# bentherien/point-cloud-reid

Hardware: NVIDIA B200
Metric: pair scores/sec (PT-256 encode + all-pairs xcorr_eff match) (higher is better)
Workload: dtype f16

## Files before the change

point-cloud-reid_b200/_lib.py:

```python
import ctypes
import os

_HERE = os.path.dirname(os.path.abspath(__file__))
LIB_PATH = os.path.join(_HERE, "libpcreid_sm100.so")
_lib = None

c_int, c_ll, c_float, c_vp = ctypes.c_int, ctypes.c_longlong, ctypes.c_float, ctypes.c_void_p


class LinearArgs(ctypes.Structure):
    _fields_ = [
        ("B", c_int), ("rows", c_int), ("CO", c_int), ("K1", c_int), ("K2", c_int),
        ("X1", c_vp), ("x1_bs", c_ll), ("ldx1", c_int), ("x1_pm", c_int), ("x1_map", c_vp),
        ("X2", c_vp), ("x2_bs", c_ll), ("ldx2", c_int), ("x2_pm", c_int), ("x2_map", c_vp),
        ("W1", c_vp), ("w1_bs", c_ll), ("w1_map", c_vp),
        ("W2", c_vp), ("w2_bs", c_ll),
        ("bias", c_vp),
        ("R", c_vp), ("r_bs", c_ll), ("ldr", c_int), ("r_map", c_vp), ("res_after_act", c_int),
        ("act", c_int),
        ("Y", c_vp), ("y_bs", c_ll), ("ldy", c_int), ("y_pm", c_int),
    ]


class NormArgs(ctypes.Structure):
    _fields_ = [
        ("B", c_int), ("rows", c_int), ("C", c_int), ("G", c_int),
        ("X", c_vp), ("x_bs", c_ll), ("ldx", c_int),
        ("gamma", c_vp), ("beta", c_vp),
        ("R", c_vp), ("r_bs", c_ll), ("ldr", c_int), ("r_map", c_vp),
        ("act", c_int),
        ("Y", c_vp), ("y_bs", c_ll), ("ldy", c_int),
    ]


_SIGS = {
    "pcreid_abi_version": [],
    "pcreid_fps": [c_int, c_int, c_int, c_vp, c_vp, c_vp, c_vp],
    "pcreid_fps_with_dist": [c_int, c_int, c_int, c_vp, c_vp, c_vp, c_vp],
    "pcreid_fps_block_size": [c_int],
    "pcreid_fps_torch": [c_int, c_int, c_int, c_vp, c_vp, c_vp, c_vp],
    "pcreid_pairwise_sqdist": [c_int, c_int, c_int, c_int, c_vp, c_vp, c_vp, c_int, c_vp],
    "pcreid_knn": [c_int, c_int, c_int, c_int, c_vp, c_vp, c_vp, c_vp, c_vp],
    "pcreid_knn_t": [c_int, c_int, c_int, c_int, c_vp, c_vp, c_vp, c_vp, c_vp],
    "pcreid_knn_point": [c_int, c_int, c_int, c_int, c_vp, c_vp, c_vp, c_vp],
    "pcreid_knn_point_set": [c_int, c_int, c_int, c_int, c_vp, c_vp, c_vp, c_vp],
    "pcreid_knn_feature": [c_int, c_int, c_int, c_int, c_vp, c_ll, c_vp, c_vp],
    "pcreid_ball_query": [c_int, c_int, c_int, c_float, c_float, c_int, c_vp, c_vp, c_vp, c_vp],
    "pcreid_query_ball_point": [c_int, c_int, c_int, c_float, c_int, c_vp, c_vp, c_vp, c_vp],
    "pcreid_group_points": [c_int, c_int, c_int, c_int, c_int, c_vp, c_vp, c_vp, c_vp],
    "pcreid_gather_points": [c_int, c_int, c_int, c_int, c_vp, c_vp, c_vp, c_vp],
    "pcreid_query_group": [c_int] * 5 + [c_vp] * 4 + [c_int, c_float, c_vp, c_vp, c_vp],
    "pcreid_crop_tiles": [c_int],
    "pcreid_crop_mask": [c_int, c_int, c_vp, c_int, c_vp, c_vp, c_vp, c_vp],
    "pcreid_crop_gather": [c_int, c_int, c_int, c_vp, c_int, c_vp, c_vp, c_vp, c_vp, c_vp, c_vp],
    "pcreid_three_nn": [c_int, c_int, c_int, c_vp, c_vp, c_vp, c_vp, c_vp],
    "pcreid_three_interpolate": [c_int, c_int, c_int, c_int, c_vp, c_vp, c_vp, c_vp, c_vp],
    "pcreid_cn_linear": [ctypes.POINTER(LinearArgs), c_vp],
    "pcreid_cn_linear_tc": [ctypes.POINTER(LinearArgs), c_vp],
    "pcreid_cn_linear_tc2": [ctypes.POINTER(LinearArgs), c_vp, c_vp, c_int, c_vp],
    "pcreid_cn_linear_tma": [ctypes.POINTER(LinearArgs), c_ll, c_ll, c_ll, c_int, c_int, c_vp],
    "pcreid_cn_linear_tma_x3": [ctypes.POINTER(LinearArgs), c_vp, c_vp, c_ll, c_ll, c_ll, c_int, c_vp],
    "pcreid_cn_groupnorm": [ctypes.POINTER(NormArgs), c_vp],
    "pcreid_gn_res_relu_dot": [c_int, c_int, c_int, c_vp, c_int, c_vp, c_vp, c_vp, c_int, c_vp, c_float, c_vp, c_vp],
    "pcreid_attn_front_blob_bytes": [c_int, c_int, c_int, c_int],
    "pcreid_attn_front": [c_int, c_int, c_int, c_int, c_int, c_int, c_vp, c_vp, c_ll, c_int, c_vp, c_vp, c_vp, c_vp, c_vp, c_ll, c_int,
                          c_vp],
    "pcreid_linattn_kv_img": [c_int, c_int, c_int, c_int, c_vp, c_ll, c_int, c_vp, c_ll, c_int, c_vp, c_vp, c_vp],
    "pcreid_attn_back_objects_per_tile": [c_int, c_int],
    "pcreid_attn_back_blob_bytes": [c_int, c_int, c_int, c_int],
    "pcreid_attn_back": [c_int] * 8 + [c_vp, c_ll, c_int, c_vp, c_ll, c_int] + [c_vp] * 7 + [c_vp, c_ll, c_int, c_vp],
    "pcreid_linattn_kv": [c_int, c_int, c_int, c_int, c_vp, c_ll, c_int, c_vp, c_ll, c_int, c_vp, c_vp, c_vp],
    "pcreid_linattn_scale": [c_int, c_int, c_int, c_int, c_int, c_vp, c_ll, c_int, c_vp, c_vp, c_vp, c_vp, c_ll, c_int, c_vp],
    "pcreid_local_linattn": [c_int, c_int, c_int, c_int, c_int, c_vp, c_vp, c_vp, c_vp],
    "pcreid_cn_pool": [c_int, c_int, c_int, c_vp, c_ll, c_int, c_int, c_vp, c_ll, c_int, c_int, c_vp, c_ll, c_ll, c_vp],
    "pcreid_cn_chanmax": [c_int, c_int, c_int, c_vp, c_ll, c_int, c_vp, c_ll, c_ll, c_vp],
    "pcreid_sa_edge_mlp": [c_int, c_int, c_int, c_int, c_int, c_vp, c_vp, c_vp, c_vp, c_vp, c_vp, c_vp, c_vp, c_vp],
    "pcreid_edge_build": [c_int, c_int, c_int, c_int, c_int, c_vp, c_vp, c_vp, c_vp, c_vp],
    "pcreid_seg_max": [c_ll, c_int, c_vp, c_vp, c_vp],
    "pcreid_seg_mean": [c_ll, c_int, c_vp, c_vp, c_vp],
    "pcreid_edge_gather_max": [c_int, c_int, c_int, c_int, c_vp, c_vp, c_vp, c_int, c_vp, c_ll, c_int, c_vp],
    "pcreid_pack_image": [c_int, c_int, c_int, c_vp, c_ll, c_int, c_int, c_int, c_vp, c_vp],
    "pcreid_pack_image_bias": [c_int, c_int, c_int, c_vp, c_ll, c_int, c_vp, c_int, c_vp, c_vp],
    "pcreid_pack_b7": [c_int, c_vp, c_vp, c_int, c_vp, c_vp],
    "pcreid_pool_finish2": [c_int, c_int, c_vp, c_vp, c_vp, c_vp],
    "pcreid_pair_p1a2": [c_int, c_int, c_int, c_int, c_float] + [c_vp] * 8 + [c_int, c_vp],
    "pcreid_pair_p1b_n": [c_int, c_int, c_int, c_int, c_float] + [c_vp] * 7 + [c_int, c_vp],
    "pcreid_pair_p2y": [c_int, c_int, c_int, c_int, c_float] + [c_vp] * 5 + [c_int, c_vp],
    "pcreid_sa_edge_mlp_tc": [c_int, c_int, c_int, c_int, c_int] + [c_vp] * 8 + [c_int, c_vp],
    "pcreid_sa_edge_mlp_tc2": [c_int, c_int, c_int, c_int, c_int] + [c_vp] * 8 + [c_int, c_int, c_vp],
    "pcreid_pair_concat_head_tc": [c_int, c_int, c_int, c_int] + [c_vp] * 10 + [c_float, c_vp, c_vp, c_int, c_vp],
    "pcreid_pair_concat_head": [c_int, c_int, c_int, c_int] + [c_vp] * 10 + [c_float, c_vp, c_vp, c_vp],
}

ERRORS = {1: "PCREID_ERR_ARG (bad pointer/size)", 2: "PCREID_ERR_LAUNCH (CUDA launch failed)",
          3: "PCREID_ERR_UNSUPPORTED (shape outside the built kernels)"}


def exported_symbols():
    return sorted(_SIGS.keys())


def lib():
    global _lib
    if _lib is not None:
        return _lib
    if not os.path.exists(LIB_PATH):
        from . import build as _build
        _build.build_library()
    if not os.path.exists(LIB_PATH):
        raise RuntimeError(f"{LIB_PATH} is missing and could not be built: the CUDA extension is required "
                           "(no CPU fallback exists)")
    L = ctypes.CDLL(LIB_PATH)
    for name, argt in _SIGS.items():
        fn = getattr(L, name)
        fn.argtypes = argt
        fn.restype = c_int
    _lib = L
    return L


ABI_CALLS = 0


def check(rc, what):
    global ABI_CALLS
    ABI_CALLS += 1
    if rc != 0:
        raise RuntimeError(f"{what} failed: {ERRORS.get(rc, rc)}")
```

point-cloud-reid_b200/csrc/attn_tc.cu:

```cuda
#include "../../include/pcreid.h"
#include "common.cuh"
#include "tc_common.cuh"

namespace {

constexpr int NTH = 128;
constexpr int RING = 3;
constexpr int MAXCH = 56;
constexpr int MAX_SLOT = 16384;

struct ChunkTab {
  int n;
  int slot_bytes;
  uint32_t off[MAXCH];
  uint32_t bytes[MAXCH];
  uint8_t per_obj[MAXCH];
};

__device__ __forceinline__ void expect_tx(uint64_t* bar, uint32_t bytes) {
  asm volatile("mbarrier.arrive.expect_tx.shared::cta.b64 _, [%0], %1;" ::"r"(tc::smem_u32(bar)), "r"(bytes) : "memory");
}
__device__ __forceinline__ void bulk_g2s(uint32_t dst, const void* src, uint32_t bytes, uint64_t* bar) {
  asm volatile("cp.async.bulk.shared::cluster.global.mbarrier::complete_tx::bytes [%0], [%1], %2, [%3];" ::"r"(dst), "l"(src),
               "r"(bytes), "r"(tc::smem_u32(bar))
               : "memory");
}

struct Pipe {
  uint64_t *full, *empty;
  uint32_t ring_s;
  const uint8_t *blob, *obj;
  const ChunkTab* tab;
  int loaded, used;
};

__device__ __forceinline__ void pipe_prefetch(Pipe& p) {
  while (p.loaded < p.tab->n && p.loaded < p.used + RING) {
    const int s = p.loaded % RING, n = p.loaded / RING;
    if (n > 0) tc::mbar_wait(&p.empty[s], (uint32_t)((n - 1) & 1));
    const uint8_t* src = (p.tab->per_obj[p.loaded] ? p.obj : p.blob) + p.tab->off[p.loaded];
    const uint32_t nb = p.tab->bytes[p.loaded];
    expect_tx(&p.full[s], nb);
    bulk_g2s(p.ring_s + (uint32_t)(s * p.tab->slot_bytes), src, nb, &p.full[s]);
    ++p.loaded;
  }
}

__device__ __forceinline__ void pipe_gemm(Pipe& p, uint32_t tmem_d, uint32_t a_img_s, int K, int N, bool accumulate) {
  int kk = 0;
  while (kk < K) {
    pipe_prefetch(p);
    const int s = p.used % RING, n = p.used / RING;
    const int kc = (int)(p.tab->bytes[p.used] / (uint32_t)(N * 4));
    tc::mbar_wait(&p.full[s], (uint32_t)(n & 1));
    tc::tc_fence_after();
    const uint32_t slot = p.ring_s + (uint32_t)(s * p.tab->slot_bytes);
    for (int n0 = 0; n0 < N; n0 += 256) {
      const int nb = min(256, N - n0);
      const uint32_t idesc = tc::instr_desc(128, nb, tc::FMT_TF32, tc::MAJOR_K, tc::MAJOR_K);
      for (int ks = 0; ks < kc / 8; ++ks) {
        const uint64_t ad = tc::smem_desc(a_img_s + (uint32_t)(((kk >> 3) + ks) * 4096), 2048, 128, tc::LAYOUT_NONE);
        const uint64_t bd = tc::smem_desc(slot + (uint32_t)(ks * 2 * N * 16 + n0 * 16), (uint32_t)(N * 16), 128, tc::LAYOUT_NONE);
        tc::umma_tf32(tmem_d + (uint32_t)n0, ad, bd, idesc, (accumulate || kk > 0 || ks > 0) ? 1u : 0u);
      }
    }
    tc::umma_commit(&p.empty[s]);
    ++p.used;
    kk += kc;
  }
}

__device__ __forceinline__ void stage_sync() {
  tc::fence_async_smem();
  tc::tc_fence_before();
  __syncthreads();
  tc::tc_fence_after();
}

__device__ __forceinline__ float elu1(float v) { return v > 0.f ? v + 1.f : __expf(v); }

template <bool RNA>
__device__ __forceinline__ void load_image_cm(uint8_t* img, const float* __restrict__ Xr, int ld, int C, int CP, bool valid, int tid) {
  for (int c0 = 0; c0 < CP; c0 += 32) {
    float v[32];
#pragma unroll
    for (int i = 0; i < 32; ++i) v[i] = (valid && c0 + i < C) ? __ldg(Xr + (size_t)(c0 + i) * ld) : 0.f;
#pragma unroll
    for (int j = 0; j < 8; ++j)
      if (c0 + 4 * j < CP)
        *reinterpret_cast<float4*>(img + ((c0 >> 2) + j) * 2048 + tid * 16) =
            RNA ? tc::tf32_rna4(make_float4(v[4 * j], v[4 * j + 1], v[4 * j + 2], v[4 * j + 3])) : make_float4(v[4 * j], v[4 * j + 1], v[4 * j + 2], v[4 * j + 3]);
  }
}
template <bool RNA>
__device__ __forceinline__ void load_image_pm(uint8_t* img, const float* __restrict__ x, int C, int CP, bool valid, int tid) {
  for (int c0 = 0; c0 < CP; c0 += 32) {
    float v[32];
#pragma unroll
    for (int i = 0; i < 32; ++i) v[i] = (valid && c0 + i < C) ? __ldg(x + c0 + i) : 0.f;
#pragma unroll
    for (int j = 0; j < 8; ++j)
      if (c0 + 4 * j < CP)
        *reinterpret_cast<float4*>(img + ((c0 >> 2) + j) * 2048 + tid * 16) =
            RNA ? tc::tf32_rna4(make_float4(v[4 * j], v[4 * j + 1], v[4 * j + 2], v[4 * j + 3])) : make_float4(v[4 * j], v[4 * j + 1], v[4 * j + 2], v[4 * j + 3]);
  }
}

__device__ __forceinline__ void row_stats(uint32_t tl, int n, float& mean, float& rstd) {
  float s = 0.f;
  for (int q = 0; q < n / 16; ++q) {
    uint32_t r[16];
    tc::tmem_ld16(tl + 16 * q, r);
    tc::tmem_ld_wait();
#pragma unroll
    for (int j = 0; j < 16; ++j) s += __uint_as_float(r[j]);
  }
  mean = s / (float)n;
  float v = 0.f;
  for (int q = 0; q < n / 16; ++q) {
    uint32_t r[16];
    tc::tmem_ld16(tl + 16 * q, r);
    tc::tmem_ld_wait();
#pragma unroll
    for (int j = 0; j < 16; ++j) {
      const float d = __uint_as_float(r[j]) - mean;
      v = fmaf(d, d, v);
    }
  }
  rstd = rsqrtf(v / (float)n + 1e-5f);
}

__host__ __device__ inline int tmem_cols(int n) {
  int c = 32;
  while (c < n) c <<= 1;
  return c;
}

struct FrontArgs {
  int B, S, C2, DP, NFP, NF;
  const float* xyz;
  const float* feat;
  long long f_bs;
  int ldf;
  const float *wp0, *bp0, *bp2;
  const uint8_t* blob;
  float* out;
  long long o_bs;
  int ldo;
  ChunkTab tab;
};

__global__ void __launch_bounds__(NTH) attn_front_kernel(const __grid_constant__ FrontArgs a) {
  extern __shared__ __align__(128) uint8_t smem[];
  __shared__ uint64_t full[RING], empty[RING], stagebar;
  __shared__ uint32_t tmem_base_s;
  const int tid = threadIdx.x, warp = tid >> 5;
  const long long flat = (long long)blockIdx.x * 128 + tid;
  const bool valid = flat < (long long)a.B * a.S;
  const int b = valid ? (int)(flat / a.S) : 0, row = valid ? (int)(flat % a.S) : 0;
  const int CA = a.DP > a.C2 ? a.DP : a.C2;
  uint8_t* imgF = smem;
  uint8_t* imgA = imgF + a.C2 * 512;
  uint8_t* ring = imgA + CA * 512;
  float* wp0_s = reinterpret_cast<float*>(ring + RING * a.tab.slot_bytes);
  float* bp0_s = wp0_s + 3 * a.DP;
  float* bp2_s = bp0_s + a.DP;
  const int ncols = a.NFP + a.NF;
  if (tid == 0) {
    for (int i = 0; i < RING; ++i) { tc::mbar_init(&full[i], 1); tc::mbar_init(&empty[i], 1); }
    tc::mbar_init(&stagebar, 1);
    tc::fence_mbar_init();
  }
  if (warp == 0) { tc::tmem_alloc(&tmem_base_s, (uint32_t)tmem_cols(max(ncols, a.C2))); tc::tmem_relinquish(); }
  for (int i = tid; i < 3 * a.DP; i += NTH) wp0_s[i] = a.wp0[i];
  for (int i = tid; i < a.DP; i += NTH) bp0_s[i] = a.bp0[i];
  for (int i = tid; i < a.C2; i += NTH) bp2_s[i] = a.bp2[i];
  tc::tc_fence_before();
  __syncthreads();
  tc::tc_fence_after();
  Pipe p;
  if (tid == 0) {
    p.full = full; p.empty = empty; p.ring_s = tc::smem_u32(ring); p.blob = a.blob; p.obj = nullptr; p.tab = &a.tab;
    p.loaded = 0; p.used = 0;
    pipe_prefetch(p);
  }
  const uint32_t tmem = tmem_base_s;
  const uint32_t tl = tmem + ((uint32_t)(warp * 32) << 16);
  uint32_t par = 0;
  load_image_cm<false>(imgF, a.feat + (size_t)b * a.f_bs + row, a.ldf, a.C2, a.C2, valid, tid);
  {
    float x = 0.f, y = 0.f, z = 0.f;
    if (valid) {
      const float* pp = a.xyz + ((size_t)b * a.S + row) * 3;
      x = __ldg(pp); y = __ldg(pp + 1); z = __ldg(pp + 2);
    }
    for (int c4 = 0; c4 < a.DP / 4; ++c4) {
      float h[4];
#pragma unroll
      for (int j = 0; j < 4; ++j) {
        const int c = 4 * c4 + j;
        h[j] = fmaxf(fmaf(x, wp0_s[c], fmaf(y, wp0_s[a.DP + c], fmaf(z, wp0_s[2 * a.DP + c], bp0_s[c]))), 0.f);
      }
      *reinterpret_cast<float4*>(imgA + c4 * 2048 + tid * 16) = tc::tf32_rna4(make_float4(h[0], h[1], h[2], h[3]));
    }
  }
  stage_sync();
  if (tid == 0) {
    pipe_gemm(p, tmem, tc::smem_u32(imgA), a.DP, a.C2, false);
    tc::umma_commit(&stagebar);
    pipe_prefetch(p);
  }
  __syncwarp();
  tc::mbar_wait(&stagebar, par);
  par ^= 1u;
  tc::tc_fence_after();
  for (int q = 0; q < a.C2 / 16; ++q) {
    uint32_t r[16];
    tc::tmem_ld16(tl + 16 * q, r);
    tc::tmem_ld_wait();
#pragma unroll
    for (int j = 0; j < 16; j += 4) {
      const int c = 16 * q + j;
      const float4 f = *reinterpret_cast<const float4*>(imgF + (c / 4) * 2048 + tid * 16);
      float4 v;
      v.x = __uint_as_float(r[j + 0]) + bp2_s[c + 0] + f.x;
      v.y = __uint_as_float(r[j + 1]) + bp2_s[c + 1] + f.y;
      v.z = __uint_as_float(r[j + 2]) + bp2_s[c + 2] + f.z;
      v.w = __uint_as_float(r[j + 3]) + bp2_s[c + 3] + f.w;
      *reinterpret_cast<float4*>(imgA + (c / 4) * 2048 + tid * 16) = tc::tf32_rna4(v);
      *reinterpret_cast<float4*>(imgF + (c / 4) * 2048 + tid * 16) = tc::tf32_rna4(f);
    }
  }
  stage_sync();
  if (tid == 0) {
    pipe_gemm(p, tmem, tc::smem_u32(imgA), a.C2, a.NFP, false);
    if (a.NF > 0) pipe_gemm(p, tmem + (uint32_t)a.NFP, tc::smem_u32(imgF), a.C2, a.NF, false);
    tc::umma_commit(&stagebar);
  }
  __syncwarp();
  tc::mbar_wait(&stagebar, par);
  par ^= 1u;
  tc::tc_fence_after();
  float* O = a.out + (size_t)b * a.o_bs;
  for (int q = 0; q < ncols / 16; ++q) {
    uint32_t r[16];
    tc::tmem_ld16(tl + 16 * q, r);
    tc::tmem_ld_wait();
    if (valid) {
#pragma unroll
      for (int j = 0; j < 16; ++j) O[(size_t)(16 * q + j) * a.ldo + row] = __uint_as_float(r[j]);
    }
  }
  tc::tc_fence_before();
  __syncthreads();
  if (warp == 0) tc::tmem_dealloc(tmem, (uint32_t)tmem_cols(max(ncols, a.C2)));
}

constexpr int KV_SC = 64, KV_SCP = KV_SC + 4;
template <int TPT>
__global__ void __launch_bounds__(256, 3) linattn_kv_img_kernel(int S, int d, int H, const float* __restrict__ K, long long k_bs, int ldk,
                                                             const float* __restrict__ V, long long v_bs, int ldv,
                                                             float* __restrict__ kvimg, float* __restrict__ ksum) {
  extern __shared__ __align__(16) float kvs[];
  float* Ks = kvs;
  float* Vs = kvs + d * KV_SCP;
  const int b = blockIdx.x, tid = threadIdx.x, dh = d / H, nb = dh / 4;
  const int ntiles = H * nb * nb;
  const int G = ntiles >= 256 ? 1 : 256 / ntiles;
  const float* Kb = K + (size_t)b * k_bs;
  const float* Vb = V + (size_t)b * v_bs;
  float acc[TPT][4][4];
#pragma unroll
  for (int u = 0; u < TPT; ++u)
#pragma unroll
    for (int i = 0; i < 4; ++i)
#pragma unroll
      for (int j = 0; j < 4; ++j) acc[u][i][j] = 0.f;
  float ks = 0.f;
  const int g = G > 1 ? tid / ntiles : 0;
  for (int s0 = 0; s0 < S; s0 += KV_SC) {
    for (int i0 = tid; i0 < d * KV_SC; i0 += 256 * 8) {
      float kq[8], vq[8];
#pragma unroll
      for (int e = 0; e < 8; ++e) {
        const int i = i0 + e * 256, c = i / KV_SC, s = i % KV_SC;
        const bool in = i < d * KV_SC && s0 + s < S;
        kq[e] = in ? __ldg(Kb + (size_t)c * ldk + s0 + s) : 0.f;
        vq[e] = in ? __ldg(Vb + (size_t)c * ldv + s0 + s) : 0.f;
      }
#pragma unroll
      for (int e = 0; e < 8; ++e) {
        const int i = i0 + e * 256, c = i / KV_SC, s = i % KV_SC;
        if (i < d * KV_SC) {
          Ks[c * KV_SCP + s] = s0 + s < S ? elu1(kq[e]) : 0.f;
          Vs[c * KV_SCP + s] = vq[e];
        }
      }
    }
    __syncthreads();
    if (tid < d) {
      const float4* kr = reinterpret_cast<const float4*>(Ks + tid * KV_SCP);
#pragma unroll 4
      for (int s = 0; s < KV_SC / 4; ++s) { const float4 x = kr[s]; ks += (x.x + x.y) + (x.z + x.w); }
    }
#pragma unroll
    for (int u = 0; u < TPT; ++u) {
      const int tile = (G > 1 ? tid % ntiles : tid) + u * 256;
      if (tile < ntiles) {
        const int h = tile / (nb * nb), ti = (tile % (nb * nb)) / nb, tj = tile % nb;
        const float* kr = Ks + (h * dh + 4 * ti) * KV_SCP;
        const float* vr = Vs + (h * dh + 4 * tj) * KV_SCP;
        for (int s = 4 * g; s < KV_SC; s += 4 * G) {
          float4 kq[4], vq[4];
#pragma unroll
          for (int i = 0; i < 4; ++i) kq[i] = *reinterpret_cast<const float4*>(kr + i * KV_SCP + s);
#pragma unroll
          for (int j = 0; j < 4; ++j) vq[j] = *reinterpret_cast<const float4*>(vr + j * KV_SCP + s);
#pragma unroll
          for (int i = 0; i < 4; ++i)
#pragma unroll
            for (int j = 0; j < 4; ++j)
              acc[u][i][j] = fmaf(kq[i].x, vq[j].x, fmaf(kq[i].y, vq[j].y, fmaf(kq[i].z, vq[j].z, fmaf(kq[i].w, vq[j].w, acc[u][i][j]))));
        }
      }
    }
    __syncthreads();
  }
  if (tid < d) ksum[(size_t)b * d + tid] = ks;
  if (G > 1) {
    float* red = kvs;
    const int tile = tid % ntiles;
#pragma unroll
    for (int i = 0; i < 4; ++i)
      *reinterpret_cast<float4*>(red + ((size_t)(g * ntiles + tile) * 16) + 4 * i) = make_float4(acc[0][i][0], acc[0][i][1], acc[0][i][2], acc[0][i][3]);
    __syncthreads();
    if (g == 0) {
      for (int gg = 1; gg < G; ++gg)
#pragma unroll
        for (int i = 0; i < 4; ++i) {
          const float4 x = *reinterpret_cast<const float4*>(red + ((size_t)(gg * ntiles + tile) * 16) + 4 * i);
          acc[0][i][0] += x.x; acc[0][i][1] += x.y; acc[0][i][2] += x.z; acc[0][i][3] += x.w;
        }
    }
  }
  float* img = kvimg + (size_t)b * d * dh;
#pragma unroll
  for (int u = 0; u < TPT; ++u) {
    const int tile = (G > 1 ? tid % ntiles : tid) + u * 256;
    if (tile < ntiles && g == 0) {
      const int h = tile / (nb * nb), ti = (tile % (nb * nb)) / nb, tj = tile % nb;
      float* ih = img + (size_t)h * dh * dh;
#pragma unroll
      for (int j = 0; j < 4; ++j)
        *reinterpret_cast<float4*>(ih + ((size_t)ti * dh + 4 * tj + j) * 4) = tc::tf32_rna4(make_float4(acc[u][0][j], acc[u][1][j], acc[u][2][j], acc[u][3][j]));
    }
  }
}

struct BackArgs {
  int B, rows, D, H, C1, C1P, CO, opt;
  int qpre, res, f1_pm;
  const float* feat1;
  long long f1_bs;
  int ldf1;
  const float* q;
  long long q_bs;
  int ldq;
  const float* ksum;
  const uint8_t* kvimg;
  const float *g1, *b1, *g2, *b2;
  const uint8_t* blob;
  float* out;
  long long o_bs;
  int ldo;
  ChunkTab tab;
};

__global__ void __launch_bounds__(NTH) attn_back_kernel(const __grid_constant__ BackArgs a) {
  extern __shared__ __align__(128) uint8_t smem[];
  __shared__ uint64_t full[RING], empty[RING], stagebar;
  __shared__ uint32_t tmem_base_s;
  const int tid = threadIdx.x, warp = tid >> 5;
  const int D = a.D, D2 = 2 * a.D, dh = a.D / a.H;
  int b0, ob, row;
  bool valid;
  if (a.opt > 1) {
    b0 = blockIdx.x * a.opt; ob = tid / a.rows; row = tid % a.rows;
    valid = b0 + ob < a.B;
  } else {
    const int tpo = (a.rows + 127) / 128;
    b0 = blockIdx.x / tpo; ob = 0; row = (blockIdx.x % tpo) * 128 + tid;
    valid = row < a.rows;
  }
  const int b = valid ? b0 + ob : b0;
  const int img_ch = (a.C1P + D) > D2 ? (a.C1P + D) : D2;
  uint8_t* imgF = smem;
  uint8_t* imgQ = imgF + a.C1P * 512;
  uint8_t* imgH = smem;
  uint8_t* ring = smem + img_ch * 512;
  float* ksum_s = reinterpret_cast<float*>(ring + RING * a.tab.slot_bytes);
  float* g1_s = ksum_s + a.opt * D;
  float* b1_s = g1_s + D;
  float* g2_s = b1_s + D;
  float* b2_s = g2_s + a.CO;
  const int tcols = tmem_cols(max(max(D2, a.CO), a.opt * D));
  if (tid == 0) {
    for (int i = 0; i < RING; ++i) { tc::mbar_init(&full[i], 1); tc::mbar_init(&empty[i], 1); }
    tc::mbar_init(&stagebar, 1);
    tc::fence_mbar_init();
  }
  if (warp == 0) { tc::tmem_alloc(&tmem_base_s, (uint32_t)tcols); tc::tmem_relinquish(); }
  for (int i = tid; i < a.opt * D; i += NTH) ksum_s[i] = (b0 + i / D < a.B) ? a.ksum[(size_t)(b0 + i / D) * D + i % D] : 0.f;
  for (int i = tid; i < D; i += NTH) { g1_s[i] = a.g1[i]; b1_s[i] = a.b1[i]; }
  for (int i = tid; i < a.CO; i += NTH) { g2_s[i] = a.g2[i]; b2_s[i] = a.b2[i]; }
  tc::tc_fence_before();
  __syncthreads();
  tc::tc_fence_after();
  Pipe p;
  if (tid == 0) {
    p.full = full; p.empty = empty; p.ring_s = tc::smem_u32(ring); p.blob = a.blob;
    p.obj = a.kvimg + (size_t)b0 * D * dh * 4; p.tab = &a.tab;
    p.loaded = 0; p.used = 0;
    pipe_prefetch(p);
  }
  const uint32_t tmem = tmem_base_s;
  const uint32_t tl = tmem + ((uint32_t)(warp * 32) << 16);
  uint32_t par = 0;
  const float* F1 = a.feat1 + (size_t)b * a.f1_bs;
  if (a.f1_pm) load_image_pm<true>(imgF, F1 + (size_t)row * a.C1, a.C1, a.C1P, valid, tid);
  else load_image_cm<true>(imgF, F1 + row, a.ldf1, a.C1, a.C1P, valid, tid);
  const float* ksr = ksum_s + ob * D;

  float z[4] = {0.f, 0.f, 0.f, 0.f};
  if (a.qpre) {
    const float* Q = a.q + (size_t)b * a.q_bs + row;
    float dot[4] = {0.f, 0.f, 0.f, 0.f};
    for (int c0 = 0; c0 < D; c0 += 16) {
      float v[16];
#pragma unroll
      for (int i = 0; i < 16; ++i) v[i] = valid ? __ldg(Q + (size_t)(c0 + i) * a.ldq) : 0.f;
      const int h = c0 / dh;
      float dd = 0.f;
#pragma unroll
      for (int i = 0; i < 16; ++i) {
        v[i] = elu1(v[i]);
        dd = fmaf(v[i], ksr[c0 + i], dd);
      }
#pragma unroll
      for (int hh = 0; hh < 4; ++hh) dot[hh] += (hh == h) ? dd : 0.f;
#pragma unroll
      for (int j = 0; j < 4; ++j)
        *reinterpret_cast<float4*>(imgQ + ((c0 >> 2) + j) * 2048 + tid * 16) = tc::tf32_rna4(make_float4(v[4 * j], v[4 * j + 1], v[4 * j + 2], v[4 * j + 3]));
    }
#pragma unroll
    for (int hh = 0; hh < 4; ++hh) z[hh] = 1.f / (dot[hh] + 1e-6f);
    stage_sync();
  } else {
    stage_sync();
    if (tid == 0) {
      pipe_gemm(p, tmem, tc::smem_u32(imgF), a.C1P, D, false);
      tc::umma_commit(&stagebar);
      pipe_prefetch(p);
    }
    __syncwarp();
    tc::mbar_wait(&stagebar, par);
    par ^= 1u;
    tc::tc_fence_after();
    float dot[4] = {0.f, 0.f, 0.f, 0.f};
    for (int q = 0; q < D / 16; ++q) {
      uint32_t r[16];
      tc::tmem_ld16(tl + 16 * q, r);
      tc::tmem_ld_wait();
      const int h = (16 * q) / dh;
      float v[16];
      float dd = 0.f;
#pragma unroll
      for (int j = 0; j < 16; ++j) {
        v[j] = elu1(__uint_as_float(r[j]));
        dd = fmaf(v[j], ksr[16 * q + j], dd);
      }
#pragma unroll
      for (int hh = 0; hh < 4; ++hh) dot[hh] += (hh == h) ? dd : 0.f;
#pragma unroll
      for (int j = 0; j < 16; j += 4)
        *reinterpret_cast<float4*>(imgQ + ((16 * q + j) / 4) * 2048 + tid * 16) = tc::tf32_rna4(make_float4(v[j], v[j + 1], v[j + 2], v[j + 3]));
    }
#pragma unroll
    for (int hh = 0; hh < 4; ++hh) z[hh] = 1.f / (dot[hh] + 1e-6f);
    stage_sync();
  }
  if (tid == 0) {
    for (int o = 0; o < a.opt; ++o)
      for (int h = 0; h < a.H; ++h)
        pipe_gemm(p, tmem + (uint32_t)(o * D + h * dh), tc::smem_u32(imgQ) + (uint32_t)((h * dh / 8) * 4096), dh, dh, false);
    tc::umma_commit(&stagebar);
    pipe_prefetch(p);
  }
  __syncwarp();
  tc::mbar_wait(&stagebar, par);
  par ^= 1u;
  tc::tc_fence_after();
  for (int q = 0; q < D / 16; ++q) {
    uint32_t r[16];
    tc::tmem_ld16(tl + (uint32_t)(ob * D + 16 * q), r);
    tc::tmem_ld_wait();
    const int h = (16 * q) / dh;
    float zz = z[0];
#pragma unroll
    for (int hh = 1; hh < 4; ++hh) zz = (hh == h) ? z[hh] : zz;
#pragma unroll
    for (int j = 0; j < 16; j += 4)
      *reinterpret_cast<float4*>(imgQ + ((16 * q + j) / 4) * 2048 + tid * 16) =
          tc::tf32_rna4(make_float4(__uint_as_float(r[j]) * zz, __uint_as_float(r[j + 1]) * zz, __uint_as_float(r[j + 2]) * zz, __uint_as_float(r[j + 3]) * zz));
  }
  stage_sync();
  if (tid == 0) {
    pipe_gemm(p, tmem, tc::smem_u32(imgQ), D, D, false);
    tc::umma_commit(&stagebar);
    pipe_prefetch(p);
  }
  __syncwarp();
  tc::mbar_wait(&stagebar, par);
  par ^= 1u;
  tc::tc_fence_after();
  {
    float mean, rstd;
    row_stats(tl, D, mean, rstd);
    for (int q = 0; q < D / 16; ++q) {
      uint32_t r[16];
      tc::tmem_ld16(tl + 16 * q, r);
      tc::tmem_ld_wait();
#pragma unroll
      for (int j = 0; j < 16; j += 4) {
        const int c = 16 * q + j;
        float4 v;
        v.x = (__uint_as_float(r[j + 0]) - mean) * rstd * g1_s[c + 0] + b1_s[c + 0];
        v.y = (__uint_as_float(r[j + 1]) - mean) * rstd * g1_s[c + 1] + b1_s[c + 1];
        v.z = (__uint_as_float(r[j + 2]) - mean) * rstd * g1_s[c + 2] + b1_s[c + 2];
        v.w = (__uint_as_float(r[j + 3]) - mean) * rstd * g1_s[c + 3] + b1_s[c + 3];
        *reinterpret_cast<float4*>(imgQ + (c / 4) * 2048 + tid * 16) = tc::tf32_rna4(v);
      }
    }
  }
  stage_sync();
  if (tid == 0) {
    pipe_gemm(p, tmem, tc::smem_u32(imgF), a.C1P, D2, false);
    pipe_gemm(p, tmem, tc::smem_u32(imgQ), D, D2, true);
    tc::umma_commit(&stagebar);
    pipe_prefetch(p);
  }
  __syncwarp();
  tc::mbar_wait(&stagebar, par);
  par ^= 1u;
  tc::tc_fence_after();
  for (int q = 0; q < D2 / 16; ++q) {
    uint32_t r[16];
    tc::tmem_ld16(tl + 16 * q, r);
    tc::tmem_ld_wait();
#pragma unroll
    for (int j = 0; j < 16; j += 4) {
      float4 v;
      v.x = fmaxf(__uint_as_float(r[j + 0]), 0.f);
      v.y = fmaxf(__uint_as_float(r[j + 1]), 0.f);
      v.z = fmaxf(__uint_as_float(r[j + 2]), 0.f);
      v.w = fmaxf(__uint_as_float(r[j + 3]), 0.f);
      *reinterpret_cast<float4*>(imgH + ((16 * q + j) / 4) * 2048 + tid * 16) = tc::tf32_rna4(v);
    }
  }
  stage_sync();
  if (tid == 0) {
    pipe_gemm(p, tmem, tc::smem_u32(imgH), D2, a.CO, false);
    tc::umma_commit(&stagebar);
  }
  __syncwarp();
  tc::mbar_wait(&stagebar, par);
  par ^= 1u;
  tc::tc_fence_after();
  {
    float mean, rstd;
    row_stats(tl, a.CO, mean, rstd);
    float* O = a.out + (size_t)b * a.o_bs;
    for (int q = 0; q < a.CO / 16; ++q) {
      uint32_t r[16];
      tc::tmem_ld16(tl + 16 * q, r);
      tc::tmem_ld_wait();
      if (valid) {
        float rr[16];
#pragma unroll
        for (int j = 0; j < 16; ++j) {
          const int c = 16 * q + j;
          rr[j] = !a.res ? 0.f : (a.f1_pm ? __ldg(F1 + (size_t)row * a.C1 + c) : __ldg(F1 + (size_t)c * a.ldf1 + row));
        }
#pragma unroll
        for (int j = 0; j < 16; ++j) {
          const int c = 16 * q + j;
          O[(size_t)c * a.ldo + row] = (__uint_as_float(r[j]) - mean) * rstd * g2_s[c] + b2_s[c] + rr[j];
        }
      }
    }
  }
  tc::tc_fence_before();
  __syncthreads();
  if (warp == 0) tc::tmem_dealloc(tmem, (uint32_t)tcols);
}

struct TabBuilder {
  ChunkTab t;
  uint32_t blob_off = 0;
  bool ok = true;
  int cap;
  explicit TabBuilder(int img_bytes) : cap(img_bytes > 96 * 1024 ? MAX_SLOT : 8192) { t.n = 0; t.slot_bytes = 0; }
  void part(int K, int N, bool per_obj, uint32_t obj_off = 0) {
    int kc = K < 32 ? K : 32;
    while (kc > 8 && kc * N * 4 > cap) kc >>= 1;
    if (kc * N * 4 > MAX_SLOT || (K % 8) || (N % 16)) { ok = false; return; }
    uint32_t off = per_obj ? obj_off : blob_off;
    for (int kk = 0; kk < K; kk += kc) {
      const int k = (K - kk) < kc ? (K - kk) : kc;
      if (t.n >= MAXCH) { ok = false; return; }
      t.off[t.n] = off;
      t.bytes[t.n] = (uint32_t)(k * N * 4);
      t.per_obj[t.n] = per_obj ? 1 : 0;
      if ((int)t.bytes[t.n] > t.slot_bytes) t.slot_bytes = (int)t.bytes[t.n];
      off += t.bytes[t.n];
      ++t.n;
    }
    if (!per_obj) blob_off = off;
  }
  void finish() { t.slot_bytes = (t.slot_bytes + 1023) & ~1023; }
};

}

extern "C" {

int pcreid_attn_front_blob_bytes(int C2, int DP, int NFP, int NF) { return 4 * (DP * C2 + C2 * NFP + C2 * NF); }

int pcreid_attn_front(int B, int S, int C2, int DP, int NFP, int NF, const float* xyz, const float* feat, long long f_bs, int ldf,
                      const float* wp0, const float* bp0, const float* bp2, const void* blob, float* out, long long o_bs, int ldo,
                      void* stream) {
  if (B <= 0 || S <= 0) return PCREID_OK;
  if (!xyz || !feat || !wp0 || !bp0 || !bp2 || !blob || !out) return PCREID_ERR_ARG;
  if (C2 % 16 || DP % 16 || NFP % 16 || NF % 16 || NFP <= 0 || C2 > 128 || DP > 128 || NFP + NF > 512 || ((long long)B * S + 127) / 128 > 0x7fffffffLL)
    return PCREID_ERR_UNSUPPORTED;
  FrontArgs a;
  a.B = B; a.S = S; a.C2 = C2; a.DP = DP; a.NFP = NFP; a.NF = NF;
  a.xyz = xyz; a.feat = feat; a.f_bs = f_bs; a.ldf = ldf; a.wp0 = wp0; a.bp0 = bp0; a.bp2 = bp2;
  a.blob = static_cast<const uint8_t*>(blob); a.out = out; a.o_bs = o_bs; a.ldo = ldo;
  TabBuilder tb((C2 + (DP > C2 ? DP : C2)) * 512);
  tb.part(DP, C2, false);
  tb.part(C2, NFP, false);
  if (NF > 0) tb.part(C2, NF, false);
  tb.finish();
  if (!tb.ok) return PCREID_ERR_UNSUPPORTED;
  a.tab = tb.t;
  const int CA = DP > C2 ? DP : C2;
  const int smem = (C2 + CA) * 512 + RING * a.tab.slot_bytes + (4 * DP + C2) * 4;
  if (smem > 227 * 1024) return PCREID_ERR_UNSUPPORTED;
  cudaFuncSetAttribute(attn_front_kernel, cudaFuncAttributeMaxDynamicSharedMemorySize, smem);
  attn_front_kernel<<<(unsigned)(((long long)B * S + 127) / 128), NTH, smem, (cudaStream_t)stream>>>(a);
  return pcreid_launch_status();
}

int pcreid_linattn_kv_img(int B, int S, int d, int H, const float* K, long long k_bs, int ldk, const float* V, long long v_bs, int ldv,
                          float* kvimg, float* ksum, void* stream) {
  if (B <= 0) return PCREID_OK;
  if (!K || !V || !kvimg || !ksum || H <= 0 || S <= 0) return PCREID_ERR_ARG;
  if (d % H || (d / H) % 4 || d > 128 || d < 16) return PCREID_ERR_UNSUPPORTED;
  const int ntiles = H * (d / H / 4) * (d / H / 4);
  if (ntiles > 512 || (ntiles < 256 && 256 % ntiles)) return PCREID_ERR_UNSUPPORTED;
  const int G = ntiles >= 256 ? 1 : 256 / ntiles;
  int smem = 2 * d * KV_SCP * 4;
  if (G > 1 && G * ntiles * 16 * 4 > smem) smem = G * ntiles * 16 * 4;
  if (ntiles > 256) {
    if (smem > 48 * 1024) cudaFuncSetAttribute(linattn_kv_img_kernel<2>, cudaFuncAttributeMaxDynamicSharedMemorySize, smem);
    linattn_kv_img_kernel<2><<<B, 256, smem, (cudaStream_t)stream>>>(S, d, H, K, k_bs, ldk, V, v_bs, ldv, kvimg, ksum);
  } else {
    if (smem > 48 * 1024) cudaFuncSetAttribute(linattn_kv_img_kernel<1>, cudaFuncAttributeMaxDynamicSharedMemorySize, smem);
    linattn_kv_img_kernel<1><<<B, 256, smem, (cudaStream_t)stream>>>(S, d, H, K, k_bs, ldk, V, v_bs, ldv, kvimg, ksum);
  }
  return pcreid_launch_status();
}

int pcreid_attn_back_objects_per_tile(int rows, int D) {
  if (rows >= 128 || rows <= 0 || 128 % rows) return 1;
  const int opt = 128 / rows;
  return (opt <= 4 && opt * D <= 512) ? opt : 1;
}

int pcreid_attn_back_blob_bytes(int D, int C1P, int CO, int qpre) {
  return 4 * ((qpre ? 0 : C1P * D) + D * D + C1P * 2 * D + D * 2 * D + 2 * D * CO);
}

int pcreid_attn_back(int B, int rows, int D, int H, int C1, int CO, int res, int f1_pm, const float* feat1, long long f1_bs,
                     int ldf1, const float* q, long long q_bs, int ldq, const float* ksum, const float* kvimg, const float* g1,
                     const float* b1, const float* g2, const float* b2, const void* blob, float* out, long long o_bs, int ldo,
                     void* stream) {
  if (B <= 0 || rows <= 0) return PCREID_OK;
  if (!feat1 || !ksum || !kvimg || !g1 || !b1 || !g2 || !b2 || !blob || !out || H <= 0) return PCREID_ERR_ARG;
  const int C1P = (C1 + 7) & ~7;
  if (D % 16 || D > 128 || H > 4 || D % H || (D / H) % 16 || CO % 16 || CO > 2 * D || C1 <= 0 || C1P > 128) return PCREID_ERR_UNSUPPORTED;
  if (res && C1 != CO) return PCREID_ERR_ARG;
  const int dh = D / H;
  BackArgs a;
  a.B = B; a.rows = rows; a.D = D; a.H = H; a.C1 = C1; a.C1P = C1P; a.CO = CO;
  a.opt = pcreid_attn_back_objects_per_tile(rows, D);
  a.qpre = q ? 1 : 0; a.res = res; a.f1_pm = f1_pm;
  a.feat1 = feat1; a.f1_bs = f1_bs; a.ldf1 = ldf1; a.q = q; a.q_bs = q_bs; a.ldq = ldq; a.ksum = ksum;
  a.kvimg = reinterpret_cast<const uint8_t*>(kvimg); a.g1 = g1; a.b1 = b1; a.g2 = g2; a.b2 = b2;
  a.blob = static_cast<const uint8_t*>(blob); a.out = out; a.o_bs = o_bs; a.ldo = ldo;
  const long long tiles = a.opt > 1 ? ((long long)B + a.opt - 1) / a.opt : (long long)B * ((rows + 127) / 128);
  if (tiles > 0x7fffffffLL) return PCREID_ERR_UNSUPPORTED;
  TabBuilder tb(((C1P + D) > 2 * D ? (C1P + D) : 2 * D) * 512);
  if (!q) tb.part(C1P, D, false);
  for (int o = 0; o < a.opt; ++o)
    for (int h = 0; h < H; ++h) tb.part(dh, dh, true, (uint32_t)((o * H + h) * dh * dh * 4));
  tb.part(D, D, false);
  tb.part(C1P, 2 * D, false);
  tb.part(D, 2 * D, false);
  tb.part(2 * D, CO, false);
  tb.finish();
  if (!tb.ok) return PCREID_ERR_UNSUPPORTED;
  a.tab = tb.t;
  const int img_ch = (C1P + D) > 2 * D ? (C1P + D) : 2 * D;
  const int smem = img_ch * 512 + RING * a.tab.slot_bytes + ((a.opt + 2) * D + 2 * CO) * 4;
  if (smem > 227 * 1024 - 256) return PCREID_ERR_UNSUPPORTED;
  cudaFuncSetAttribute(attn_back_kernel, cudaFuncAttributeMaxDynamicSharedMemorySize, smem);
  attn_back_kernel<<<(unsigned)tiles, NTH, smem, (cudaStream_t)stream>>>(a);
  return pcreid_launch_status();
}

}
```

point-cloud-reid_b200/csrc/pair_common.cuh:

```cuda
#pragma once
#include "../../include/pcreid.h"
#include "common.cuh"
#include "tc_common.cuh"

namespace {


constexpr int IMG = 16384;
constexpr int NB7H = 80;
constexpr int B7_HEAD = (NB7H / 8) * 32 * 16;
constexpr int B7_BYTES = 2 * B7_HEAD;
constexpr int ONES_BYTES = 2 * 2048;
constexpr float LN_EPS = 1e-5f;

struct P1Args {
  int n_units, NT, role;
  int npts;
  float att_eps;
  float kv_scale;
  const int *u_search, *u_templ, *u_slot;
  const uint8_t *QF1, *H, *PV;
  const uint8_t* MK1;
  const uint8_t* W;
  uint8_t* A_out;
  uint8_t* B7_out;
};
struct P2Args {
  int n_units, NT, role;
  int npts;
  float att_eps;
  const int* u_slot;
  const uint8_t* A_in;
  const uint8_t* B7_in;
  const uint8_t* W;
  float* pool_part;
};

__device__ __forceinline__ float elu1(float x) { return x > 0.f ? x + 1.f : __expf(x); }

__device__ __forceinline__ uint4 ldg_early(const void* p) {
  uint4 v;
  asm volatile("ld.global.nc.L1::no_allocate.v4.u32 {%0,%1,%2,%3}, [%4];" : "=r"(v.x), "=r"(v.y), "=r"(v.z), "=r"(v.w) : "l"(p));
  return v;
}

__device__ __forceinline__ void prefetch_l2_16k(const uint8_t* img, int t) {
  asm volatile("prefetch.global.L2 [%0];" ::"l"(img + (size_t)t * 128));
}

__device__ __forceinline__ void copy_to_smem(uint8_t* dst, const uint8_t* __restrict__ src, int bytes, int t, int nthr) {
  for (int i = t * 16; i < bytes; i += nthr * 16) cp_async16(dst + i, src + i);
}

struct Opnd {
  uint64_t desc;
  uint32_t kstep;
};
__device__ __forceinline__ Opnd opnd(uint32_t addr, uint32_t lbo, uint32_t sbo, uint32_t kstep_bytes) {
  Opnd o;
  o.desc = tc::smem_desc(addr, lbo, sbo, tc::LAYOUT_NONE);
  o.kstep = kstep_bytes >> 4;
  return o;
}
#define A_IMG(addr) opnd((addr), 2048u, 128u, 4096u)
#define W_IMG(addr, N) opnd((addr), (uint32_t)((N)*16), 128u, (uint32_t)(2 * (N)*16))
#define B7_IMG(addr) opnd((addr), 128u, 512u, 256u)

template <int KSTEPS>
__device__ __forceinline__ void issue_gemm(uint32_t tmem_d, const Opnd& A, const Opnd& B, uint32_t idesc, bool accumulate) {
#pragma unroll
  for (int ks = 0; ks < KSTEPS; ++ks)
    tc::umma_f16(tmem_d, A.desc + (uint64_t)(ks * A.kstep), B.desc + (uint64_t)(ks * B.kstep), idesc, (accumulate || ks > 0) ? 1u : 0u);
}

template <int NCH>
__device__ __forceinline__ void load_side(uint4 (&sd)[NCH], const uint8_t* __restrict__ img, int chunk0, int row) {
#pragma unroll
  for (int c = 0; c < NCH; ++c) sd[c] = __ldg(reinterpret_cast<const uint4*>(img + (chunk0 + c) * 2048 + row * 16));
}

template <class F>
__device__ __forceinline__ void write_b7_part(const float (&M32)[32], int c_lo, float ksum, bool tail, int d, uint8_t* dst) {
  uint8_t* base = dst + (d >> 5) * B7_HEAD + (d & 31) * 16;
#pragma unroll
  for (int c = 0; c < 4; ++c) {
    uint32_t w[4];
#pragma unroll
    for (int j = 0; j < 4; ++j) w[j] = F::pack(M32[c * 8 + 2 * j], M32[c * 8 + 2 * j + 1]);
    *reinterpret_cast<uint4*>(base + (c_lo + c) * 512) = make_uint4(w[0], w[1], w[2], w[3]);
  }
  if (tail) {
    *reinterpret_cast<uint4*>(base + 8 * 512) = make_uint4(F::pack(ksum, 0.f), 0, 0, 0);
    *reinterpret_cast<uint4*>(base + 9 * 512) = make_uint4(0, 0, 0, 0);
  }
}

constexpr int GX = 128, NGX = 3;
struct GroupX {
  int t, gid;
  bool issuer;
  uint32_t tmem, tlane;
  uint64_t* bar;
  uint32_t par;
  __device__ __forceinline__ void sync() { tc::bar_sync(1 + gid, GX); }
  __device__ __forceinline__ void publish() { tc::fence_async_smem(); tc::tc_fence_before(); sync(); tc::tc_fence_after(); }
  __device__ __forceinline__ void wait() { tc::mbar_wait(bar, par); par ^= 1u; tc::tc_fence_after(); }
};

__device__ __forceinline__ void ld32_stats(uint32_t taddr, float (&o)[32], float& s, float& ss) {
#pragma unroll
  for (int half = 0; half < 2; ++half) {
    uint32_t r[16];
    tc::tmem_ld16(taddr + 16 * half, r);
    tc::tmem_ld_wait();
#pragma unroll
    for (int j = 0; j < 16; ++j) {
      const float v = __uint_as_float(r[j]);
      o[16 * half + j] = v;
      s += v;
      ss = fmaf(v, v, ss);
    }
  }
}

template <class F>
__device__ __forceinline__ void write_b7_row(const float (&M)[64], float ksum, int d, uint8_t* dst) {
  float lo[32], hi[32];
#pragma unroll
  for (int j = 0; j < 32; ++j) { lo[j] = M[j]; hi[j] = M[32 + j]; }
  write_b7_part<F>(lo, 0, ksum, true, d, dst);
  write_b7_part<F>(hi, 4, ksum, false, d, dst);
}

__device__ __forceinline__ void groupx_setup(GroupX& g, uint64_t* bars, uint32_t tmem_base) {
  const int warp_u = (int)tc::uniform(threadIdx.x >> 5);
  g.gid = warp_u / 4;
  g.t = threadIdx.x % GX;
  g.issuer = (warp_u % 4) == 0;
  g.tmem = tc::uniform(tmem_base) + g.gid * 160;
  g.tlane = g.tmem + ((uint32_t)((warp_u % 4) * 32) << 16);
  g.bar = bars + g.gid;
  g.par = 0;
}

}
```

point-cloud-reid_b200/csrc/pair_tc.cu:

```cuda
#include "pair_common.cuh"
#include <stdlib.h>

namespace {

constexpr int P1B_WKV = 0, P1B_WM = 16384, P1B_WBYTES = 24576;
constexpr int P1B_AIMG = 0, P1B_KFV = IMG, P1B_GBYTES = IMG + 2 * IMG + ONES_BYTES;

template <class F, int CS>
__global__ void __launch_bounds__(NGX * GX * CS, 1) pair_p1b_kernel(const P1Args a) {
  constexpr int GT = GX * CS, NTHR = NGX * GT;
  constexpr int QB = 4 / CS, CB = 8 / CS;
  extern __shared__ __align__(1024) uint8_t smem[];
  __shared__ uint64_t bars[2 * NGX];
  __shared__ uint32_t tmem_base_s;
  uint8_t* Wsm = smem;
  if (threadIdx.x == 0) {
    for (int i = 0; i < 2 * NGX; ++i) tc::mbar_init(&bars[i], 1);
    tc::fence_mbar_init();
  }
  if (threadIdx.x < 32) { tc::tmem_alloc(&tmem_base_s, 512); tc::tmem_relinquish(); }
  copy_to_smem(Wsm, a.W, P1B_WBYTES, threadIdx.x, NTHR);
  cp_async_commit();
  cp_async_wait<0>();
  tc::fence_async_smem();
  tc::tc_fence_before();
  __syncthreads();
  tc::tc_fence_after();
  const int warp_u = (int)tc::uniform(threadIdx.x >> 5);
  const int gid = warp_u / (4 * CS), wg = warp_u % (4 * CS), gt = threadIdx.x % GT;
  const int half = wg / 4;
  const int row = (wg % 4) * 32 + (threadIdx.x & 31);
  const bool issuer = wg == 0;
  const uint32_t tmem = tc::uniform(tmem_base_s) + gid * 160;
  const uint32_t tlane = tmem + ((uint32_t)((wg % 4) * 32) << 16);
  uint64_t* bar = bars + gid;
  uint32_t par = 0;
  auto gsync = [&]() { tc::bar_sync(1 + gid, GT); };
  auto publish = [&]() { tc::fence_async_smem(); tc::tc_fence_before(); gsync(); tc::tc_fence_after(); };
  auto gwait = [&]() { tc::mbar_wait(bar, par); par ^= 1u; tc::tc_fence_after(); };
  uint64_t* bar2 = bars + NGX + gid;
  uint32_t par2 = 0;
  uint8_t* G = smem + P1B_WBYTES + gid * P1B_GBYTES;
  uint8_t* Aimg = G + P1B_AIMG;
  uint8_t* KfV = G + P1B_KFV;
  {
    uint4* ones = reinterpret_cast<uint4*>(KfV + 2 * IMG);
    for (int i = gt; i < 256; i += GT) ones[i] = i < 128 ? make_uint4(F::ONE_LO, 0, 0, 0) : make_uint4(0, 0, 0, 0);
  }
  const uint32_t sA = tc::smem_u32(Aimg), sKfV = tc::smem_u32(KfV), sW = tc::smem_u32(Wsm);
  const uint32_t id64 = tc::instr_desc(128, 64, F::FMT, tc::MAJOR_K, tc::MAJOR_K);
  const uint32_t idkv = tc::instr_desc(128, 80, F::FMT, tc::MAJOR_MN, tc::MAJOR_MN);
  const Opnd oA = A_IMG(sA), oWk = W_IMG(sW + P1B_WKV, 128), oWv = W_IMG(sW + P1B_WKV + 64 * 16, 128), oWm = W_IMG(sW + P1B_WM, 64),
             oKfV = opnd(sKfV, 128u, 2048u, 256u), oVones = opnd(sKfV + 8 * 2048, 128u, 2048u, 256u);
  const uint32_t KVC = 64;

  const int ngroups = gridDim.x * NGX, gg = blockIdx.x * NGX + gid;
  const int u0 = (int)((long long)a.n_units * gg / ngroups), u1 = (int)((long long)a.n_units * (gg + 1) / ngroups);
  int so_next = u0 < u1 ? a.u_search[u0] : 0, slot_next = u0 < u1 ? a.u_slot[u0] : 0;
  bool prefetched = false;
  for (int u = u0; u < u1; ++u) {
    const int so = so_next, slot = slot_next;
    if (u + 1 < u1) { so_next = a.u_search[u + 1]; slot_next = a.u_slot[u + 1]; }
    for (int tile = 0; tile < a.NT; ++tile) {
      const size_t ti = (size_t)so * a.NT + tile;
      if (!prefetched) copy_to_smem(Aimg, a.A_out + (((size_t)slot * 2 + a.role) * a.NT + tile) * IMG, IMG, gt, GT);
      prefetched = false;
      cp_async_commit();
      {
        int ns = slot, nt = tile + 1;
        if (nt == a.NT) { ns = slot_next; nt = 0; }
        if ((nt != 0 || u + 1 < u1) && gt < 128) prefetch_l2_16k(a.A_out + (((size_t)ns * 2 + a.role) * a.NT + nt) * IMG, gt);
      }
      cp_async_wait<0>();
      publish();
      if (issuer) { if (tc::elect_one()) { issue_gemm<4>(tmem, oA, oWk, id64, false); tc::umma_commit(bar); } __syncwarp(); }
      gwait();
      if (tile > 0) { tc::mbar_wait(bar2, par2); par2 ^= 1u; tc::tc_fence_after(); }
      {
        const bool keep = tile * 128 + row < a.npts;
#pragma unroll
        for (int qq = 0; qq < QB; ++qq) {
          const int q = half * QB + qq;
          uint32_t r[16];
          tc::tmem_ld16(tlane + 16 * q, r);
          tc::tmem_ld_wait();
#pragma unroll
          for (int c = 0; c < 2; ++c) {
            uint32_t w[4];
#pragma unroll
            for (int j = 0; j < 4; ++j)
              w[j] = keep ? F::elu1(__uint_as_float(r[c * 8 + 2 * j]), __uint_as_float(r[c * 8 + 2 * j + 1])) : 0u;
            *reinterpret_cast<uint4*>(KfV + (2 * q + c) * 2048 + row * 16) = make_uint4(w[0], w[1], w[2], w[3]);
          }
        }
      }
      tc::tc_fence_before();
      gsync();
      tc::tc_fence_after();
      if (issuer) { if (tc::elect_one()) { issue_gemm<4>(tmem, oA, oWv, id64, false); tc::umma_commit(bar); } __syncwarp(); }
      {
        uint4 sdPV[CB];
        load_side<CB>(sdPV, a.PV + ti * IMG, half * CB, row);
        gwait();
        if (tile + 1 < a.NT) {
          copy_to_smem(Aimg, a.A_out + (((size_t)slot * 2 + a.role) * a.NT + tile + 1) * IMG, IMG, gt, GT);
          cp_async_commit();
          prefetched = true;
        }
#pragma unroll
        for (int qq = 0; qq < QB; ++qq) {
          const int q = half * QB + qq;
          uint32_t r[16];
          tc::tmem_ld16(tlane + 16 * q, r);
          tc::tmem_ld_wait();
#pragma unroll
          for (int c = 0; c < 2; ++c) {
            const uint4 s4 = sdPV[2 * qq + c];
            const uint32_t sw[4] = {s4.x, s4.y, s4.z, s4.w};
            uint32_t w[4];
#pragma unroll
            for (int j = 0; j < 4; ++j)
              w[j] = F::add(__uint_as_float(r[c * 8 + 2 * j]), __uint_as_float(r[c * 8 + 2 * j + 1]), sw[j]);
            *reinterpret_cast<uint4*>(KfV + (8 + 2 * q + c) * 2048 + row * 16) = make_uint4(w[0], w[1], w[2], w[3]);
          }
        }
      }
      publish();
      if (issuer) {
        if (tc::elect_one()) { issue_gemm<8>(tmem + KVC, oKfV, oVones, idkv, tile > 0); tc::umma_commit(bar2); }
        __syncwarp();
      }
    }
    tc::mbar_wait(bar2, par2);
    par2 ^= 1u;
    tc::tc_fence_after();
    {
      float kv[64 / CS];
      float ksum = 0.f;
      if (row < 64) {
#pragma unroll
        for (int qq = 0; qq < QB; ++qq) {
          uint32_t r[16];
          tc::tmem_ld16(tlane + KVC + 16 * (half * QB + qq), r);
          tc::tmem_ld_wait();
#pragma unroll
          for (int j = 0; j < 16; ++j) kv[16 * qq + j] = __uint_as_float(r[j]) * a.kv_scale;
        }
        uint32_t r8[8];
        tc::tmem_ld8(tlane + KVC + 64, r8);
        tc::tmem_ld_wait();
        ksum = __uint_as_float(r8[0]) * a.kv_scale;
        const int hd = row >> 5;
#pragma unroll
        for (int cc = 0; cc < CB; ++cc) {
          const int c = half * CB + cc;
          uint32_t w[4];
#pragma unroll
          for (int j = 0; j < 4; ++j) w[j] = ((c >> 2) == hd) ? F::pack(kv[cc * 8 + 2 * j], kv[cc * 8 + 2 * j + 1]) : 0u;
          *reinterpret_cast<uint4*>(Aimg + c * 2048 + row * 16) = make_uint4(w[0], w[1], w[2], w[3]);
        }
      } else {
#pragma unroll
        for (int cc = 0; cc < CB; ++cc) *reinterpret_cast<uint4*>(Aimg + (half * CB + cc) * 2048 + row * 16) = make_uint4(0, 0, 0, 0);
      }
      publish();
      if (issuer) { if (tc::elect_one()) { issue_gemm<4>(tmem, oA, oWm, id64, false); tc::umma_commit(bar); } __syncwarp(); }
      gwait();
      if (u + 1 < u1) {
        copy_to_smem(Aimg, a.A_out + ((size_t)slot_next * 2 + a.role) * a.NT * IMG, IMG, gt, GT);
        cp_async_commit();
        prefetched = true;
      }
      if (row < 64) {
#pragma unroll
        for (int qq = 0; qq < QB; ++qq) {
          uint32_t r[16];
          tc::tmem_ld16(tlane + 16 * (half * QB + qq), r);
          tc::tmem_ld_wait();
#pragma unroll
          for (int j = 0; j < 16; ++j) kv[16 * qq + j] = __uint_as_float(r[j]);
        }
        uint8_t* dst = a.B7_out + ((size_t)slot * 2 + a.role) * B7_BYTES;
        if constexpr (CS == 1) write_b7_row<F>(kv, ksum, row, dst);
        else write_b7_part<F>(kv, 4 * half, ksum, half == 0, row, dst);
      }
      tc::tc_fence_before();
      gsync();
    }
  }
  tc::tc_fence_before();
  __syncthreads();
  if (threadIdx.x < 32) tc::tmem_dealloc(tmem_base_s, 512);
}

template <class F>
__global__ void __launch_bounds__(NGX * GX, 1) pair_p1b2_kernel(const P1Args a) {
  constexpr int TG = 168, KVC = 64, AC = 136;
  extern __shared__ __align__(1024) uint8_t smem[];
  __shared__ uint64_t bars[2 * NGX];
  __shared__ uint32_t tmem_base_s;
  __shared__ float ksum_s[NGX][64];
  uint8_t* Wsm = smem;
  if (threadIdx.x == 0) {
    for (int i = 0; i < 2 * NGX; ++i) tc::mbar_init(&bars[i], 1);
    tc::fence_mbar_init();
  }
  if (threadIdx.x < 32) { tc::tmem_alloc(&tmem_base_s, 512); tc::tmem_relinquish(); }
  copy_to_smem(Wsm, a.W, P1B_WBYTES, threadIdx.x, NGX * GX);
  cp_async_commit();
  cp_async_wait<0>();
  tc::fence_async_smem();
  tc::tc_fence_before();
  __syncthreads();
  tc::tc_fence_after();
  const int warp_u = (int)tc::uniform(threadIdx.x >> 5);
  const int gid = warp_u / 4, wq = warp_u % 4, row = threadIdx.x % GX, lane = threadIdx.x & 31;
  const bool issuer = wq == 0;
  const uint32_t tmem = tc::uniform(tmem_base_s) + gid * TG;
  const uint32_t tlane = tmem + ((uint32_t)(wq * 32) << 16);
  uint64_t* bar = bars + gid;
  uint32_t par = 0;
  auto gsync = [&]() { tc::bar_sync(1 + gid, GX); };
  auto publish = [&]() { tc::fence_async_smem(); tc::tc_fence_before(); gsync(); tc::tc_fence_after(); };
  auto gwait = [&]() { tc::mbar_wait(bar, par); par ^= 1u; tc::tc_fence_after(); };
  uint64_t* bar2 = bars + NGX + gid;
  uint32_t par2 = 0;
  uint8_t* G = smem + P1B_WBYTES + gid * P1B_GBYTES;
  uint8_t* Aimg = G + P1B_AIMG;
  uint8_t* KfV = G + P1B_KFV;
  {
    uint4* ones = reinterpret_cast<uint4*>(KfV + 2 * IMG);
    ones[row] = make_uint4(F::ONE_LO, 0, 0, 0);
    ones[128 + row] = make_uint4(0, 0, 0, 0);
  }
  const uint32_t sA = tc::smem_u32(Aimg), sKfV = tc::smem_u32(KfV), sW = tc::smem_u32(Wsm);
  const uint32_t id64 = tc::instr_desc(128, 64, F::FMT, tc::MAJOR_K, tc::MAJOR_K);
  const uint32_t idkv = tc::instr_desc(64, 72, F::FMT, tc::MAJOR_MN, tc::MAJOR_MN);
  const Opnd oA = A_IMG(sA), oWk = W_IMG(sW + P1B_WKV, 128), oWv = W_IMG(sW + P1B_WKV + 64 * 16, 128), oWm = W_IMG(sW + P1B_WM, 64),
             oKf = opnd(sKfV, 128u, 2048u, 256u), oVones = opnd(sKfV + 8 * 2048, 128u, 2048u, 256u);

  const int ngroups = gridDim.x * NGX, gg = blockIdx.x * NGX + gid;
  const int u0 = (int)((long long)a.n_units * gg / ngroups), u1 = (int)((long long)a.n_units * (gg + 1) / ngroups);
  int so_next = u0 < u1 ? a.u_search[u0] : 0, slot_next = u0 < u1 ? a.u_slot[u0] : 0;
  uint32_t areg[32];
  auto load_row = [&](const uint8_t* img) {
#pragma unroll
    for (int c = 0; c < 8; ++c) {
      const uint4 v = ldg_early(img + c * 2048 + row * 16);
      areg[4 * c] = v.x; areg[4 * c + 1] = v.y; areg[4 * c + 2] = v.z; areg[4 * c + 3] = v.w;
    }
  };
  if (u0 < u1) load_row(a.A_out + ((size_t)slot_next * 2 + a.role) * a.NT * IMG);
  for (int u = u0; u < u1; ++u) {
    const int so = so_next, slot = slot_next;
    if (u + 1 < u1) { so_next = a.u_search[u + 1]; slot_next = a.u_slot[u + 1]; }
    for (int tile = 0; tile < a.NT; ++tile) {
      const size_t ti = (size_t)so * a.NT + tile;
      tc::tmem_st32(tlane + AC, areg);
      tc::tmem_st_wait();
      tc::tc_fence_before();
      gsync();
      tc::tc_fence_after();
      if (issuer) {
        if (tc::elect_one()) {
#pragma unroll
          for (int ks = 0; ks < 4; ++ks) tc::umma_f16_ts(tmem, tmem + AC + 8 * ks, oWk.desc + (uint64_t)(ks * oWk.kstep), id64, ks > 0 ? 1u : 0u);
          tc::umma_commit(bar);
        }
        __syncwarp();
      }
      {
        int ns = slot, nt = tile + 1;
        if (nt == a.NT) { ns = slot_next; nt = 0; }
        if (nt != 0 || u + 1 < u1) {
          load_row(a.A_out + (((size_t)ns * 2 + a.role) * a.NT + nt) * IMG);
          int ns2 = ns, nt2 = nt + 1;
          if (nt2 == a.NT) { nt2 = 0; ns2 = -1; }
          if (ns2 >= 0) prefetch_l2_16k(a.A_out + (((size_t)ns2 * 2 + a.role) * a.NT + nt2) * IMG, row);
        }
      }
      gwait();
      if (tile > 0) { tc::mbar_wait(bar2, par2); par2 ^= 1u; tc::tc_fence_after(); }
      {
        const bool keep = tile * 128 + row < a.npts;
#pragma unroll
        for (int q = 0; q < 4; ++q) {
          uint32_t r[16];
          tc::tmem_ld16(tlane + 16 * q, r);
          tc::tmem_ld_wait();
#pragma unroll
          for (int c = 0; c < 2; ++c) {
            uint32_t w[4];
#pragma unroll
            for (int j = 0; j < 4; ++j)
              w[j] = keep ? F::elu1(__uint_as_float(r[c * 8 + 2 * j]), __uint_as_float(r[c * 8 + 2 * j + 1])) : 0u;
            *reinterpret_cast<uint4*>(KfV + (2 * q + c) * 2048 + row * 16) = make_uint4(w[0], w[1], w[2], w[3]);
          }
        }
      }
      tc::tc_fence_before();
      gsync();
      tc::tc_fence_after();
      if (issuer) {
        if (tc::elect_one()) {
#pragma unroll
          for (int ks = 0; ks < 4; ++ks) tc::umma_f16_ts(tmem, tmem + AC + 8 * ks, oWv.desc + (uint64_t)(ks * oWv.kstep), id64, ks > 0 ? 1u : 0u);
          tc::umma_commit(bar);
        }
        __syncwarp();
      }
      {
        uint4 sdPV[8];
        load_side<8>(sdPV, a.PV + ti * IMG, 0, row);
        gwait();
#pragma unroll
        for (int q = 0; q < 4; ++q) {
          uint32_t r[16];
          tc::tmem_ld16(tlane + 16 * q, r);
          tc::tmem_ld_wait();
#pragma unroll
          for (int c = 0; c < 2; ++c) {
            const uint4 s4 = sdPV[2 * q + c];
            const uint32_t sw[4] = {s4.x, s4.y, s4.z, s4.w};
            uint32_t w[4];
#pragma unroll
            for (int j = 0; j < 4; ++j)
              w[j] = F::add(__uint_as_float(r[c * 8 + 2 * j]), __uint_as_float(r[c * 8 + 2 * j + 1]), sw[j]);
            *reinterpret_cast<uint4*>(KfV + (8 + 2 * q + c) * 2048 + row * 16) = make_uint4(w[0], w[1], w[2], w[3]);
          }
        }
      }
      publish();
      if (issuer) {
        if (tc::elect_one()) { issue_gemm<8>(tmem + KVC, oKf, oVones, idkv, tile > 0); tc::umma_commit(bar2); }
        __syncwarp();
      }
    }
    tc::mbar_wait(bar2, par2);
    par2 ^= 1u;
    tc::tc_fence_after();
    {
      {
        float kv[64];
        uint32_t r8[8];
#pragma unroll
        for (int q = 0; q < 4; ++q) {
          uint32_t r[16];
          tc::tmem_ld16(tlane + KVC + 16 * q, r);
          tc::tmem_ld_wait();
#pragma unroll
          for (int j = 0; j < 16; ++j) kv[16 * q + j] = __uint_as_float(r[j]) * a.kv_scale;
        }
        tc::tmem_ld8(tlane + KVC + 64, r8);
        tc::tmem_ld_wait();
        if (lane < 16) {
          const int i = 16 * wq + lane, hd = i >> 5;
          ksum_s[gid][i] = __uint_as_float(r8[0]) * a.kv_scale;
#pragma unroll
          for (int c = 0; c < 8; ++c) {
            uint32_t w[4];
#pragma unroll
            for (int j = 0; j < 4; ++j) w[j] = ((c >> 2) == hd) ? F::pack(kv[c * 8 + 2 * j], kv[c * 8 + 2 * j + 1]) : 0u;
            *reinterpret_cast<uint4*>(Aimg + c * 2048 + i * 16) = make_uint4(w[0], w[1], w[2], w[3]);
          }
        }
      }
      if (row >= 64) {
#pragma unroll
        for (int c = 0; c < 8; ++c) *reinterpret_cast<uint4*>(Aimg + c * 2048 + row * 16) = make_uint4(0, 0, 0, 0);
      }
      publish();
      if (issuer) { if (tc::elect_one()) { issue_gemm<4>(tmem, oA, oWm, id64, false); tc::umma_commit(bar); } __syncwarp(); }
      gwait();
      if (row < 64) {
        float kv[64];
#pragma unroll
        for (int q = 0; q < 4; ++q) {
          uint32_t r[16];
          tc::tmem_ld16(tlane + 16 * q, r);
          tc::tmem_ld_wait();
#pragma unroll
          for (int j = 0; j < 16; ++j) kv[16 * q + j] = __uint_as_float(r[j]);
        }
        write_b7_row<F>(kv, ksum_s[gid][row], row, a.B7_out + ((size_t)slot * 2 + a.role) * B7_BYTES);
      }
      tc::tc_fence_before();
      gsync();
    }
  }
  tc::tc_fence_before();
  __syncthreads();
  if (threadIdx.x < 32) tc::tmem_dealloc(tmem_base_s, 512);
}


template <class F>
__global__ void __launch_bounds__(256) pack_image_kernel(int B, int C, int N, const float* __restrict__ src, long long s_bs,
                                                         int lds, int act, uint8_t* __restrict__ dst) {
  const int nt = (N + 127) / 128, nch = C / 8;
  const long long idx = (long long)blockIdx.x * blockDim.x + threadIdx.x;
  const int row = (int)(idx % 128);
  const int chunk = (int)((idx / 128) % nch);
  const int tile = (int)((idx / (128LL * nch)) % nt);
  const long long b = idx / (128LL * nch * nt);
  if (b >= B) return;
  const float* s = src + b * s_bs + (size_t)(chunk * 8) * lds + tile * 128 + row;
  uint32_t w[4] = {0u, 0u, 0u, 0u};
  if (tile * 128 + row < N) {
#pragma unroll
    for (int j = 0; j < 4; ++j) {
      float x0 = s[(size_t)(2 * j) * lds], x1 = s[(size_t)(2 * j + 1) * lds];
      if (act == ACT_ELU1) { x0 = x0 > 0.f ? x0 + 1.f : expf(x0); x1 = x1 > 0.f ? x1 + 1.f : expf(x1); }
      w[j] = F::pack(x0, x1);
    }
  }
  *reinterpret_cast<uint4*>(dst + (((size_t)b * nt + tile) * nch + chunk) * 2048 + row * 16) = make_uint4(w[0], w[1], w[2], w[3]);
}

template <class F>
__global__ void __launch_bounds__(64) pack_b7_kernel(const float* __restrict__ M, const float* __restrict__ ksum,
                                                     uint8_t* __restrict__ dst) {
  const int b = blockIdx.x, d = threadIdx.x;
  float m[64];
#pragma unroll
  for (int j = 0; j < 64; ++j) m[j] = M[((size_t)b * 64 + d) * 64 + j];
  write_b7_row<F>(m, ksum[(size_t)b * 64 + d], d, dst + (size_t)b * B7_BYTES);
}

}

template <class F, int CS>
static int launch_p1b_cs(const P1Args& a, int grid, cudaStream_t st) {
  const int smem = P1B_WBYTES + NGX * P1B_GBYTES;
  cudaFuncSetAttribute(pair_p1b_kernel<F, CS>, cudaFuncAttributeMaxDynamicSharedMemorySize, smem);
  pair_p1b_kernel<F, CS><<<grid, NGX * GX * CS, smem, st>>>(a);
  return pcreid_launch_status();
}
template <class F>
static int launch_p1b(const P1Args& a, int grid, cudaStream_t st) {
  static const int gen = [] { const char* e = getenv("PCREID_P1B"); return e ? atoi(e) : 2; }();
  static const int cs = [] { const char* e = getenv("PCREID_P1B_SPLIT"); return e ? atoi(e) : 1; }();
  if (gen == 2) {
    const int smem = P1B_WBYTES + NGX * P1B_GBYTES;
    cudaFuncSetAttribute(pair_p1b2_kernel<F>, cudaFuncAttributeMaxDynamicSharedMemorySize, smem);
    pair_p1b2_kernel<F><<<grid, NGX * GX, smem, st>>>(a);
    return pcreid_launch_status();
  }
  return cs == 2 ? launch_p1b_cs<F, 2>(a, grid, st) : launch_p1b_cs<F, 1>(a, grid, st);
}

extern "C" {

int pcreid_pack_image(int B, int C, int N, const float* src, long long s_bs, int lds, int act, int fmt, void* dst, void* stream) {
  if (B <= 0) return PCREID_OK;
  if (!src || !dst || C % 8 || N <= 0 || (fmt != PCREID_FMT_BF16 && fmt != PCREID_FMT_F16)) return PCREID_ERR_ARG;
  const long long per = 128LL * (C / 8) * ((N + 127) / 128);
  const unsigned grid = (unsigned)((per * B + 255) / 256);
  if (fmt == PCREID_FMT_F16)
    pack_image_kernel<tc::OpF16><<<grid, 256, 0, (cudaStream_t)stream>>>(B, C, N, src, s_bs, lds, act, (uint8_t*)dst);
  else
    pack_image_kernel<tc::OpBF16><<<grid, 256, 0, (cudaStream_t)stream>>>(B, C, N, src, s_bs, lds, act, (uint8_t*)dst);
  return pcreid_launch_status();
}

int pcreid_pack_b7(int B, const float* M, const float* ksum, int fmt, void* dst, void* stream) {
  if (B <= 0) return PCREID_OK;
  if (!M || !ksum || !dst || (fmt != PCREID_FMT_BF16 && fmt != PCREID_FMT_F16)) return PCREID_ERR_ARG;
  if (fmt == PCREID_FMT_F16) pack_b7_kernel<tc::OpF16><<<B, 64, 0, (cudaStream_t)stream>>>(M, ksum, (uint8_t*)dst);
  else pack_b7_kernel<tc::OpBF16><<<B, 64, 0, (cudaStream_t)stream>>>(M, ksum, (uint8_t*)dst);
  return pcreid_launch_status();
}

int pcreid_pair_p1b_n(int n_units, int npts, int role, int fmt, float kv_scale, const int* u_search, const int* u_templ,
                      const int* u_slot, const void* PV, const void* W, void* A_out, void* B7_out, int n_ctas, void* stream) {
  if (n_units <= 0) return PCREID_OK;
  if (!u_search || !u_templ || !u_slot || !PV || !W || !A_out || !B7_out || npts <= 0 ||
      (fmt != PCREID_FMT_BF16 && fmt != PCREID_FMT_F16))
    return PCREID_ERR_ARG;
  const int NT = (npts + 127) / 128;
  P1Args a{n_units, NT, role, npts, 0.f, kv_scale, u_search, u_templ, u_slot, nullptr, nullptr, (const uint8_t*)PV, nullptr,
           (const uint8_t*)W, (uint8_t*)A_out, (uint8_t*)B7_out};
  int grid = n_ctas > 0 ? n_ctas : 148;
  if (grid * NGX > n_units) grid = (n_units + NGX - 1) / NGX;
  return fmt == PCREID_FMT_F16 ? launch_p1b<tc::OpF16>(a, grid, (cudaStream_t)stream) : launch_p1b<tc::OpBF16>(a, grid, (cudaStream_t)stream);
}

}
```

point-cloud-reid_b200/csrc/rowops.cu:

```cuda
#include "../../include/pcreid.h"
#include "common.cuh"

namespace {

constexpr int TR = 128;
constexpr int KC = 16;
constexpr int NTHR = 256;

template <int TN>
struct TileCols { static constexpr int value = 16 * TN; };

template <int TN>
__device__ __forceinline__ void fma_chunk(const float* __restrict__ Xs, const float* __restrict__ Ws, int tx, int ty,
                                          float (&acc)[8][TN]) {
  constexpr int TC = TileCols<TN>::value;
#pragma unroll
  for (int kk = 0; kk < KC; ++kk) {
    const float4 a0 = *reinterpret_cast<const float4*>(Xs + kk * TR + tx * 4);
    const float4 a1 = *reinterpret_cast<const float4*>(Xs + kk * TR + 64 + tx * 4);
    const float a[8] = {a0.x, a0.y, a0.z, a0.w, a1.x, a1.y, a1.z, a1.w};
    float w[TN];
    {
      const float4 w0 = *reinterpret_cast<const float4*>(Ws + kk * TC + ty * 4);
      w[0] = w0.x; w[1] = w0.y; w[2] = w0.z; w[3] = w0.w;
      if (TN == 8) {
        const float4 w1 = *reinterpret_cast<const float4*>(Ws + kk * TC + 64 + ty * 4);
        w[TN - 4] = w1.x; w[TN - 3] = w1.y; w[TN - 2] = w1.z; w[TN - 1] = w1.w;
      }
    }
#pragma unroll
    for (int i = 0; i < 8; ++i)
#pragma unroll
      for (int j = 0; j < TN; ++j) acc[i][j] = fmaf(a[i], w[j], acc[i][j]);
  }
}

template <int TN>
__device__ __forceinline__ int col_of(int ty, int j) {
  return (TN == 8 && j >= 4) ? 64 + ty * 4 + (j - 4) : ty * 4 + j;
}
__device__ __forceinline__ int row_of(int tx, int i) { return (i >= 4 ? 64 : 0) + tx * 4 + (i & 3); }

template <int TN>
__device__ __forceinline__ void load_w_chunk(float* __restrict__ Ws, const float* __restrict__ W, int K, int CO, int k0,
                                             int co0, bool vec) {
  constexpr int TC = TileCols<TN>::value;
  if (vec) {
    for (int i = threadIdx.x; i < KC * TC / 4; i += NTHR) {
      int kk = i / (TC / 4), c4 = (i % (TC / 4)) * 4;
      float* dst = Ws + kk * TC + c4;
      int k = k0 + kk, co = co0 + c4;
      if (k < K && co < CO) cp_async16(dst, W + (size_t)k * CO + co);
      else *reinterpret_cast<float4*>(dst) = make_float4(0.f, 0.f, 0.f, 0.f);
    }
  } else {
    for (int i = threadIdx.x; i < KC * TC; i += NTHR) {
      int kk = i / TC, c = i % TC;
      int k = k0 + kk, co = co0 + c;
      Ws[kk * TC + c] = (k < K && co < CO) ? __ldg(W + (size_t)k * CO + co) : 0.f;
    }
  }
}

__device__ __forceinline__ void load_x_chunk(float* __restrict__ Xs, const float* __restrict__ X, int K, int ld, int pm,
                                             int rows, int k0, int n0, bool vec) {
  if (!pm && vec) {
    for (int i = threadIdx.x; i < KC * TR / 4; i += NTHR) {
      int kk = i / (TR / 4), r4 = (i % (TR / 4)) * 4;
      float* dst = Xs + kk * TR + r4;
      int k = k0 + kk, n = n0 + r4;
      if (k < K && n < rows) cp_async16(dst, X + (size_t)k * ld + n);
      else *reinterpret_cast<float4*>(dst) = make_float4(0.f, 0.f, 0.f, 0.f);
    }
  } else if (!pm) {
    for (int i = threadIdx.x; i < KC * TR; i += NTHR) {
      int kk = i / TR, r = i % TR;
      int k = k0 + kk, n = n0 + r;
      Xs[kk * TR + r] = (k < K && n < rows) ? __ldg(X + (size_t)k * ld + n) : 0.f;
    }
  } else {
    for (int i = threadIdx.x; i < KC * TR; i += NTHR) {
      int r = i / KC, kk = i % KC;
      int k = k0 + kk, n = n0 + r;
      Xs[kk * TR + r] = (k < K && n < rows) ? __ldg(X + (size_t)n * ld + k) : 0.f;
    }
  }
}

__device__ __forceinline__ void load_x_chunk_packed(float* __restrict__ Xs, const float* __restrict__ X, long long bs, int K, int ld,
                                                    int rows, int k0, int b0, int B) {
  for (int i = threadIdx.x; i < KC * TR / 4; i += NTHR) {
    int kk = i / (TR / 4), r4 = (i % (TR / 4)) * 4;
    float* dst = Xs + kk * TR + r4;
    int k = k0 + kk, ob = b0 + r4 / rows, n = r4 % rows;
    if (k < K && ob < B) cp_async16(dst, X + (size_t)ob * bs + (size_t)k * ld + n);
    else *reinterpret_cast<float4*>(dst) = make_float4(0.f, 0.f, 0.f, 0.f);
  }
}

__device__ __forceinline__ bool aligned16(const void* p) { return (reinterpret_cast<uintptr_t>(p) & 15) == 0; }

template <int TN, bool PACK = false>
__global__ void __launch_bounds__(NTHR) cn_linear_kernel(const pcreid_linear_args a) {
  constexpr int TC = TileCols<TN>::value;
  __shared__ __align__(16) float Xs[2][KC * TR];
  __shared__ __align__(16) float Ws[2][KC * TC];
  const int b = PACK ? blockIdx.z * (TR / a.rows) : blockIdx.z, n0 = blockIdx.x * TR, co0 = blockIdx.y * TC;
  const int tx = threadIdx.x & 15, ty = threadIdx.x >> 4;
  if (PACK) {
    const float* W1 = a.W1;
    const float* W2 = a.K2 > 0 ? a.W2 : nullptr;
    const int nch1 = ceil_div(a.K1, KC), nch2 = a.K2 > 0 ? ceil_div(a.K2, KC) : 0, nch = nch1 + nch2;
    auto load = [&](int stage, int ch) {
      if (ch < nch1) {
        load_x_chunk_packed(Xs[stage], a.X1, a.x1_bs, a.K1, a.ldx1, a.rows, ch * KC, b, a.B);
        load_w_chunk<TN>(Ws[stage], W1, a.K1, a.CO, ch * KC, co0, true);
      } else {
        load_x_chunk_packed(Xs[stage], a.X2, a.x2_bs, a.K2, a.ldx2, a.rows, (ch - nch1) * KC, b, a.B);
        load_w_chunk<TN>(Ws[stage], W2, a.K2, a.CO, (ch - nch1) * KC, co0, true);
      }
    };
    float acc[8][TN];
#pragma unroll
    for (int i = 0; i < 8; ++i)
#pragma unroll
      for (int j = 0; j < TN; ++j) acc[i][j] = 0.f;
    load(0, 0);
    cp_async_commit();
    for (int ch = 0; ch < nch; ++ch) {
      if (ch + 1 < nch) load((ch + 1) & 1, ch + 1);
      cp_async_commit();
      cp_async_wait<1>();
      __syncthreads();
      fma_chunk<TN>(Xs[ch & 1], Ws[ch & 1], tx, ty, acc);
      __syncthreads();
    }
#pragma unroll
    for (int j = 0; j < TN; ++j) {
      const int co = co0 + col_of<TN>(ty, j);
      if (co >= a.CO) continue;
      const float bv = a.bias ? __ldg(a.bias + co) : 0.f;
#pragma unroll
      for (int h = 0; h < 2; ++h) {
        const int r = h * 64 + tx * 4, ob = b + r / a.rows, n = r % a.rows;
        if (ob >= a.B) continue;
        float4 rr = make_float4(0.f, 0.f, 0.f, 0.f);
        if (a.R) rr = *reinterpret_cast<const float4*>(a.R + (size_t)ob * a.r_bs + (size_t)co * a.ldr + n);
        const float rv[4] = {rr.x, rr.y, rr.z, rr.w};
        float v[4];
#pragma unroll
        for (int i = 0; i < 4; ++i) {
          float x = acc[h * 4 + i][j] + bv;
          if (a.R && !a.res_after_act) x += rv[i];
          x = apply_act(x, a.act);
          if (a.R && a.res_after_act) x += rv[i];
          v[i] = x;
        }
        *reinterpret_cast<float4*>(a.Y + (size_t)ob * a.y_bs + (size_t)co * a.ldy + n) = make_float4(v[0], v[1], v[2], v[3]);
      }
    }
    return;
  }

  const int xb1 = a.x1_map ? a.x1_map[b] : b;
  const float* X1 = a.X1 + (size_t)xb1 * a.x1_bs;
  const int wb1 = a.w1_map ? a.w1_map[b] : b;
  const float* W1 = a.W1 + (size_t)wb1 * a.w1_bs;
  const float* X2 = nullptr;
  const float* W2 = nullptr;
  if (a.K2 > 0) {
    const int xb2 = a.x2_map ? a.x2_map[b] : b;
    X2 = a.X2 + (size_t)xb2 * a.x2_bs;
    W2 = a.W2 + (size_t)b * a.w2_bs;
  }
  const bool vx1 = !a.x1_pm && (a.ldx1 % 4 == 0) && (a.rows % 4 == 0) && aligned16(X1);
  const bool vx2 = a.K2 > 0 && !a.x2_pm && (a.ldx2 % 4 == 0) && (a.rows % 4 == 0) && aligned16(X2);
  const bool vw1 = (a.CO % 4 == 0) && aligned16(W1);
  const bool vw2 = a.K2 > 0 && (a.CO % 4 == 0) && aligned16(W2);

  const int nch1 = ceil_div(a.K1, KC), nch2 = a.K2 > 0 ? ceil_div(a.K2, KC) : 0, nch = nch1 + nch2;
  auto load = [&](int stage, int ch) {
    if (ch < nch1) {
      load_x_chunk(Xs[stage], X1, a.K1, a.ldx1, a.x1_pm, a.rows, ch * KC, n0, vx1);
      load_w_chunk<TN>(Ws[stage], W1, a.K1, a.CO, ch * KC, co0, vw1);
    } else {
      load_x_chunk(Xs[stage], X2, a.K2, a.ldx2, a.x2_pm, a.rows, (ch - nch1) * KC, n0, vx2);
      load_w_chunk<TN>(Ws[stage], W2, a.K2, a.CO, (ch - nch1) * KC, co0, vw2);
    }
  };

  float acc[8][TN];
#pragma unroll
  for (int i = 0; i < 8; ++i)
#pragma unroll
    for (int j = 0; j < TN; ++j) acc[i][j] = 0.f;

  load(0, 0);
  cp_async_commit();
  for (int ch = 0; ch < nch; ++ch) {
    if (ch + 1 < nch) load((ch + 1) & 1, ch + 1);
    cp_async_commit();
    cp_async_wait<1>();
    __syncthreads();
    fma_chunk<TN>(Xs[ch & 1], Ws[ch & 1], tx, ty, acc);
    __syncthreads();
  }

  float* Y = a.Y + (size_t)b * a.y_bs;
  const float* R = nullptr;
  if (a.R) R = a.R + (size_t)(a.r_map ? a.r_map[b] : b) * a.r_bs;
  const bool vy = !a.y_pm && (a.ldy % 4 == 0) && (a.rows % 4 == 0) && aligned16(Y) && (!R || ((a.ldr % 4 == 0) && aligned16(R)));
  if (a.y_pm && !R && (a.ldy % 4 == 0) && (a.CO % 4 == 0) && aligned16(Y)) {
#pragma unroll
    for (int jb = 0; jb < TN; jb += 4) {
      const int co = co0 + col_of<TN>(ty, jb);
      if (co >= a.CO) continue;
      float bv[4];
#pragma unroll
      for (int j = 0; j < 4; ++j) bv[j] = a.bias ? __ldg(a.bias + co + j) : 0.f;
#pragma unroll
      for (int i = 0; i < 8; ++i) {
        const int n = n0 + (i >= 4 ? 64 : 0) + tx * 4 + (i & 3);
        if (n >= a.rows) continue;
        float4 v;
        v.x = apply_act(acc[i][jb + 0] + bv[0], a.act);
        v.y = apply_act(acc[i][jb + 1] + bv[1], a.act);
        v.z = apply_act(acc[i][jb + 2] + bv[2], a.act);
        v.w = apply_act(acc[i][jb + 3] + bv[3], a.act);
        *reinterpret_cast<float4*>(Y + (size_t)n * a.ldy + co) = v;
      }
    }
    return;
  }
#pragma unroll
  for (int j = 0; j < TN; ++j) {
    const int co = co0 + col_of<TN>(ty, j);
    if (co >= a.CO) continue;
    const float bv = a.bias ? __ldg(a.bias + co) : 0.f;
#pragma unroll
    for (int h = 0; h < 2; ++h) {
      const int n = n0 + h * 64 + tx * 4;
      if (n >= a.rows) continue;
      float v[4];
#pragma unroll
      for (int i = 0; i < 4; ++i) v[i] = acc[h * 4 + i][j] + bv;
      if (vy) {
        float4 r = make_float4(0.f, 0.f, 0.f, 0.f);
        if (R) r = *reinterpret_cast<const float4*>(R + (size_t)co * a.ldr + n);
        const float rr[4] = {r.x, r.y, r.z, r.w};
#pragma unroll
        for (int i = 0; i < 4; ++i) {
          if (R && !a.res_after_act) v[i] += rr[i];
          v[i] = apply_act(v[i], a.act);
          if (R && a.res_after_act) v[i] += rr[i];
        }
        *reinterpret_cast<float4*>(Y + (size_t)co * a.ldy + n) = make_float4(v[0], v[1], v[2], v[3]);
      } else {
#pragma unroll
        for (int i = 0; i < 4; ++i) {
          if (n + i >= a.rows) break;
          float x = v[i];
          float r = R ? R[(size_t)co * a.ldr + n + i] : 0.f;
          if (R && !a.res_after_act) x += r;
          x = apply_act(x, a.act);
          if (R && a.res_after_act) x += r;
          if (a.y_pm) Y[(size_t)(n + i) * a.ldy + co] = x;
          else Y[(size_t)co * a.ldy + n + i] = x;
        }
      }
    }
  }
}

template <int CG>
__global__ void __launch_bounds__(128) cn_groupnorm_kernel(const pcreid_norm_args a) {
  const long long idx = (long long)blockIdx.x * blockDim.x + threadIdx.x;
  if (idx >= (long long)a.B * a.rows) return;
  const int b = (int)(idx / a.rows), n = (int)(idx % a.rows);
  const float* X = a.X + (size_t)b * a.x_bs + n;
  const float* R = a.R ? a.R + (size_t)(a.r_map ? a.r_map[b] : b) * a.r_bs + n : nullptr;
  float* Y = a.Y + (size_t)b * a.y_bs + n;
  const int cg = CG > 0 ? CG : a.C / a.G;
  for (int g = 0; g < a.G; ++g) {
    if (CG > 0) {
      float x[CG > 0 ? CG : 1];
#pragma unroll
      for (int i = 0; i < CG; ++i) x[i] = X[(size_t)(g * CG + i) * a.ldx];
      float s = 0.f;
#pragma unroll
      for (int i = 0; i < CG; ++i) s += x[i];
      const float mean = s / (float)CG;
      float v = 0.f;
#pragma unroll
      for (int i = 0; i < CG; ++i) { const float d = x[i] - mean; v = fmaf(d, d, v); }
      const float rstd = rsqrtf(v / (float)CG + 1e-5f);
#pragma unroll
      for (int i = 0; i < CG; ++i) {
        const int c = g * CG + i;
        float y = (x[i] - mean) * rstd * __ldg(a.gamma + c) + __ldg(a.beta + c);
        if (R) y += R[(size_t)c * a.ldr];
        Y[(size_t)c * a.ldy] = apply_act(y, a.act);
      }
      continue;
    }
    float s = 0.f;
    for (int c = g * cg; c < (g + 1) * cg; ++c) s += X[(size_t)c * a.ldx];
    const float mean = s / (float)cg;
    float v = 0.f;
    for (int c = g * cg; c < (g + 1) * cg; ++c) {
      float d = X[(size_t)c * a.ldx] - mean;
      v = fmaf(d, d, v);
    }
    const float rstd = rsqrtf(v / (float)cg + 1e-5f);
    for (int c = g * cg; c < (g + 1) * cg; ++c) {
      float y = (X[(size_t)c * a.ldx] - mean) * rstd * __ldg(a.gamma + c) + __ldg(a.beta + c);
      if (R) y += R[(size_t)c * a.ldr];
      Y[(size_t)c * a.ldy] = apply_act(y, a.act);
    }
  }
}

template <int CG>
__global__ void __launch_bounds__(128) gn_res_relu_dot_kernel(int rows, int C, int G, const float* __restrict__ X, int ldx,
                                                              const float* __restrict__ gamma, const float* __restrict__ beta,
                                                              const float* __restrict__ R, int ldr, const float* __restrict__ w,
                                                              float bias, float* __restrict__ out) {
  const int n = blockIdx.x * blockDim.x + threadIdx.x;
  if (n >= rows) return;
  const int cg = CG > 0 ? CG : C / G;
  float acc = 0.f;
  for (int g = 0; g < G; ++g) {
    if (CG > 0) {
      float x[CG > 0 ? CG : 1];
#pragma unroll
      for (int i = 0; i < CG; ++i) x[i] = X[(size_t)(g * CG + i) * ldx + n];
      float s = 0.f;
#pragma unroll
      for (int i = 0; i < CG; ++i) s += x[i];
      const float mean = s / (float)CG;
      float v = 0.f;
#pragma unroll
      for (int i = 0; i < CG; ++i) { const float d = x[i] - mean; v = fmaf(d, d, v); }
      const float rstd = rsqrtf(v / (float)CG + 1e-5f);
#pragma unroll
      for (int i = 0; i < CG; ++i) {
        const int c = g * CG + i;
        const float y = (x[i] - mean) * rstd * __ldg(gamma + c) + __ldg(beta + c) + R[(size_t)c * ldr + n];
        acc = fmaf(fmaxf(y, 0.f), __ldg(w + c), acc);
      }
      continue;
    }
    float s = 0.f;
    for (int c = g * cg; c < (g + 1) * cg; ++c) s += X[(size_t)c * ldx + n];
    const float mean = s / (float)cg;
    float v = 0.f;
    for (int c = g * cg; c < (g + 1) * cg; ++c) { const float d = X[(size_t)c * ldx + n] - mean; v = fmaf(d, d, v); }
    const float rstd = rsqrtf(v / (float)cg + 1e-5f);
    for (int c = g * cg; c < (g + 1) * cg; ++c) {
      const float y = (X[(size_t)c * ldx + n] - mean) * rstd * __ldg(gamma + c) + __ldg(beta + c) + R[(size_t)c * ldr + n];
      acc = fmaf(fmaxf(y, 0.f), __ldg(w + c), acc);
    }
  }
  out[n] = acc + bias;
}

constexpr int KV_SC_DEFAULT = 128;
template <int KV_SC>
__global__ void __launch_bounds__(256) linattn_kv_kernel(int S, int d, int H, const float* __restrict__ K, long long k_bs,
                                                         int ldk, const float* __restrict__ V, long long v_bs, int ldv,
                                                         float* __restrict__ Wkv, float* __restrict__ ksum) {
  extern __shared__ float sm[];
  const int D = d / H, h = blockIdx.x, b = blockIdx.y, e0 = blockIdx.z * 4096;
  float* Ks = sm;
  float* Vs = sm + D * (KV_SC + 1);
  const float* Kb = K + (size_t)b * k_bs + (size_t)h * D * ldk;
  const float* Vb = V + (size_t)b * v_bs + (size_t)h * D * ldv;
  const int nout = D * D;
  float acc[16];
#pragma unroll
  for (int o = 0; o < 16; ++o) acc[o] = 0.f;
  float ks = 0.f;
  const float invS = (float)S;
  for (int s0 = 0; s0 < S; s0 += KV_SC) {
    const int sc = min(KV_SC, S - s0);
    for (int i = threadIdx.x; i < D * KV_SC; i += blockDim.x) {
      int c = i / KV_SC, s = i % KV_SC;
      float kv = 0.f, vv = 0.f;
      if (s < sc) {
        kv = apply_act(Kb[(size_t)c * ldk + s0 + s], ACT_ELU1);
        vv = Vb[(size_t)c * ldv + s0 + s] / invS;
      }
      Ks[c * (KV_SC + 1) + s] = kv;
      Vs[c * (KV_SC + 1) + s] = vv;
    }
    __syncthreads();
#pragma unroll
    for (int o = 0; o < 16; ++o) {
      int e = e0 + threadIdx.x + o * 256;
      if (e < nout) {
        const float* kr = Ks + (e / D) * (KV_SC + 1);
        const float* vr = Vs + (e % D) * (KV_SC + 1);
        float s = acc[o];
        for (int t = 0; t < sc; ++t) s = fmaf(kr[t], vr[t], s);
        acc[o] = s;
      }
    }
    if (blockIdx.z == 0 && threadIdx.x < D) {
      const float* kr = Ks + threadIdx.x * (KV_SC + 1);
      for (int t = 0; t < sc; ++t) ks += kr[t];
    }
    __syncthreads();
  }
  float* Wb = Wkv + (size_t)b * d * d;
#pragma unroll
  for (int o = 0; o < 16; ++o) {
    int e = e0 + threadIdx.x + o * 256;
    if (e < nout) Wb[(size_t)(h * D + e / D) * d + h * D + (e % D)] = acc[o];
  }
  if (blockIdx.z == 0 && threadIdx.x < D) ksum[(size_t)b * d + h * D + threadIdx.x] = ks;
}

__global__ void __launch_bounds__(128) linattn_scale_kernel(int rows, int d, int H, int S, const float* __restrict__ Q,
                                                            long long q_bs, int ldq, const int* __restrict__ q_map,
                                                            const float* __restrict__ ksum, const int* __restrict__ ksum_map,
                                                            float* __restrict__ Qs, long long qs_bs, int ldqs) {
  const int n = blockIdx.x * blockDim.x + threadIdx.x, b = blockIdx.y;
  if (n >= rows) return;
  const float* q = Q + (size_t)(q_map ? q_map[b] : b) * q_bs + n;
  const float* ks = ksum + (size_t)(ksum_map ? ksum_map[b] : b) * d;
  float* o = Qs + (size_t)b * qs_bs + n;
  const int D = d / H;
  for (int h = 0; h < H; ++h) {
    float dot = 0.f;
    for (int c = h * D; c < (h + 1) * D; ++c) dot = fmaf(apply_act(q[(size_t)c * ldq], ACT_ELU1), __ldg(ks + c), dot);
    const float z = (1.f / (dot + 1e-6f)) * (float)S;
    for (int c = h * D; c < (h + 1) * D; ++c) o[(size_t)c * ldqs] = apply_act(q[(size_t)c * ldq], ACT_ELU1) * z;
  }
}

template <int CPL>
__global__ void __launch_bounds__(256) local_linattn_kernel(long long rows, int N, int C, int H, int knum, const float* __restrict__ qkv,
                                                            const int* __restrict__ idx, float* __restrict__ out) {
  const long long r = (long long)blockIdx.x * 8 + (threadIdx.x >> 5);
  const int lane = threadIdx.x & 31;
  if (r >= rows) return;
  const long long b = r / N;
  const float* base = qkv + (size_t)b * N * 3 * C;
  const float* qrow = qkv + (size_t)r * 3 * C + lane * CPL;
  const int lph = 32 / H;
  float qf[CPL], acc[CPL];
#pragma unroll
  for (int i = 0; i < CPL; ++i) { qf[i] = apply_act(qrow[i], ACT_ELU1); acc[i] = 0.f; }
  float wsum = 0.f;
  const int* ir = idx + (size_t)r * knum;
  for (int j = 0; j < knum; ++j) {
    const float* nrow = base + (size_t)__ldg(ir + j) * 3 * C + lane * CPL;
    float w = 0.f;
#pragma unroll
    for (int i = 0; i < CPL; ++i) w = fmaf(qf[i], apply_act(__ldg(nrow + C + i), ACT_ELU1), w);
    for (int o = lph >> 1; o > 0; o >>= 1) w += __shfl_xor_sync(FULL_MASK, w, o);
    wsum += w;
#pragma unroll
    for (int i = 0; i < CPL; ++i) acc[i] = fmaf(w, __ldg(nrow + 2 * C + i), acc[i]);
  }
  const float z = 1.f / (wsum + 1e-6f);
  float* o = out + (size_t)r * C + lane * CPL;
#pragma unroll
  for (int i = 0; i < CPL; ++i) o[i] = acc[i] * z;
}

__global__ void __launch_bounds__(256) edge_build_kernel(int C, int N, int S, int k, const float* __restrict__ P1,
                                                         const float* __restrict__ Cc, const int* __restrict__ idx,
                                                         float* __restrict__ out) {
  const int e = blockIdx.x * blockDim.x + threadIdx.x, b = blockIdx.z;
  const int E = S * k;
  if (e >= E) return;
  const int s = e / k, src = idx[(size_t)b * E + e];
  const int c0 = blockIdx.y * 16;
#pragma unroll 4
  for (int c = c0; c < min(c0 + 16, C); ++c)
    out[((size_t)b * C + c) * E + e] = fmaxf(__ldg(P1 + ((size_t)b * C + c) * N + src) + __ldg(Cc + ((size_t)b * C + c) * S + s), 0.f);
}

__global__ void __launch_bounds__(256) seg_max_kernel(long long rows, int k, const float* __restrict__ x, float* __restrict__ out) {
  const long long i = (long long)blockIdx.x * blockDim.x + threadIdx.x;
  if (i >= rows) return;
  const float* r = x + i * k;
  float mx = r[0];
  for (int j = 1; j < k; ++j) mx = fmaxf(mx, r[j]);
  out[i] = mx;
}

__global__ void __launch_bounds__(256) seg_mean_kernel(long long rows, int k, const float* __restrict__ x, float* __restrict__ out) {
  const long long i = (long long)blockIdx.x * blockDim.x + threadIdx.x;
  if (i >= rows) return;
  const float* r = x + i * k;
  float s = r[0];
  for (int j = 1; j < k; ++j) s += r[j];
  out[i] = s / (float)k;
}

__global__ void __launch_bounds__(256) cn_pool_kernel(int B, int C, int rows1, const float* __restrict__ X1, long long x1_bs,
                                                      int ldx1, int rows2, const float* __restrict__ X2, long long x2_bs,
                                                      int ldx2, int mode, float* __restrict__ out, long long ob, long long oc) {
  const int w = blockIdx.x * (blockDim.x >> 5) + (threadIdx.x >> 5), lane = threadIdx.x & 31;
  if (w >= B * C) return;
  const int b = w / C, c = w % C;
  float mx = -INFINITY, sm = 0.f;
  const float* r1 = X1 + (size_t)b * x1_bs + (size_t)c * ldx1;
  for (int n = lane; n < rows1; n += 32) { float v = r1[n]; mx = fmaxf(mx, v); sm += v; }
  if (X2) {
    const float* r2 = X2 + (size_t)b * x2_bs + (size_t)c * ldx2;
    for (int n = lane; n < rows2; n += 32) { float v = r2[n]; mx = fmaxf(mx, v); sm += v; }
  }
  mx = warp_max(mx);
  sm = warp_sum(sm);
  if (lane == 0) {
    out[(size_t)b * ob + (size_t)c * oc] = mx;
    if (mode == 0) out[(size_t)b * ob + (size_t)(C + c) * oc] = sm / (float)(rows1 + (X2 ? rows2 : 0));
  }
}

__global__ void __launch_bounds__(128) cn_chanmax_kernel(int C, int rows, const float* __restrict__ X, long long x_bs, int ldx,
                                                         float* __restrict__ out, long long ob, long long on) {
  const int n = blockIdx.x * blockDim.x + threadIdx.x, b = blockIdx.y;
  if (n >= rows) return;
  const float* x = X + (size_t)b * x_bs + n;
  float mx = -INFINITY;
  for (int c = 0; c < C; ++c) mx = fmaxf(mx, x[(size_t)c * ldx]);
  out[(size_t)b * ob + (size_t)n * on] = mx;
}

template <int TN>
__global__ void __launch_bounds__(NTHR) sa_edge_mlp_kernel(int C, int N, int S, int k, int cpt, const float* __restrict__ P1,
                                                           const float* __restrict__ Cc, const int* __restrict__ idx,
                                                           const float* __restrict__ W2, const float* __restrict__ b2,
                                                           const float* __restrict__ W3, const float* __restrict__ b3,
                                                           float* __restrict__ out) {
  constexpr int TC = TileCols<TN>::value;
  extern __shared__ __align__(16) float smf[];
  float* A = smf;
  float* Bm = A + (size_t)C * TR;
  float* Ws = Bm + (size_t)C * TR;
  const int b = blockIdx.y, s0 = blockIdx.x * cpt;
  const int ncen = min(cpt, S - s0), nedge = ncen * k;
  const int tx = threadIdx.x & 15, ty = threadIdx.x >> 4;
  const float* Pb = P1 + (size_t)b * C * N;
  const float* Cb = Cc + (size_t)b * C * S;

  {
    const int e = threadIdx.x & (TR - 1);
    int src = -1, cen = 0;
    if (e < nedge) { cen = s0 + e / k; src = idx[((size_t)b * S + cen) * k + (e % k)]; }
    for (int c = threadIdx.x / TR; c < C; c += NTHR / TR) {
      float v = 0.f;
      if (src >= 0) v = fmaxf(__ldg(Pb + (size_t)c * N + src) + __ldg(Cb + (size_t)c * S + cen), 0.f);
      A[c * TR + e] = v;
    }
  }
  const bool vw = (C % 4 == 0) && aligned16(W2) && aligned16(W3);
  const int nch = ceil_div(C, KC);
  for (int layer = 0; layer < 2; ++layer) {
    const float* W = layer == 0 ? W2 : W3;
    const float* bias = layer == 0 ? b2 : b3;
    const float* Xin = layer == 0 ? A : Bm;
    float* Xout = layer == 0 ? Bm : A;
    for (int co0 = 0; co0 < C; co0 += TC) {
      float acc[8][TN];
#pragma unroll
      for (int i = 0; i < 8; ++i)
#pragma unroll
        for (int j = 0; j < TN; ++j) acc[i][j] = 0.f;
      __syncthreads();
      load_w_chunk<TN>(Ws, W, C, C, 0, co0, vw);
      cp_async_commit();
      for (int ch = 0; ch < nch; ++ch) {
        if (ch + 1 < nch) load_w_chunk<TN>(Ws + ((ch + 1) & 1) * KC * TC, W, C, C, (ch + 1) * KC, co0, vw);
        cp_async_commit();
        cp_async_wait<1>();
        __syncthreads();
        fma_chunk<TN>(Xin + (size_t)ch * KC * TR, Ws + (ch & 1) * KC * TC, tx, ty, acc);
        __syncthreads();
      }
#pragma unroll
      for (int j = 0; j < TN; ++j) {
        const int co = co0 + col_of<TN>(ty, j);
        if (co >= C) continue;
        const float bv = __ldg(bias + co);
#pragma unroll
        for (int h = 0; h < 2; ++h) {
          float4 v;
          v.x = fmaxf(acc[h * 4 + 0][j] + bv, 0.f);
          v.y = fmaxf(acc[h * 4 + 1][j] + bv, 0.f);
          v.z = fmaxf(acc[h * 4 + 2][j] + bv, 0.f);
          v.w = fmaxf(acc[h * 4 + 3][j] + bv, 0.f);
          *reinterpret_cast<float4*>(Xout + (size_t)co * TR + h * 64 + tx * 4) = v;
        }
      }
    }
  }
  __syncthreads();
  for (int i = threadIdx.x; i < C * ncen; i += NTHR) {
    const int c = i / ncen, cl = i % ncen;
    const float* r = A + (size_t)c * TR + cl * k;
    float mx = r[0];
    for (int j = 1; j < k; ++j) mx = fmaxf(mx, r[j]);
    out[((size_t)b * C + c) * S + s0 + cl] = mx;
  }
}

__global__ void __launch_bounds__(256) edge_gather_max_kernel(int C, int N, int k, const float* __restrict__ P,
                                                              const float* __restrict__ Q, const int* __restrict__ idx,
                                                              int act, float* __restrict__ out, long long o_bs, int ldo) {
  extern __shared__ int sidx[];
  const int b = blockIdx.y, i0 = blockIdx.x * 128;
  const int ni = min(128, N - i0);
  for (int t = threadIdx.x; t < ni * k; t += blockDim.x) sidx[t] = idx[((size_t)b * N + i0) * k + t];
  __syncthreads();
  const int il = threadIdx.x & 127;
  if (il >= ni) return;
  const int* id = sidx + il * k;
  for (int c = threadIdx.x >> 7; c < C; c += 2) {
    const float* row = P + ((size_t)b * C + c) * N;
    float mx = -INFINITY;
    for (int j = 0; j < k; ++j) mx = fmaxf(mx, __ldg(row + id[j]));
    out[(size_t)b * o_bs + (size_t)c * ldo + i0 + il] = apply_act(mx + Q[((size_t)b * C + c) * N + i0 + il], act);
  }
}

constexpr int PH_DT = 32;
template <int HD, int CG>
__global__ void __launch_bounds__(256) pair_concat_head_kernel(int T, int D, int E, const float* __restrict__ A,
                                                               const float* __restrict__ Bv, const float* __restrict__ Et,
                                                               const float* __restrict__ Ed, const float* __restrict__ W2,
                                                               const float* __restrict__ g1, const float* __restrict__ be1,
                                                               const float* __restrict__ g2, const float* __restrict__ be2,
                                                               const float* __restrict__ w, float b0,
                                                               const unsigned char* __restrict__ mask, float* __restrict__ out) {
  constexpr int CPW = HD / 8;
  static_assert(CPW % CG == 0 && CPW % 4 == 0, "groups must not straddle warps");
  __shared__ float H1[HD][PH_DT + 1];
  __shared__ float red[8][PH_DT];
  const int t = blockIdx.y, d0 = blockIdx.x * PH_DT;
  const int lane = threadIdx.x & 31, wq = threadIdx.x >> 5;
  const int d = d0 + lane;
  const bool valid = d < D;
  float x[CPW];
#pragma unroll
  for (int i = 0; i < CPW; ++i) {
    const int c = wq * CPW + i;
    x[i] = valid ? __ldg(A + (size_t)t * HD + c) + __ldg(Bv + (size_t)d * HD + c) : 0.f;
  }
#pragma unroll
  for (int g0 = 0; g0 < CPW; g0 += CG) {
    float s = 0.f;
#pragma unroll
    for (int i = 0; i < CG; ++i) s += x[g0 + i];
    const float mean = s / (float)CG;
    float v = 0.f;
#pragma unroll
    for (int i = 0; i < CG; ++i) { float dd = x[g0 + i] - mean; v = fmaf(dd, dd, v); }
    const float rstd = rsqrtf(v / (float)CG + 1e-5f);
#pragma unroll
    for (int i = 0; i < CG; ++i) {
      const int c = wq * CPW + g0 + i;
      x[g0 + i] = fmaxf((x[g0 + i] - mean) * rstd * __ldg(g1 + c) + __ldg(be1 + c), 0.f);
    }
  }
#pragma unroll
  for (int i = 0; i < CPW; ++i) H1[wq * CPW + i][lane] = x[i];
  __syncthreads();
  float y[CPW];
#pragma unroll
  for (int i = 0; i < CPW; ++i) y[i] = 0.f;
  for (int kk = 0; kk < HD; ++kk) {
    const float hv = H1[kk][lane];
    const float4* wr = reinterpret_cast<const float4*>(W2 + (size_t)kk * HD + wq * CPW);
#pragma unroll
    for (int i = 0; i < CPW / 4; ++i) {
      const float4 w4 = __ldg(wr + i);
      y[4 * i + 0] = fmaf(hv, w4.x, y[4 * i + 0]);
      y[4 * i + 1] = fmaf(hv, w4.y, y[4 * i + 1]);
      y[4 * i + 2] = fmaf(hv, w4.z, y[4 * i + 2]);
      y[4 * i + 3] = fmaf(hv, w4.w, y[4 * i + 3]);
    }
  }
  float part = 0.f;
#pragma unroll
  for (int g0 = 0; g0 < CPW; g0 += CG) {
    float s = 0.f;
#pragma unroll
    for (int i = 0; i < CG; ++i) s += y[g0 + i];
    const float mean = s / (float)CG;
    float v = 0.f;
#pragma unroll
    for (int i = 0; i < CG; ++i) { float dd = y[g0 + i] - mean; v = fmaf(dd, dd, v); }
    const float rstd = rsqrtf(v / (float)CG + 1e-5f);
#pragma unroll
    for (int i = 0; i < CG; ++i) {
      const int c = wq * CPW + g0 + i;
      float r = 0.f;
      if (valid) r = c < E ? __ldg(Et + (size_t)t * E + c) : __ldg(Ed + (size_t)d * E + (c - E));
      const float o = fmaxf((y[g0 + i] - mean) * rstd * __ldg(g2 + c) + __ldg(be2 + c) + r, 0.f);
      part = fmaf(o, __ldg(w + c), part);
    }
  }
  red[wq][lane] = part;
  __syncthreads();
  if (wq == 0 && valid) {
    float s = b0;
#pragma unroll
    for (int i = 0; i < 8; ++i) s += red[i][lane];
    if (mask && !mask[(size_t)t * D + d]) s = 0.f;
    out[(size_t)t * D + d] = s;
  }
}

}

extern "C" {

int pcreid_abi_version(void) { return 1; }

int pcreid_cn_linear(const pcreid_linear_args* p, void* stream) {
  if (!p) return PCREID_ERR_ARG;
  pcreid_linear_args a = *p;
  if (a.B <= 0 || a.rows <= 0 || a.CO <= 0) return PCREID_OK;
  if (a.K1 <= 0 || !a.X1 || !a.W1 || !a.Y) return PCREID_ERR_ARG;
  if (a.K2 > 0 && (!a.X2 || !a.W2)) return PCREID_ERR_ARG;
  if (a.B > 65535 * 32) return PCREID_ERR_UNSUPPORTED;
  cudaStream_t st = (cudaStream_t)stream;
  const int zmax = 65535;
  for (int b0 = 0; b0 < a.B; b0 += zmax) {
    pcreid_linear_args s = a;
    s.B = (a.B - b0 < zmax) ? a.B - b0 : zmax;
    if (b0) {
      if (s.x1_map) s.x1_map += b0; else s.X1 += (size_t)b0 * s.x1_bs;
      if (s.K2 > 0) { if (s.x2_map) s.x2_map += b0; else s.X2 += (size_t)b0 * s.x2_bs; s.W2 += (size_t)b0 * s.w2_bs; }
      if (s.w1_map) s.w1_map += b0; else s.W1 += (size_t)b0 * s.w1_bs;
      if (s.R) { if (s.r_map) s.r_map += b0; else s.R += (size_t)b0 * s.r_bs; }
      s.Y += (size_t)b0 * s.y_bs;
    }
    auto a16 = [](const void* q) { return (reinterpret_cast<uintptr_t>(q) & 15) == 0; };
    const bool pack = s.rows < TR && TR % s.rows == 0 && s.rows % 4 == 0 && s.B > 1 && !s.x1_map && !s.x2_map && !s.w1_map && !s.r_map &&
                      !s.x1_pm && !s.x2_pm && !s.y_pm && s.w1_bs == 0 && (s.K2 == 0 || s.w2_bs == 0) && s.CO % 4 == 0 &&
                      a16(s.X1) && s.ldx1 % 4 == 0 && s.x1_bs % 4 == 0 && a16(s.W1) && a16(s.Y) && s.ldy % 4 == 0 && s.y_bs % 4 == 0 &&
                      (s.K2 == 0 || (a16(s.X2) && s.ldx2 % 4 == 0 && s.x2_bs % 4 == 0 && a16(s.W2))) &&
                      (!s.R || (a16(s.R) && s.ldr % 4 == 0 && s.r_bs % 4 == 0));
    if (pack) {
      const int nz = ceil_div(s.B, TR / s.rows);
      if (a.CO > 64) cn_linear_kernel<8, true><<<dim3(1, ceil_div(a.CO, 128), nz), NTHR, 0, st>>>(s);
      else cn_linear_kernel<4, true><<<dim3(1, 1, nz), NTHR, 0, st>>>(s);
    } else if (a.CO > 64) {
      dim3 grid(ceil_div(a.rows, TR), ceil_div(a.CO, 128), s.B);
      cn_linear_kernel<8><<<grid, NTHR, 0, st>>>(s);
    } else {
      dim3 grid(ceil_div(a.rows, TR), 1, s.B);
      cn_linear_kernel<4><<<grid, NTHR, 0, st>>>(s);
    }
  }
  return pcreid_launch_status();
}

int pcreid_cn_groupnorm(const pcreid_norm_args* p, void* stream) {
  if (!p) return PCREID_ERR_ARG;
  pcreid_norm_args a = *p;
  if (a.B <= 0 || a.rows <= 0 || a.C <= 0) return PCREID_OK;
  if (!a.X || !a.Y || !a.gamma || !a.beta || a.G <= 0 || a.C % a.G) return PCREID_ERR_ARG;
  cudaStream_t st = (cudaStream_t)stream;
  const int ymax = 65535;
  for (int b0 = 0; b0 < a.B; b0 += ymax) {
    pcreid_norm_args s = a;
    s.B = (a.B - b0 < ymax) ? a.B - b0 : ymax;
    s.X += (size_t)b0 * s.x_bs;
    s.Y += (size_t)b0 * s.y_bs;
    if (s.R) { if (s.r_map) s.r_map += b0; else s.R += (size_t)b0 * s.r_bs; }
    const unsigned grid = (unsigned)(((long long)s.B * a.rows + 127) / 128);
    switch (a.C / a.G) {
      case 4: cn_groupnorm_kernel<4><<<grid, 128, 0, st>>>(s); break;
      case 8: cn_groupnorm_kernel<8><<<grid, 128, 0, st>>>(s); break;
      case 16: cn_groupnorm_kernel<16><<<grid, 128, 0, st>>>(s); break;
      case 32: cn_groupnorm_kernel<32><<<grid, 128, 0, st>>>(s); break;
      case 64: cn_groupnorm_kernel<64><<<grid, 128, 0, st>>>(s); break;
      case 128: cn_groupnorm_kernel<128><<<grid, 128, 0, st>>>(s); break;
      default: cn_groupnorm_kernel<0><<<grid, 128, 0, st>>>(s); break;
    }
  }
  return pcreid_launch_status();
}

int pcreid_gn_res_relu_dot(int rows, int C, int G, const float* X, int ldx, const float* gamma, const float* beta, const float* R,
                           int ldr, const float* w, float bias, float* out, void* stream) {
  if (rows <= 0) return PCREID_OK;
  if (!X || !gamma || !beta || !R || !w || !out || C <= 0 || G <= 0 || C % G) return PCREID_ERR_ARG;
  cudaStream_t st = (cudaStream_t)stream;
  const unsigned grid = (unsigned)((rows + 127) / 128);
  switch (C / G) {
    case 8: gn_res_relu_dot_kernel<8><<<grid, 128, 0, st>>>(rows, C, G, X, ldx, gamma, beta, R, ldr, w, bias, out); break;
    case 16: gn_res_relu_dot_kernel<16><<<grid, 128, 0, st>>>(rows, C, G, X, ldx, gamma, beta, R, ldr, w, bias, out); break;
    case 32: gn_res_relu_dot_kernel<32><<<grid, 128, 0, st>>>(rows, C, G, X, ldx, gamma, beta, R, ldr, w, bias, out); break;
    default: gn_res_relu_dot_kernel<0><<<grid, 128, 0, st>>>(rows, C, G, X, ldx, gamma, beta, R, ldr, w, bias, out); break;
  }
  return pcreid_launch_status();
}

int pcreid_linattn_kv(int B, int S, int d, int H, const float* K, long long k_bs, int ldk, const float* V, long long v_bs,
                      int ldv, float* Wkv, float* ksum, void* stream) {
  if (B <= 0) return PCREID_OK;
  if (!K || !V || !Wkv || !ksum || S <= 0 || H <= 0 || d % H) return PCREID_ERR_ARG;
  const int D = d / H;
  if (D > 256) return PCREID_ERR_UNSUPPORTED;
  cudaStream_t st = (cudaStream_t)stream;
  cudaMemsetAsync(Wkv, 0, (size_t)B * d * d * sizeof(float), st);
  const int nz = ceil_div(D * D, 4096);
  for (int b0 = 0; b0 < B; b0 += 65535) {
    int nb = B - b0 < 65535 ? B - b0 : 65535;
    if (D <= 64) {
      size_t smem = (size_t)2 * D * (KV_SC_DEFAULT + 1) * sizeof(float);
      if (smem > 48 * 1024) cudaFuncSetAttribute(linattn_kv_kernel<KV_SC_DEFAULT>, cudaFuncAttributeMaxDynamicSharedMemorySize, (int)smem);
      linattn_kv_kernel<KV_SC_DEFAULT><<<dim3(H, nb, nz), 256, smem, st>>>(S, d, H, K + (size_t)b0 * k_bs, k_bs, ldk, V + (size_t)b0 * v_bs,
                                                                       v_bs, ldv, Wkv + (size_t)b0 * d * d, ksum + (size_t)b0 * d);
    } else {
      size_t smem = (size_t)2 * D * (32 + 1) * sizeof(float);
      if (smem > 48 * 1024) cudaFuncSetAttribute(linattn_kv_kernel<32>, cudaFuncAttributeMaxDynamicSharedMemorySize, (int)smem);
      linattn_kv_kernel<32><<<dim3(H, nb, nz), 256, smem, st>>>(S, d, H, K + (size_t)b0 * k_bs, k_bs, ldk, V + (size_t)b0 * v_bs, v_bs, ldv,
                                                                Wkv + (size_t)b0 * d * d, ksum + (size_t)b0 * d);
    }
  }
  return pcreid_launch_status();
}

int pcreid_linattn_scale(int B, int rows, int d, int H, int S, const float* Q, long long q_bs, int ldq, const int* q_map,
                         const float* ksum, const int* ksum_map, float* Qs, long long qs_bs, int ldqs, void* stream) {
  if (B <= 0 || rows <= 0) return PCREID_OK;
  if (!Q || !ksum || !Qs || H <= 0 || d % H) return PCREID_ERR_ARG;
  cudaStream_t st = (cudaStream_t)stream;
  for (int b0 = 0; b0 < B; b0 += 65535) {
    int nb = B - b0 < 65535 ? B - b0 : 65535;
    linattn_scale_kernel<<<dim3(ceil_div(rows, 128), nb), 128, 0, st>>>(
        rows, d, H, S, q_map ? Q : Q + (size_t)b0 * q_bs, q_bs, ldq, q_map ? q_map + b0 : nullptr,
        ksum_map ? ksum : ksum + (size_t)b0 * d, ksum_map ? ksum_map + b0 : nullptr, Qs + (size_t)b0 * qs_bs, qs_bs, ldqs);
  }
  return pcreid_launch_status();
}

int pcreid_local_linattn(int B, int N, int C, int H, int knum, const float* qkv, const int* idx, float* out, void* stream) {
  if (B <= 0 || N <= 0) return PCREID_OK;
  if (!qkv || !idx || !out || knum <= 0 || H <= 0) return PCREID_ERR_ARG;
  if (C % 32 || C > 128 || (H != 1 && H != 2 && H != 4) || C % H) return PCREID_ERR_UNSUPPORTED;
  const long long rows = (long long)B * N;
  const unsigned grid = (unsigned)((rows + 7) / 8);
  cudaStream_t st = (cudaStream_t)stream;
  switch (C / 32) {
    case 1: local_linattn_kernel<1><<<grid, 256, 0, st>>>(rows, N, C, H, knum, qkv, idx, out); break;
    case 2: local_linattn_kernel<2><<<grid, 256, 0, st>>>(rows, N, C, H, knum, qkv, idx, out); break;
    case 3: local_linattn_kernel<3><<<grid, 256, 0, st>>>(rows, N, C, H, knum, qkv, idx, out); break;
    default: local_linattn_kernel<4><<<grid, 256, 0, st>>>(rows, N, C, H, knum, qkv, idx, out); break;
  }
  return pcreid_launch_status();
}

int pcreid_cn_pool(int B, int C, int rows1, const float* X1, long long x1_bs, int ldx1, int rows2, const float* X2,
                   long long x2_bs, int ldx2, int mode, float* out, long long ob, long long oc, void* stream) {
  if (B <= 0 || C <= 0) return PCREID_OK;
  if (!X1 || !out || rows1 <= 0) return PCREID_ERR_ARG;
  long long nw = (long long)B * C;
  cn_pool_kernel<<<(unsigned)((nw + 7) / 8), 256, 0, (cudaStream_t)stream>>>(B, C, rows1, X1, x1_bs, ldx1, rows2, X2, x2_bs,
                                                                             ldx2, mode, out, ob, oc);
  return pcreid_launch_status();
}

int pcreid_cn_chanmax(int B, int C, int rows, const float* X, long long x_bs, int ldx, float* out, long long ob, long long on,
                      void* stream) {
  if (B <= 0 || rows <= 0) return PCREID_OK;
  if (!X || !out || C <= 0) return PCREID_ERR_ARG;
  cudaStream_t st = (cudaStream_t)stream;
  for (int b0 = 0; b0 < B; b0 += 65535) {
    int nb = B - b0 < 65535 ? B - b0 : 65535;
    cn_chanmax_kernel<<<dim3(ceil_div(rows, 128), nb), 128, 0, st>>>(C, rows, X + (size_t)b0 * x_bs, x_bs, ldx,
                                                                     out + (size_t)b0 * ob, ob, on);
  }
  return pcreid_launch_status();
}

int pcreid_sa_edge_mlp(int B, int C, int N, int S, int k, const float* P1, const float* Cc, const int* idx, const float* W2,
                       const float* b2, const float* W3, const float* b3, float* out, void* stream) {
  if (B <= 0 || S <= 0) return PCREID_OK;
  if (!P1 || !Cc || !idx || !W2 || !b2 || !W3 || !b3 || !out || k <= 0 || N <= 0) return PCREID_ERR_ARG;
  if (k > TR || C > 128 || C % 16) return PCREID_ERR_UNSUPPORTED;
  cudaStream_t st = (cudaStream_t)stream;
  const int cpt = TR / k;
  if (B > 65535) return PCREID_ERR_UNSUPPORTED;
  dim3 grid(ceil_div(S, cpt), B);
  if (C > 64) {
    size_t smem = ((size_t)2 * C * TR + 2 * KC * 128) * sizeof(float);
    cudaFuncSetAttribute(sa_edge_mlp_kernel<8>, cudaFuncAttributeMaxDynamicSharedMemorySize, (int)smem);
    sa_edge_mlp_kernel<8><<<grid, NTHR, smem, st>>>(C, N, S, k, cpt, P1, Cc, idx, W2, b2, W3, b3, out);
  } else {
    size_t smem = ((size_t)2 * C * TR + 2 * KC * 64) * sizeof(float);
    cudaFuncSetAttribute(sa_edge_mlp_kernel<4>, cudaFuncAttributeMaxDynamicSharedMemorySize, (int)smem);
    sa_edge_mlp_kernel<4><<<grid, NTHR, smem, st>>>(C, N, S, k, cpt, P1, Cc, idx, W2, b2, W3, b3, out);
  }
  return pcreid_launch_status();
}

int pcreid_edge_build(int B, int C, int N, int S, int k, const float* P1, const float* Cc, const int* idx, float* out, void* stream) {
  if (B <= 0 || S <= 0) return PCREID_OK;
  if (!P1 || !Cc || !idx || !out || C <= 0 || k <= 0 || N <= 0) return PCREID_ERR_ARG;
  if (B > 65535 || ceil_div(C, 16) > 65535) return PCREID_ERR_UNSUPPORTED;
  edge_build_kernel<<<dim3(ceil_div(S * k, 256), ceil_div(C, 16), B), 256, 0, (cudaStream_t)stream>>>(C, N, S, k, P1, Cc, idx, out);
  return pcreid_launch_status();
}

int pcreid_seg_max(long long rows, int k, const float* x, float* out, void* stream) {
  if (rows <= 0) return PCREID_OK;
  if (!x || !out || k <= 0) return PCREID_ERR_ARG;
  seg_max_kernel<<<(unsigned)((rows + 255) / 256), 256, 0, (cudaStream_t)stream>>>(rows, k, x, out);
  return pcreid_launch_status();
}

int pcreid_seg_mean(long long rows, int k, const float* x, float* out, void* stream) {
  if (rows <= 0) return PCREID_OK;
  if (!x || !out || k <= 0) return PCREID_ERR_ARG;
  seg_mean_kernel<<<(unsigned)((rows + 255) / 256), 256, 0, (cudaStream_t)stream>>>(rows, k, x, out);
  return pcreid_launch_status();
}

int pcreid_edge_gather_max(int B, int C, int N, int k, const float* P, const float* Q, const int* idx, int act, float* out,
                           long long o_bs, int ldo, void* stream) {
  if (B <= 0 || N <= 0) return PCREID_OK;
  if (!P || !Q || !idx || !out || C <= 0 || k <= 0) return PCREID_ERR_ARG;
  if (B > 65535 || (size_t)128 * k * 4 > 48 * 1024) return PCREID_ERR_UNSUPPORTED;
  edge_gather_max_kernel<<<dim3(ceil_div(N, 128), B), 256, (size_t)128 * k * sizeof(int), (cudaStream_t)stream>>>(
      C, N, k, P, Q, idx, act, out, o_bs, ldo);
  return pcreid_launch_status();
}

int pcreid_pair_concat_head(int T, int D, int E, int G, const float* A, const float* Bv, const float* Et, const float* Ed,
                            const float* W2, const float* g1, const float* be1, const float* g2, const float* be2,
                            const float* w, float b0, const unsigned char* mask, float* out, void* stream) {
  if (T <= 0 || D <= 0) return PCREID_OK;
  if (!A || !Bv || !Et || !Ed || !W2 || !g1 || !be1 || !g2 || !be2 || !w || !out) return PCREID_ERR_ARG;
  const int HD = 2 * E;
  if (G <= 0 || HD % G) return PCREID_ERR_ARG;
  const int cg = HD / G;
  if (T > 65535) return PCREID_ERR_UNSUPPORTED;
  dim3 grid(ceil_div(D, PH_DT), T);
  cudaStream_t st = (cudaStream_t)stream;
  if ((reinterpret_cast<uintptr_t>(W2) & 15) != 0) return PCREID_ERR_ARG;
  if (HD == 256 && cg == 8)
    pair_concat_head_kernel<256, 8><<<grid, 256, 0, st>>>(T, D, E, A, Bv, Et, Ed, W2, g1, be1, g2, be2, w, b0, mask, out);
  else if (HD == 256 && cg == 16)
    pair_concat_head_kernel<256, 16><<<grid, 256, 0, st>>>(T, D, E, A, Bv, Et, Ed, W2, g1, be1, g2, be2, w, b0, mask, out);
  else if (HD == 128 && cg == 8)
    pair_concat_head_kernel<128, 8><<<grid, 256, 0, st>>>(T, D, E, A, Bv, Et, Ed, W2, g1, be1, g2, be2, w, b0, mask, out);
  else if (HD == 128 && cg == 16)
    pair_concat_head_kernel<128, 16><<<grid, 256, 0, st>>>(T, D, E, A, Bv, Et, Ed, W2, g1, be1, g2, be2, w, b0, mask, out);
  else
    return PCREID_ERR_UNSUPPORTED;
  return pcreid_launch_status();
}

}
```

point-cloud-reid_b200/csrc/tc_common.cuh:

```cuda
#pragma once
#include <cuda_bf16.h>
#include <cuda_runtime.h>
#include <stdint.h>

namespace tc {

__device__ __forceinline__ uint32_t smem_u32(const void* p) { return (uint32_t)__cvta_generic_to_shared(p); }

__device__ __forceinline__ void mbar_init(uint64_t* bar, uint32_t count) {
  asm volatile("mbarrier.init.shared::cta.b64 [%0], %1;" ::"r"(smem_u32(bar)), "r"(count) : "memory");
}
__device__ __forceinline__ void fence_mbar_init() { asm volatile("fence.mbarrier_init.release.cluster;" ::: "memory"); }
__device__ __forceinline__ void mbar_wait(uint64_t* bar, uint32_t parity) {
  uint32_t ok;
  const uint32_t a = smem_u32(bar);
  do {
    asm volatile(
        "{\n\t.reg .pred p;\n\t"
        "mbarrier.try_wait.parity.shared::cta.b64 p, [%1], %2;\n\t"
        "selp.u32 %0, 1, 0, p;\n\t}\n"
        : "=r"(ok)
        : "r"(a), "r"(parity)
        : "memory");
  } while (!ok);
}

__device__ __forceinline__ void fence_async_smem() { asm volatile("fence.proxy.async.shared::cta;" ::: "memory"); }
__device__ __forceinline__ void tc_fence_before() { asm volatile("tcgen05.fence::before_thread_sync;" ::: "memory"); }
__device__ __forceinline__ void tc_fence_after() { asm volatile("tcgen05.fence::after_thread_sync;" ::: "memory"); }

__device__ __forceinline__ void tmem_alloc(uint32_t* smem_dst, uint32_t ncols) {
  asm volatile("tcgen05.alloc.cta_group::1.sync.aligned.shared::cta.b32 [%0], %1;" ::"r"(smem_u32(smem_dst)), "r"(ncols)
               : "memory");
}
__device__ __forceinline__ void tmem_relinquish() {
  asm volatile("tcgen05.relinquish_alloc_permit.cta_group::1.sync.aligned;" ::: "memory");
}
__device__ __forceinline__ void tmem_dealloc(uint32_t taddr, uint32_t ncols) {
  asm volatile("tcgen05.dealloc.cta_group::1.sync.aligned.b32 %0, %1;" ::"r"(taddr), "r"(ncols) : "memory");
}

enum { LAYOUT_NONE = 0, LAYOUT_SW128_BASE32B = 1, LAYOUT_SW128 = 2, LAYOUT_SW64 = 4, LAYOUT_SW32 = 6 };
__device__ __forceinline__ uint64_t smem_desc(uint32_t saddr, uint32_t lbo_bytes, uint32_t sbo_bytes, uint32_t layout) {
  uint64_t d = 0;
  d |= (uint64_t)((saddr >> 4) & 0x3fff);
  d |= (uint64_t)((lbo_bytes >> 4) & 0x3fff) << 16;
  d |= (uint64_t)((sbo_bytes >> 4) & 0x3fff) << 32;
  d |= (uint64_t)1 << 46;
  d |= (uint64_t)(layout & 7) << 61;
  return d;
}
enum { FMT_F16 = 0, FMT_BF16 = 1, FMT_TF32 = 2 };
enum { MAJOR_K = 0, MAJOR_MN = 1 };
__host__ __device__ constexpr uint32_t instr_desc(int M, int N, int fmt, int a_major, int b_major) {
  return (1u << 4) | ((uint32_t)fmt << 7) | ((uint32_t)fmt << 10) | ((uint32_t)a_major << 15) | ((uint32_t)b_major << 16) |
         ((uint32_t)(N >> 3) << 17) | ((uint32_t)(M >> 4) << 24);
}

__device__ __forceinline__ void umma_f16(uint32_t tmem_d, uint64_t adesc, uint64_t bdesc, uint32_t idesc, uint32_t accumulate) {
  asm volatile(
      "{\n\t.reg .pred p;\n\t"
      "setp.ne.b32 p, %4, 0;\n\t"
      "tcgen05.mma.cta_group::1.kind::f16 [%0], %1, %2, %3, p;\n\t}\n" ::"r"(tmem_d),
      "l"(adesc), "l"(bdesc), "r"(idesc), "r"(accumulate)
      : "memory");
}
__device__ __forceinline__ void umma_tf32(uint32_t tmem_d, uint64_t adesc, uint64_t bdesc, uint32_t idesc, uint32_t accumulate) {
  asm volatile(
      "{\n\t.reg .pred p;\n\t"
      "setp.ne.b32 p, %4, 0;\n\t"
      "tcgen05.mma.cta_group::1.kind::tf32 [%0], %1, %2, %3, p;\n\t}\n" ::"r"(tmem_d),
      "l"(adesc), "l"(bdesc), "r"(idesc), "r"(accumulate)
      : "memory");
}
__device__ __forceinline__ void umma_f16_ts(uint32_t tmem_d, uint32_t tmem_a, uint64_t bdesc, uint32_t idesc, uint32_t accumulate) {
  asm volatile(
      "{\n\t.reg .pred p;\n\t"
      "setp.ne.b32 p, %4, 0;\n\t"
      "tcgen05.mma.cta_group::1.kind::f16 [%0], [%1], %2, %3, p;\n\t}\n" ::"r"(tmem_d),
      "r"(tmem_a), "l"(bdesc), "r"(idesc), "r"(accumulate)
      : "memory");
}
__device__ __forceinline__ void umma_tf32_ts(uint32_t tmem_d, uint32_t tmem_a, uint64_t bdesc, uint32_t idesc, uint32_t accumulate) {
  asm volatile(
      "{\n\t.reg .pred p;\n\t"
      "setp.ne.b32 p, %4, 0;\n\t"
      "tcgen05.mma.cta_group::1.kind::tf32 [%0], [%1], %2, %3, p;\n\t}\n" ::"r"(tmem_d),
      "r"(tmem_a), "l"(bdesc), "r"(idesc), "r"(accumulate)
      : "memory");
}
__device__ __forceinline__ void umma_commit(uint64_t* bar) {
  asm volatile("tcgen05.commit.cta_group::1.mbarrier::arrive::one.shared::cluster.b64 [%0];" ::"r"(smem_u32(bar)) : "memory");
}

__device__ __forceinline__ void tmem_ld8(uint32_t taddr, uint32_t (&r)[8]) {
  asm volatile("tcgen05.ld.sync.aligned.32x32b.x8.b32 {%0,%1,%2,%3,%4,%5,%6,%7}, [%8];"
               : "=r"(r[0]), "=r"(r[1]), "=r"(r[2]), "=r"(r[3]), "=r"(r[4]), "=r"(r[5]), "=r"(r[6]), "=r"(r[7])
               : "r"(taddr));
}
__device__ __forceinline__ void tmem_ld16(uint32_t taddr, uint32_t (&r)[16]) {
  asm volatile(
      "tcgen05.ld.sync.aligned.32x32b.x16.b32 {%0,%1,%2,%3,%4,%5,%6,%7,%8,%9,%10,%11,%12,%13,%14,%15}, [%16];"
      : "=r"(r[0]), "=r"(r[1]), "=r"(r[2]), "=r"(r[3]), "=r"(r[4]), "=r"(r[5]), "=r"(r[6]), "=r"(r[7]), "=r"(r[8]), "=r"(r[9]),
        "=r"(r[10]), "=r"(r[11]), "=r"(r[12]), "=r"(r[13]), "=r"(r[14]), "=r"(r[15])
      : "r"(taddr));
}
__device__ __forceinline__ void tmem_ld32(uint32_t taddr, uint32_t (&r)[32]) {
#pragma unroll
  for (int q = 0; q < 4; ++q)
    asm volatile("tcgen05.ld.sync.aligned.32x32b.x8.b32 {%0,%1,%2,%3,%4,%5,%6,%7}, [%8];"
                 : "=r"(r[8 * q]), "=r"(r[8 * q + 1]), "=r"(r[8 * q + 2]), "=r"(r[8 * q + 3]), "=r"(r[8 * q + 4]), "=r"(r[8 * q + 5]),
                   "=r"(r[8 * q + 6]), "=r"(r[8 * q + 7])
                 : "r"(taddr + 8 * q));
}
__device__ __forceinline__ void tmem_ld_wait() { asm volatile("tcgen05.wait::ld.sync.aligned;" ::: "memory"); }
__device__ __forceinline__ void tmem_st8(uint32_t taddr, const uint32_t (&r)[8]) {
  asm volatile("tcgen05.st.sync.aligned.32x32b.x8.b32 [%0], {%1,%2,%3,%4,%5,%6,%7,%8};" ::"r"(taddr), "r"(r[0]), "r"(r[1]),
               "r"(r[2]), "r"(r[3]), "r"(r[4]), "r"(r[5]), "r"(r[6]), "r"(r[7])
               : "memory");
}
__device__ __forceinline__ void tmem_st16(uint32_t taddr, const uint32_t (&r)[16]) {
  asm volatile("tcgen05.st.sync.aligned.32x32b.x16.b32 [%0], {%1,%2,%3,%4,%5,%6,%7,%8,%9,%10,%11,%12,%13,%14,%15,%16};" ::"r"(taddr),
               "r"(r[0]), "r"(r[1]), "r"(r[2]), "r"(r[3]), "r"(r[4]), "r"(r[5]), "r"(r[6]), "r"(r[7]), "r"(r[8]), "r"(r[9]), "r"(r[10]),
               "r"(r[11]), "r"(r[12]), "r"(r[13]), "r"(r[14]), "r"(r[15])
               : "memory");
}
__device__ __forceinline__ void tmem_st32(uint32_t taddr, const uint32_t (&r)[32]) {
  asm volatile(
      "tcgen05.st.sync.aligned.32x32b.x32.b32 [%0], "
      "{%1,%2,%3,%4,%5,%6,%7,%8,%9,%10,%11,%12,%13,%14,%15,%16,%17,%18,%19,%20,%21,%22,%23,%24,%25,%26,%27,%28,%29,%30,%31,%32};" ::"r"(taddr),
      "r"(r[0]), "r"(r[1]), "r"(r[2]), "r"(r[3]), "r"(r[4]), "r"(r[5]), "r"(r[6]), "r"(r[7]), "r"(r[8]), "r"(r[9]), "r"(r[10]),
      "r"(r[11]), "r"(r[12]), "r"(r[13]), "r"(r[14]), "r"(r[15]), "r"(r[16]), "r"(r[17]), "r"(r[18]), "r"(r[19]), "r"(r[20]),
      "r"(r[21]), "r"(r[22]), "r"(r[23]), "r"(r[24]), "r"(r[25]), "r"(r[26]), "r"(r[27]), "r"(r[28]), "r"(r[29]), "r"(r[30]),
      "r"(r[31])
      : "memory");
}
__device__ __forceinline__ void tmem_st_wait() { asm volatile("tcgen05.wait::st.sync.aligned;" ::: "memory"); }

__device__ __forceinline__ uint32_t pack_bf16(float lo, float hi) {
  __nv_bfloat162 v = __floats2bfloat162_rn(lo, hi);
  return *reinterpret_cast<uint32_t*>(&v);
}

__device__ __forceinline__ uint32_t bf2_add(uint32_t a, uint32_t b) { uint32_t r; asm("add.rn.bf16x2 %0, %1, %2;" : "=r"(r) : "r"(a), "r"(b)); return r; }
__device__ __forceinline__ uint32_t bf2_mul(uint32_t a, uint32_t b) { uint32_t r; asm("mul.rn.bf16x2 %0, %1, %2;" : "=r"(r) : "r"(a), "r"(b)); return r; }
__device__ __forceinline__ uint32_t bf2_max(uint32_t a, uint32_t b) { uint32_t r; asm("max.bf16x2 %0, %1, %2;" : "=r"(r) : "r"(a), "r"(b)); return r; }
__device__ __forceinline__ uint32_t bf2_min(uint32_t a, uint32_t b) { uint32_t r; asm("min.bf16x2 %0, %1, %2;" : "=r"(r) : "r"(a), "r"(b)); return r; }
__device__ __forceinline__ uint32_t bf2_ex2(uint32_t a) { uint32_t r; asm("ex2.approx.ftz.bf16x2 %0, %1;" : "=r"(r) : "r"(a)); return r; }
__device__ __forceinline__ uint32_t bf2_elu1(uint32_t x) {
  const uint32_t LOG2E = 0x3fb93fb9u;
  return bf2_add(bf2_max(x, 0u), bf2_ex2(bf2_mul(bf2_min(x, 0u), LOG2E)));
}

__device__ __forceinline__ uint32_t bf2_fma(uint32_t a, uint32_t b, uint32_t c) { uint32_t r; asm("fma.rn.bf16x2 %0, %1, %2, %3;" : "=r"(r) : "r"(a), "r"(b), "r"(c)); return r; }
__device__ __forceinline__ uint32_t bf2_fma_relu(uint32_t a, uint32_t b, uint32_t c) { uint32_t r; asm("fma.rn.relu.bf16x2 %0, %1, %2, %3;" : "=r"(r) : "r"(a), "r"(b), "r"(c)); return r; }
__device__ __forceinline__ uint32_t pack_bf16_relu(float lo, float hi) { uint32_t r; asm("cvt.rn.relu.bf16x2.f32 %0, %1, %2;" : "=r"(r) : "f"(hi), "f"(lo)); return r; }
__device__ __forceinline__ uint32_t bf2_elu1s(uint32_t x) {
  const uint32_t LN2B = 0x3f313f31u;
  return bf2_fma(bf2_max(x, 0u), LN2B, bf2_ex2(bf2_min(x, 0u)));
}

struct OpBF16 {
  static constexpr int FMT = FMT_BF16;
  static constexpr uint32_t ONE_LO = 0x00003f80u;
  static constexpr bool PACKED_MATH = true;
  static __device__ __forceinline__ uint32_t pack(float lo, float hi) { return pack_bf16(lo, hi); }
  static __device__ __forceinline__ uint32_t pack_relu(float lo, float hi) { return pack_bf16_relu(lo, hi); }
  static __device__ __forceinline__ float lo(uint32_t w) { return __uint_as_float(w << 16); }
  static __device__ __forceinline__ float hi(uint32_t w) { return __uint_as_float(w & 0xffff0000u); }
  static __device__ __forceinline__ uint32_t add_relu(float a, float b, uint32_t side) {
    return bf2_fma_relu(pack_bf16(a, b), 0x3f803f80u, side);
  }
  static __device__ __forceinline__ uint32_t add(float a, float b, uint32_t side) { return bf2_add(pack_bf16(a, b), side); }
  static __device__ __forceinline__ uint32_t elu1_scaled(float a, float b) { return bf2_elu1s(pack_bf16(a, b)); }
  static __device__ __forceinline__ uint32_t elu1(float a, float b) { return bf2_elu1(pack_bf16(a, b)); }
};
__device__ __forceinline__ uint32_t h2_add(uint32_t a, uint32_t b) { uint32_t r; asm("add.rn.f16x2 %0, %1, %2;" : "=r"(r) : "r"(a), "r"(b)); return r; }
__device__ __forceinline__ uint32_t h2_mul(uint32_t a, uint32_t b) { uint32_t r; asm("mul.rn.f16x2 %0, %1, %2;" : "=r"(r) : "r"(a), "r"(b)); return r; }
__device__ __forceinline__ uint32_t h2_max(uint32_t a, uint32_t b) { uint32_t r; asm("max.f16x2 %0, %1, %2;" : "=r"(r) : "r"(a), "r"(b)); return r; }
__device__ __forceinline__ uint32_t h2_min(uint32_t a, uint32_t b) { uint32_t r; asm("min.f16x2 %0, %1, %2;" : "=r"(r) : "r"(a), "r"(b)); return r; }
__device__ __forceinline__ uint32_t h2_ex2(uint32_t a) { uint32_t r; asm("ex2.approx.f16x2 %0, %1;" : "=r"(r) : "r"(a)); return r; }
__device__ __forceinline__ uint32_t h2_fma(uint32_t a, uint32_t b, uint32_t c) { uint32_t r; asm("fma.rn.f16x2 %0, %1, %2, %3;" : "=r"(r) : "r"(a), "r"(b), "r"(c)); return r; }

struct OpF16 {
  static constexpr int FMT = FMT_F16;
  static constexpr uint32_t ONE_LO = 0x00003c00u;
#ifdef PCREID_F16_PACKED
  static constexpr bool PACKED_MATH = true;
#else
  static constexpr bool PACKED_MATH = false;
#endif
  static __device__ __forceinline__ uint32_t pack(float lo, float hi) {
    uint32_t r; asm("cvt.rn.satfinite.f16x2.f32 %0, %1, %2;" : "=r"(r) : "f"(hi), "f"(lo)); return r;
  }
  static __device__ __forceinline__ uint32_t pack_relu(float lo, float hi) {
    uint32_t r; asm("cvt.rn.relu.satfinite.f16x2.f32 %0, %1, %2;" : "=r"(r) : "f"(hi), "f"(lo)); return r;
  }
  static __device__ __forceinline__ float lo(uint32_t w) {
    float f; asm("{\n\t.reg .b16 l, h;\n\tmov.b32 {l, h}, %1;\n\tcvt.f32.f16 %0, l;\n\t}\n" : "=f"(f) : "r"(w)); return f;
  }
  static __device__ __forceinline__ float hi(uint32_t w) {
    float f; asm("{\n\t.reg .b16 l, h;\n\tmov.b32 {l, h}, %1;\n\tcvt.f32.f16 %0, h;\n\t}\n" : "=f"(f) : "r"(w)); return f;
  }
  static __device__ __forceinline__ uint32_t add_relu(float a, float b, uint32_t side) { return pack_relu(a + lo(side), b + hi(side)); }
#ifdef PCREID_F16_PACKED
  static __device__ __forceinline__ uint32_t add(float a, float b, uint32_t side) { return h2_add(pack(a, b), side); }
#else
  static __device__ __forceinline__ uint32_t add(float a, float b, uint32_t side) { return pack(a + lo(side), b + hi(side)); }
#endif
  static __device__ __forceinline__ float elu1s_f(float x) {
    float e; asm("ex2.approx.ftz.f32 %0, %1;" : "=f"(e) : "f"(fminf(x, 0.f)));
    return fmaf(fmaxf(x, 0.f), 0.69314718056f, e);
  }
#ifdef PCREID_F16_PACKED
  static __device__ __forceinline__ uint32_t elu1_scaled(float a, float b) {
    const uint32_t x = pack(a, b);
    return h2_fma(h2_max(x, 0u), 0x398c398cu, h2_ex2(h2_min(x, 0u)));
  }
#else
  static __device__ __forceinline__ uint32_t elu1_scaled(float a, float b) { return pack(elu1s_f(a), elu1s_f(b)); }
#endif
  static __device__ __forceinline__ float elu1_f(float x) {
    float e; asm("ex2.approx.ftz.f32 %0, %1;" : "=f"(e) : "f"(fminf(x, 0.f) * 1.4426950408889634f));
    return fmaxf(x, 0.f) + e;
  }
#ifdef PCREID_F16_PACKED
  static __device__ __forceinline__ uint32_t elu1(float a, float b) {
    const uint32_t x = pack(a, b);
    return h2_add(h2_max(x, 0u), h2_ex2(h2_mul(h2_min(x, 0u), 0x3dc53dc5u)));
  }
#else
  static __device__ __forceinline__ uint32_t elu1(float a, float b) { return pack(elu1_f(a), elu1_f(b)); }
#endif
};

__device__ __forceinline__ float tf32_rna(float x) {
  uint32_t r;
  asm("cvt.rna.tf32.f32 %0, %1;" : "=r"(r) : "f"(x));
  return __uint_as_float(r);
}
__device__ __forceinline__ float4 tf32_rna4(float4 v) { return make_float4(tf32_rna(v.x), tf32_rna(v.y), tf32_rna(v.z), tf32_rna(v.w)); }

__device__ __forceinline__ uint32_t uniform(uint32_t v) { return __shfl_sync(0xffffffffu, v, 0); }
__device__ __forceinline__ bool elect_one() {
  uint32_t pred;
  asm volatile("{\n\t.reg .pred P;\n\telect.sync _|P, 0xffffffff;\n\tselp.u32 %0, 1, 0, P;\n\t}\n" : "=r"(pred));
  return pred != 0;
}

__device__ __forceinline__ void bar_sync(int id, int nthreads) { asm volatile("bar.sync %0, %1;" ::"r"(id), "r"(nthreads) : "memory"); }

}
```

point-cloud-reid_b200/models/fused_pairs.py:

```python
import math
import os

import torch

from .. import kernels as K
from .. import torch_ops as _T
from ._packing import kmajor

IMG = 16384
B7_BYTES = int(os.environ.get("PCREID_B7_BYTES", 10240))
FMT_BF16, FMT_F16 = 0, 1
LN2H = 0.693359375
LN2B = 0.69140625
ATT_EPS = 1e-6


def _center_out(w):
    w = w.detach().float()
    return w - w.mean(0, keepdim=True)


_OPS = _T.ops


def _w_image(w, dtype):
    N, Kd = w.shape
    return w.detach().to(dtype).view(N, Kd // 8, 8).permute(1, 0, 2).contiguous().view(torch.uint8).flatten()


def _f32_bytes(*ts):
    return torch.cat([t.detach().float().flatten() for t in ts]).contiguous().view(torch.uint8)


def supported(model, n_points):
    X1, X2 = model.cross_stage1, model.cross_stage2
    return (model.match_type == 'xcorr_eff' and model.combine == 'point-cat' and model.pool_type == 'both'
            and X1 is not None and X2 is not None and X1.q_proj.weight.shape == (64, 64) and X1.nhead == 2
            and X2.q_proj.weight.shape == (64, 64) and X2.nhead == 2 and n_points >= 1)


class ObjectPack:
    __slots__ = ("n", "npts", "fmt", "QF1", "H", "PV", "MK1")


class FusedXcorr:
    def __init__(self, model, fmt=FMT_BF16):
        self.model = model
        self.fmt = fmt
        self.dtype = torch.float16 if fmt == FMT_F16 else torch.bfloat16
        self._key = None
        self.n_ctas = None
        self._n_ctas_dev = None
        self.timing = None
        self._units = {}

    def _weights(self):
        X1, X2 = self.model.cross_stage1, self.model.cross_stage2
        key = tuple((t.data_ptr(), t._version) for t in list(X1.parameters()) + list(X2.parameters()))
        if key != self._key:
            with torch.no_grad():
                d, dt = 64, self.dtype
                f = lambda t: t.detach().float()
                W0_1, W0_2 = f(X1.mlp[0].weight), f(X2.mlp[0].weight)
                self._b2_1 = f(X1.norm2.bias).contiguous()
                W0ext1 = torch.zeros((2 * d, 2 * d + 16), device=W0_1.device)
                W0ext1[:, :d] = W0_1[:, d:] * f(X1.norm1.weight)[None, :]
                W0ext1[:, d:2 * d] = W0_1[:, :d]
                W0ext1[:, 2 * d] = W0_1[:, d:] @ f(X1.norm1.bias) - W0_1[:, :d] @ self._b2_1
                self._w1a2 = torch.cat([
                    _w_image(W0ext1, dt), _w_image(_center_out(X1.mlp[2].weight), dt), _f32_bytes(X1.norm2.weight)]).contiguous()
                self._merge1c = kmajor(_center_out(X1.merge.weight))
                self._w1b2 = torch.cat([
                    _w_image(torch.cat([X2.k_proj.weight, X2.v_proj.weight], 0), dt),
                    _w_image(_center_out(X2.merge.weight), dt)]).contiguous()
                W0ext = torch.zeros((2 * d, 2 * d + 16), device=W0_2.device)
                W0ext[:, :d] = W0_2[:, :d]
                W0ext[:, d:2 * d] = W0_2[:, d:] * f(X2.norm1.weight)[None, :]
                W0ext[:, 2 * d] = W0_2[:, d:] @ f(X2.norm1.bias)
                ln2 = (LN2H if os.environ.get("PCREID_F16_PACKED") == "1" else math.log(2.0)) if self.fmt == FMT_F16 else LN2B
                self._w2y = torch.cat([
                    _w_image(f(X2.q_proj.weight) / ln2, dt), _w_image(W0ext, dt), _w_image(_center_out(X2.mlp[2].weight), dt),
                    _f32_bytes(X2.norm2.weight)]).contiguous()
                self._b2_2 = f(X2.norm2.bias).contiguous()
                assert self._w1a2.numel() == 53504 and self._w2y.numel() == 61696 and self._w1b2.numel() == 24576
            self._key = key

    def _tick(self):
        if self.timing is None:
            return None
        e = torch.cuda.Event(enable_timing=True)
        e.record()
        return e

    def _tock(self, name, e0, units):
        if e0 is not None:
            e1 = torch.cuda.Event(enable_timing=True)
            e1.record()
            self.timing.append((name, e0, e1, units))

    def _pack_image(self, x, act=K.ACT_NONE):
        B, C, N = x.shape
        out = torch.empty((B, (N + 127) // 128, C // 8, 128, 16), device=x.device, dtype=torch.uint8)
        _OPS.pack_image(B, C, N, x, x.stride(0), x.stride(1), act, self.fmt, out)
        return out

    def kv_scale(self, npts):
        return 1.0 / npts if self.fmt == FMT_F16 else 1.0

    def prepare(self, h, xyz):
        X1, X2 = self.model.cross_stage1, self.model.cross_stage2
        pk1, pk2 = X1.packed(), X2.packed()
        self._weights()
        B, C, N = h.shape
        o = ObjectPack()
        o.n, o.npts, o.fmt = B, N, self.fmt
        o.QF1 = self._pack_image(K.cn_linear(h, pk1["q"]), K.ACT_ELU1)
        o.H = torch.empty((B, (N + 127) // 128, C // 8, 128, 16), device=h.device, dtype=torch.uint8)
        _OPS.pack_image_bias(B, C, N, h, h.stride(0), h.stride(1), self._b2_1, self.fmt, o.H)
        pos2 = X2.position_code(xyz)
        if pos2 is None:
            o.PV = torch.zeros((B, (N + 127) // 128, C // 8, 128, 16), device=h.device, dtype=torch.uint8)
        else:
            o.PV = self._pack_image(K.cn_linear(pos2, pk2["v"]))
        wkv, ksum = X1.template_summary(h, X1.position_code(xyz))
        M = K.cn_linear(wkv, self._merge1c, x1_pm=True, y_pm=True)
        sc = self.kv_scale(N)
        M.mul_(float(N) * sc)
        if sc != 1.0:
            ksum = ksum * sc
        o.MK1 = torch.empty((B, B7_BYTES), device=h.device, dtype=torch.uint8)
        _OPS.pack_b7(B, M, ksum, self.fmt, o.MK1)
        return o

    def _dense_units(self, dev, r0, nrows, Dn, by_search, b_by_search):
        key = (str(dev), r0, nrows, Dn, by_search, b_by_search)
        capturing = torch.cuda.is_current_stream_capturing()
        hit = None if capturing else self._units.get(key)
        if hit is not None:
            return hit
        P = nrows * Dn
        u = torch.arange(P, device=dev, dtype=torch.int32)
        t_of, d_of = r0 + u % nrows, u // nrows
        c = lambda *xs: tuple(x.contiguous() for x in xs)
        lists_s = (c(r0 + u // Dn, u % Dn, u),
                   c(u // nrows, r0 + u % nrows, (u % nrows) * Dn + u // nrows))
        lists_t = (c(t_of, d_of, (t_of - r0) * Dn + d_of),
                   c(u % Dn, r0 + u // Dn, u))
        out = (lists_s if by_search else lists_t, lists_s if b_by_search else lists_t)
        if not capturing:
            if len(self._units) >= 64:
                self._units.pop(next(iter(self._units)))
            self._units[key] = out
        return out

    def match(self, pt, pd, ti, dj, debug=None, dense=None):
        assert pt.npts == pd.npts, "fused matcher expects equal point counts on both sides"
        assert pt.fmt == self.fmt and pd.fmt == self.fmt, "object packs were prepared for another operand format"
        self._weights()
        dev = pt.H.device
        if self.n_ctas is None or self._n_ctas_dev != dev:
            self.n_ctas, self._n_ctas_dev = torch.cuda.get_device_properties(dev).multi_processor_count, dev
        by_search = False
        b_by_search = os.environ.get("PCREID_P1B_ORDER", "search") == "search"
        if dense is not None:
            r0, nrows, Dn = dense
            P = nrows * Dn
            unit_lists, unit_lists_b = self._dense_units(dev, r0, nrows, Dn, by_search, b_by_search)
        else:
            P = ti.numel()
            ti, dj = ti.long(), dj.long()
            unit_lists = None
        NT, N = (pt.npts + 127) // 128, pt.npts
        A = torch.empty((P, 2, NT, IMG), device=dev, dtype=torch.uint8)
        B7 = torch.empty((P, 2, B7_BYTES), device=dev, dtype=torch.uint8)
        part = torch.empty((P, 2, 128), device=dev, dtype=torch.float32)
        sc = self.kv_scale(N)
        for role, (srch, tmpl, ps, pm) in enumerate(((ti, dj, pt, pd), (dj, ti, pd, pt))):
            if unit_lists is not None:
                us, ut, sl = unit_lists[role]
                bs, bt, bl = unit_lists_b[role]
            else:
                order = torch.argsort(tmpl, stable=True)
                us, ut, sl = srch[order].int().contiguous(), tmpl[order].int().contiguous(), order.int().contiguous()
                bs, bt, bl = us, ut, sl
                if b_by_search:
                    order = torch.argsort(srch, stable=True)
                    bs, bt, bl = srch[order].int().contiguous(), tmpl[order].int().contiguous(), order.int().contiguous()
            e0 = self._tick()
            _OPS.pair_p1a2(P, N, role, self.fmt, ATT_EPS * sc, us, ut, sl, ps.QF1, ps.H, pm.MK1, self._w1a2, A, self.n_ctas)
            self._tock("pair_p1a2_kernel", e0, P)
            e0 = self._tick()
            _OPS.pair_p1b_n(P, N, role, self.fmt, sc, bs, bt, bl, ps.PV, self._w1b2, A, B7, self.n_ctas)
            self._tock("pair_p1b_kernel" if os.environ.get("PCREID_P1B") == "1" else "pair_p1b2_kernel", e0, P)
        slots = torch.arange(P, device=dev, dtype=torch.int32)
        pooled = torch.empty((1, 128, P), device=dev, dtype=torch.float32)
        for role in (0, 1):
            e0 = self._tick()
            _OPS.pair_p2y(P, N, role, self.fmt, ATT_EPS * sc, slots, A, B7, self._w2y, part, self.n_ctas)
            self._tock("pair_p2y_kernel", e0, P)
        _OPS.pool_finish2(P, N, part, self._b2_2, pooled)
        if debug is not None:
            debug.update(A=A, B7=B7, part=part, pooled=pooled)
        return self.model._head_cn(pooled)


def decode_image(img, dtype=torch.bfloat16):
    x = img.contiguous().view(dtype).float().transpose(-1, -2)
    return x.reshape(*x.shape[:-3], x.shape[-3] * 8, 128)


def decode_b7(img, dtype=torch.bfloat16):
    x = img.contiguous().view(dtype).float().reshape(*img.shape[:-1], 2, 10, 32, 8)
    nd = x.dim()
    return x.permute(*range(nd - 3), nd - 2, nd - 3, nd - 1).reshape(*img.shape[:-1], 2, 32, 80)
```

Baseline: 7.447 million.

## Fold value projection into merge weights and double-buffer A tiles with bulk copies

Folds the per-head value projection into the merge weight on the host. The pair stage-1b kernel then multiplies keys directly against the raw A tile, plus a position term, instead of first computing V per tile, which drops one GEMM and its epilogue per tile. The new p1b3 kernel double-buffers A tiles, loads them with cp.async.bulk on mbarriers by default, issues the next key GEMM ahead, and skips the position path entirely when there is no position code. It relies on reassociating matmuls in reduced precision, which may change numerics slightly, and it adds more complex barrier and parity bookkeeping.

```diff
diff --git a/point-cloud-reid_b200/_lib.py b/point-cloud-reid_b200/_lib.py
--- a/point-cloud-reid_b200/_lib.py
+++ b/point-cloud-reid_b200/_lib.py
@@ -6,6 +6,7 @@
 _lib = None
 
 c_int, c_ll, c_float, c_vp = ctypes.c_int, ctypes.c_longlong, ctypes.c_float, ctypes.c_void_p
+ABI_VERSION = 2
 
 
 class LinearArgs(ctypes.Structure):
@@ -115,6 +116,8 @@
         fn = getattr(L, name)
         fn.argtypes = argt
         fn.restype = c_int
+    if L.pcreid_abi_version() < ABI_VERSION:
+        raise RuntimeError(f"{LIB_PATH} has ABI {L.pcreid_abi_version()}, this package needs {ABI_VERSION}: rebuild it")
     _lib = L
     return L
 
diff --git a/point-cloud-reid_b200/csrc/attn_tc.cu b/point-cloud-reid_b200/csrc/attn_tc.cu
--- a/point-cloud-reid_b200/csrc/attn_tc.cu
+++ b/point-cloud-reid_b200/csrc/attn_tc.cu
@@ -17,15 +17,6 @@
   uint8_t per_obj[MAXCH];
 };
 
-__device__ __forceinline__ void expect_tx(uint64_t* bar, uint32_t bytes) {
-  asm volatile("mbarrier.arrive.expect_tx.shared::cta.b64 _, [%0], %1;" ::"r"(tc::smem_u32(bar)), "r"(bytes) : "memory");
-}
-__device__ __forceinline__ void bulk_g2s(uint32_t dst, const void* src, uint32_t bytes, uint64_t* bar) {
-  asm volatile("cp.async.bulk.shared::cluster.global.mbarrier::complete_tx::bytes [%0], [%1], %2, [%3];" ::"r"(dst), "l"(src),
-               "r"(bytes), "r"(tc::smem_u32(bar))
-               : "memory");
-}
-
 struct Pipe {
   uint64_t *full, *empty;
   uint32_t ring_s;
@@ -40,8 +31,8 @@
     if (n > 0) tc::mbar_wait(&p.empty[s], (uint32_t)((n - 1) & 1));
     const uint8_t* src = (p.tab->per_obj[p.loaded] ? p.obj : p.blob) + p.tab->off[p.loaded];
     const uint32_t nb = p.tab->bytes[p.loaded];
-    expect_tx(&p.full[s], nb);
-    bulk_g2s(p.ring_s + (uint32_t)(s * p.tab->slot_bytes), src, nb, &p.full[s]);
+    tc::expect_tx(&p.full[s], nb);
+    tc::bulk_g2s(p.ring_s + (uint32_t)(s * p.tab->slot_bytes), src, nb, &p.full[s]);
     ++p.loaded;
   }
 }
diff --git a/point-cloud-reid_b200/csrc/pair_common.cuh b/point-cloud-reid_b200/csrc/pair_common.cuh
--- a/point-cloud-reid_b200/csrc/pair_common.cuh
+++ b/point-cloud-reid_b200/csrc/pair_common.cuh
@@ -19,7 +19,8 @@
   float att_eps;
   float kv_scale;
   const int *u_search, *u_templ, *u_slot;
-  const uint8_t *QF1, *H, *PV;
+  const uint8_t *QF1, *H;
+  const uint8_t* PV;
   const uint8_t* MK1;
   const uint8_t* W;
   uint8_t* A_out;
diff --git a/point-cloud-reid_b200/csrc/pair_tc.cu b/point-cloud-reid_b200/csrc/pair_tc.cu
--- a/point-cloud-reid_b200/csrc/pair_tc.cu
+++ b/point-cloud-reid_b200/csrc/pair_tc.cu
@@ -3,19 +3,21 @@
 
 namespace {
 
-constexpr int P1B_WKV = 0, P1B_WM = 16384, P1B_WBYTES = 24576;
-constexpr int P1B_AIMG = 0, P1B_KFV = IMG, P1B_GBYTES = IMG + 2 * IMG + ONES_BYTES;
-
-template <class F, int CS>
-__global__ void __launch_bounds__(NGX * GX * CS, 1) pair_p1b_kernel(const P1Args a) {
+constexpr int P1B_WK = 0, P1B_WC = 8192, P1B_WBYTES = 24576;
+constexpr int P1B_A = 0, P1B_KF = 2 * IMG, P1B_P = 3 * IMG, P1B_ONES = 4 * IMG, P1B_GBYTES = 4 * IMG + 2048;
+constexpr int P1B_TG = 136, P1B_KVC = 64;
+
+template <class F, int CS, bool BULK>
+__global__ void __launch_bounds__(NGX * GX * CS, 1) pair_p1b3_kernel(const P1Args a) {
   constexpr int GT = GX * CS, NTHR = NGX * GT;
   constexpr int QB = 4 / CS, CB = 8 / CS;
+  constexpr uint32_t KVC = P1B_KVC;
   extern __shared__ __align__(1024) uint8_t smem[];
-  __shared__ uint64_t bars[2 * NGX];
+  __shared__ uint64_t bars[4 * NGX];
   __shared__ uint32_t tmem_base_s;
   uint8_t* Wsm = smem;
   if (threadIdx.x == 0) {
-    for (int i = 0; i < 2 * NGX; ++i) tc::mbar_init(&bars[i], 1);
+    for (int i = 0; i < 4 * NGX; ++i) tc::mbar_init(&bars[i], 1);
     tc::fence_mbar_init();
   }
   if (threadIdx.x < 32) { tc::tmem_alloc(&tmem_base_s, 512); tc::tmem_relinquish(); }
@@ -28,54 +30,79 @@
   tc::tc_fence_after();
   const int warp_u = (int)tc::uniform(threadIdx.x >> 5);
   const int gid = warp_u / (4 * CS), wg = warp_u % (4 * CS), gt = threadIdx.x % GT;
-  const int half = wg / 4;
-  const int row = (wg % 4) * 32 + (threadIdx.x & 31);
+  const int half = wg / 4, wq = wg % 4, lane = threadIdx.x & 31;
+  const int row = wq * 32 + lane;
+  const int i64 = 16 * wq + lane;
   const bool issuer = wg == 0;
-  const uint32_t tmem = tc::uniform(tmem_base_s) + gid * 160;
-  const uint32_t tlane = tmem + ((uint32_t)((wg % 4) * 32) << 16);
-  uint64_t* bar = bars + gid;
-  uint32_t par = 0;
+  const uint32_t tmem = tc::uniform(tmem_base_s) + gid * P1B_TG;
+  const uint32_t tlane = tmem + ((uint32_t)(wq * 32) << 16);
+  uint64_t* bar = bars + 4 * gid;
+  uint64_t* bar2 = bar + 1;
+  uint64_t* full = bar + 2;
+  uint32_t par = 0, par2 = 0, fpar = 0;
   auto gsync = [&]() { tc::bar_sync(1 + gid, GT); };
   auto publish = [&]() { tc::fence_async_smem(); tc::tc_fence_before(); gsync(); tc::tc_fence_after(); };
   auto gwait = [&]() { tc::mbar_wait(bar, par); par ^= 1u; tc::tc_fence_after(); };
-  uint64_t* bar2 = bars + NGX + gid;
-  uint32_t par2 = 0;
+  auto gwait2 = [&]() { tc::mbar_wait(bar2, par2); par2 ^= 1u; tc::tc_fence_after(); };
   uint8_t* G = smem + P1B_WBYTES + gid * P1B_GBYTES;
-  uint8_t* Aimg = G + P1B_AIMG;
-  uint8_t* KfV = G + P1B_KFV;
-  {
-    uint4* ones = reinterpret_cast<uint4*>(KfV + 2 * IMG);
-    for (int i = gt; i < 256; i += GT) ones[i] = i < 128 ? make_uint4(F::ONE_LO, 0, 0, 0) : make_uint4(0, 0, 0, 0);
-  }
-  const uint32_t sA = tc::smem_u32(Aimg), sKfV = tc::smem_u32(KfV), sW = tc::smem_u32(Wsm);
-  const uint32_t id64 = tc::instr_desc(128, 64, F::FMT, tc::MAJOR_K, tc::MAJOR_K);
-  const uint32_t idkv = tc::instr_desc(128, 80, F::FMT, tc::MAJOR_MN, tc::MAJOR_MN);
-  const Opnd oA = A_IMG(sA), oWk = W_IMG(sW + P1B_WKV, 128), oWv = W_IMG(sW + P1B_WKV + 64 * 16, 128), oWm = W_IMG(sW + P1B_WM, 64),
-             oKfV = opnd(sKfV, 128u, 2048u, 256u), oVones = opnd(sKfV + 8 * 2048, 128u, 2048u, 256u);
-  const uint32_t KVC = 64;
+  uint8_t* Kf = G + P1B_KF;
+  for (int i = gt; i < 128; i += GT) reinterpret_cast<uint4*>(G + P1B_ONES)[i] = make_uint4(F::ONE_LO, 0, 0, 0);
+  const uint32_t sG = tc::smem_u32(G), sW = tc::smem_u32(Wsm);
+  const uint32_t id_k = tc::instr_desc(128, 64, F::FMT, tc::MAJOR_K, tc::MAJOR_K);
+  const uint32_t id_p = tc::instr_desc(64, 72, F::FMT, tc::MAJOR_MN, tc::MAJOR_MN);
+  const uint32_t id_1 = tc::instr_desc(64, 8, F::FMT, tc::MAJOR_MN, tc::MAJOR_MN);
+  const uint32_t id_a = tc::instr_desc(64, 64, F::FMT, tc::MAJOR_MN, tc::MAJOR_MN);
+  const uint32_t id_m = tc::instr_desc(64, 64, F::FMT, tc::MAJOR_K, tc::MAJOR_K);
+  const Opnd oAk = A_IMG(sG + P1B_A), oAr = opnd(sG + P1B_A, 128u, 2048u, 256u);
+  auto buf = [](Opnd o, int b) { o.desc += (uint64_t)(b * (IMG >> 4)); return o; };
+  const Opnd oKf = opnd(sG + P1B_KF, 128u, 2048u, 256u), oP1 = opnd(sG + P1B_P, 128u, 2048u, 256u),
+             oOnes = opnd(sG + P1B_ONES, 128u, 2048u, 256u), oWk = W_IMG(sW + P1B_WK, 64), oWc = W_IMG(sW + P1B_WC, 64),
+             oKV = opnd(sG + P1B_KF, 1024u, 128u, 2048u);
+  const bool has_pos = a.PV != nullptr;
+  auto a_img = [&](int slot, int tile) { return a.A_out + (((size_t)slot * 2 + a.role) * a.NT + tile) * IMG; };
+  auto load = [&](int buf_off, const uint8_t* src, uint64_t* fb) {
+    if constexpr (BULK) {
+      if (gt == 0) { tc::expect_tx(fb, IMG); tc::bulk_g2s(sG + buf_off, src, IMG, fb); }
+    } else {
+      copy_to_smem(G + buf_off, src, IMG, gt, GT);
+      cp_async_commit();
+    }
+  };
+  auto issue_k = [&](int b) {
+    if constexpr (BULK) { tc::mbar_wait(&full[b], (fpar >> b) & 1u); tc::tc_fence_after(); }
+    issue_gemm<4>(tmem, buf(oAk, b), oWk, id_k, false);
+  };
 
   const int ngroups = gridDim.x * NGX, gg = blockIdx.x * NGX + gid;
   const int u0 = (int)((long long)a.n_units * gg / ngroups), u1 = (int)((long long)a.n_units * (gg + 1) / ngroups);
   int so_next = u0 < u1 ? a.u_search[u0] : 0, slot_next = u0 < u1 ? a.u_slot[u0] : 0;
-  bool prefetched = false;
+  int b = 0;
+  uint4 pos_r[CB];
+  auto load_pos = [&](int so_, int tile_) {
+    const uint8_t* img = a.PV + ((size_t)so_ * a.NT + tile_) * IMG;
+#pragma unroll
+    for (int c = 0; c < CB; ++c) pos_r[c] = ldg_early(img + (half * CB + c) * 2048 + row * 16);
+  };
+  if (u0 < u1) {
+    if (has_pos) load_pos(so_next, 0);
+    load(P1B_A, a_img(slot_next, 0), &full[0]);
+    if constexpr (!BULK) cp_async_wait<0>();
+    publish();
+    if (issuer) { if (tc::elect_one()) { issue_k(0); tc::umma_commit(bar); } __syncwarp(); }
+    if constexpr (BULK) fpar ^= 1u;
+  }
   for (int u = u0; u < u1; ++u) {
     const int so = so_next, slot = slot_next;
     if (u + 1 < u1) { so_next = a.u_search[u + 1]; slot_next = a.u_slot[u + 1]; }
     for (int tile = 0; tile < a.NT; ++tile) {
-      const size_t ti = (size_t)so * a.NT + tile;
-      if (!prefetched) copy_to_smem(Aimg, a.A_out + (((size_t)slot * 2 + a.role) * a.NT + tile) * IMG, IMG, gt, GT);
-      prefetched = false;
-      cp_async_commit();
-      {
-        int ns = slot, nt = tile + 1;
-        if (nt == a.NT) { ns = slot_next; nt = 0; }
-        if ((nt != 0 || u + 1 < u1) && gt < 128) prefetch_l2_16k(a.A_out + (((size_t)ns * 2 + a.role) * a.NT + nt) * IMG, gt);
-      }
-      cp_async_wait<0>();
-      publish();
-      if (issuer) { if (tc::elect_one()) { issue_gemm<4>(tmem, oA, oWk, id64, false); tc::umma_commit(bar); } __syncwarp(); }
+      const bool last = tile + 1 == a.NT, more = !last || u + 1 < u1;
       gwait();
-      if (tile > 0) { tc::mbar_wait(bar2, par2); par2 ^= 1u; tc::tc_fence_after(); }
+      if (more) load(P1B_A + (b ^ 1) * IMG, last ? a_img(slot_next, 0) : a_img(slot, tile + 1), &full[b ^ 1]);
+      if (has_pos) {
+#pragma unroll
+        for (int c = 0; c < CB; ++c) *reinterpret_cast<uint4*>(G + P1B_P + (half * CB + c) * 2048 + row * 16) = pos_r[c];
+        if (more) load_pos(last ? so_next : so, last ? 0 : tile + 1);
+      }
       {
         const bool keep = tile * 128 + row < a.npts;
 #pragma unroll
@@ -90,309 +117,85 @@
 #pragma unroll
             for (int j = 0; j < 4; ++j)
               w[j] = keep ? F::elu1(__uint_as_float(r[c * 8 + 2 * j]), __uint_as_float(r[c * 8 + 2 * j + 1])) : 0u;
-            *reinterpret_cast<uint4*>(KfV + (2 * q + c) * 2048 + row * 16) = make_uint4(w[0], w[1], w[2], w[3]);
+            *reinterpret_cast<uint4*>(Kf + (2 * q + c) * 2048 + row * 16) = make_uint4(w[0], w[1], w[2], w[3]);
           }
         }
       }
-      tc::tc_fence_before();
-      gsync();
-      tc::tc_fence_after();
-      if (issuer) { if (tc::elect_one()) { issue_gemm<4>(tmem, oA, oWv, id64, false); tc::umma_commit(bar); } __syncwarp(); }
-      {
-        uint4 sdPV[CB];
-        load_side<CB>(sdPV, a.PV + ti * IMG, half * CB, row);
-        gwait();
-        if (tile + 1 < a.NT) {
-          copy_to_smem(Aimg, a.A_out + (((size_t)slot * 2 + a.role) * a.NT + tile + 1) * IMG, IMG, gt, GT);
-          cp_async_commit();
-          prefetched = true;
-        }
-#pragma unroll
-        for (int qq = 0; qq < QB; ++qq) {
-          const int q = half * QB + qq;
-          uint32_t r[16];
-          tc::tmem_ld16(tlane + 16 * q, r);
-          tc::tmem_ld_wait();
-#pragma unroll
-          for (int c = 0; c < 2; ++c) {
-            const uint4 s4 = sdPV[2 * qq + c];
-            const uint32_t sw[4] = {s4.x, s4.y, s4.z, s4.w};
-            uint32_t w[4];
-#pragma unroll
-            for (int j = 0; j < 4; ++j)
-              w[j] = F::add(__uint_as_float(r[c * 8 + 2 * j]), __uint_as_float(r[c * 8 + 2 * j + 1]), sw[j]);
-            *reinterpret_cast<uint4*>(KfV + (8 + 2 * q + c) * 2048 + row * 16) = make_uint4(w[0], w[1], w[2], w[3]);
-          }
-        }
-      }
+      if constexpr (!BULK) cp_async_wait<0>();
       publish();
       if (issuer) {
-        if (tc::elect_one()) { issue_gemm<8>(tmem + KVC, oKfV, oVones, idkv, tile > 0); tc::umma_commit(bar2); }
+        if (tc::elect_one()) {
+          if (has_pos) issue_gemm<8>(tmem + KVC, oKf, oP1, id_p, tile > 0);
+          else issue_gemm<8>(tmem + KVC + 64, oKf, oOnes, id_1, tile > 0);
+          issue_gemm<8>(tmem + KVC, oKf, buf(oAr, b), id_a, tile > 0 || has_pos);
+          if (!last) { issue_k(b ^ 1); tc::umma_commit(bar); }
+          else tc::umma_commit(bar2);
+        }
         __syncwarp();
       }
-    }
-    tc::mbar_wait(bar2, par2);
-    par2 ^= 1u;
-    tc::tc_fence_after();
+      if constexpr (BULK) { if (!last) fpar ^= 1u << (b ^ 1); }
+      b ^= 1;
+    }
+    gwait2();
+    float kv[64 / CS];
+    float ksum = 0.f;
+#pragma unroll
+    for (int qq = 0; qq < QB; ++qq) {
+      uint32_t r[16];
+      tc::tmem_ld16(tlane + KVC + 16 * (half * QB + qq), r);
+      tc::tmem_ld_wait();
+#pragma unroll
+      for (int j = 0; j < 16; ++j) kv[16 * qq + j] = __uint_as_float(r[j]) * a.kv_scale;
+    }
     {
-      float kv[64 / CS];
-      float ksum = 0.f;
-      if (row < 64) {
-#pragma unroll
-        for (int qq = 0; qq < QB; ++qq) {
-          uint32_t r[16];
-          tc::tmem_ld16(tlane + KVC + 16 * (half * QB + qq), r);
-          tc::tmem_ld_wait();
-#pragma unroll
-          for (int j = 0; j < 16; ++j) kv[16 * qq + j] = __uint_as_float(r[j]) * a.kv_scale;
-        }
-        uint32_t r8[8];
-        tc::tmem_ld8(tlane + KVC + 64, r8);
-        tc::tmem_ld_wait();
-        ksum = __uint_as_float(r8[0]) * a.kv_scale;
-        const int hd = row >> 5;
-#pragma unroll
-        for (int cc = 0; cc < CB; ++cc) {
-          const int c = half * CB + cc;
-          uint32_t w[4];
-#pragma unroll
-          for (int j = 0; j < 4; ++j) w[j] = ((c >> 2) == hd) ? F::pack(kv[cc * 8 + 2 * j], kv[cc * 8 + 2 * j + 1]) : 0u;
-          *reinterpret_cast<uint4*>(Aimg + c * 2048 + row * 16) = make_uint4(w[0], w[1], w[2], w[3]);
-        }
-      } else {
-#pragma unroll
-        for (int cc = 0; cc < CB; ++cc) *reinterpret_cast<uint4*>(Aimg + (half * CB + cc) * 2048 + row * 16) = make_uint4(0, 0, 0, 0);
-      }
-      publish();
-      if (issuer) { if (tc::elect_one()) { issue_gemm<4>(tmem, oA, oWm, id64, false); tc::umma_commit(bar); } __syncwarp(); }
-      gwait();
-      if (u + 1 < u1) {
-        copy_to_smem(Aimg, a.A_out + ((size_t)slot_next * 2 + a.role) * a.NT * IMG, IMG, gt, GT);
-        cp_async_commit();
-        prefetched = true;
-      }
-      if (row < 64) {
-#pragma unroll
-        for (int qq = 0; qq < QB; ++qq) {
-          uint32_t r[16];
-          tc::tmem_ld16(tlane + 16 * (half * QB + qq), r);
-          tc::tmem_ld_wait();
-#pragma unroll
-          for (int j = 0; j < 16; ++j) kv[16 * qq + j] = __uint_as_float(r[j]);
-        }
-        uint8_t* dst = a.B7_out + ((size_t)slot * 2 + a.role) * B7_BYTES;
-        if constexpr (CS == 1) write_b7_row<F>(kv, ksum, row, dst);
-        else write_b7_part<F>(kv, 4 * half, ksum, half == 0, row, dst);
-      }
-      tc::tc_fence_before();
-      gsync();
-    }
-  }
+      uint32_t r8[8];
+      tc::tmem_ld8(tlane + KVC + 64, r8);
+      tc::tmem_ld_wait();
+      ksum = __uint_as_float(r8[0]) * a.kv_scale;
+    }
+    if (lane < 16) {
+      const int hd = i64 >> 5;
+#pragma unroll
+      for (int cc = 0; cc < CB; ++cc) {
+        uint32_t w[4];
+#pragma unroll
+        for (int j = 0; j < 4; ++j) w[j] = F::pack(kv[cc * 8 + 2 * j], kv[cc * 8 + 2 * j + 1]);
+        const int c = half * CB + cc;
+        *reinterpret_cast<uint4*>(Kf + (8 * hd + c) * 1024 + i64 * 16) = make_uint4(w[0], w[1], w[2], w[3]);
+        *reinterpret_cast<uint4*>(Kf + (8 * (1 - hd) + c) * 1024 + i64 * 16) = make_uint4(0, 0, 0, 0);
+      }
+    }
+    publish();
+    if (issuer) {
+      if (tc::elect_one()) {
+        issue_gemm<8>(tmem + KVC, oKV, oWc, id_m, false);
+        tc::umma_commit(bar2);
+        if (u + 1 < u1) { issue_k(b); tc::umma_commit(bar); }
+      }
+      __syncwarp();
+    }
+    if constexpr (BULK) { if (u + 1 < u1) fpar ^= 1u << b; }
+    gwait2();
+#pragma unroll
+    for (int qq = 0; qq < QB; ++qq) {
+      uint32_t r[16];
+      tc::tmem_ld16(tlane + KVC + 16 * (half * QB + qq), r);
+      tc::tmem_ld_wait();
+#pragma unroll
+      for (int j = 0; j < 16; ++j) kv[16 * qq + j] = __uint_as_float(r[j]);
+    }
+    if (lane < 16) {
+      uint8_t* dst = a.B7_out + ((size_t)slot * 2 + a.role) * B7_BYTES;
+      if constexpr (CS == 1) write_b7_row<F>(kv, ksum, i64, dst);
+      else write_b7_part<F>(kv, 4 * half, ksum, half == 0, i64, dst);
+    }
+    tc::tc_fence_before();
+  }
+  if constexpr (!BULK) cp_async_wait<0>();
   tc::tc_fence_before();
   __syncthreads();
   if (threadIdx.x < 32) tc::tmem_dealloc(tmem_base_s, 512);
 }
-
-template <class F>
-__global__ void __launch_bounds__(NGX * GX, 1) pair_p1b2_kernel(const P1Args a) {
-  constexpr int TG = 168, KVC = 64, AC = 136;
-  extern __shared__ __align__(1024) uint8_t smem[];
-  __shared__ uint64_t bars[2 * NGX];
-  __shared__ uint32_t tmem_base_s;
-  __shared__ float ksum_s[NGX][64];
-  uint8_t* Wsm = smem;
-  if (threadIdx.x == 0) {
-    for (int i = 0; i < 2 * NGX; ++i) tc::mbar_init(&bars[i], 1);
-    tc::fence_mbar_init();
-  }
-  if (threadIdx.x < 32) { tc::tmem_alloc(&tmem_base_s, 512); tc::tmem_relinquish(); }
-  copy_to_smem(Wsm, a.W, P1B_WBYTES, threadIdx.x, NGX * GX);
-  cp_async_commit();
-  cp_async_wait<0>();
-  tc::fence_async_smem();
-  tc::tc_fence_before();
-  __syncthreads();
-  tc::tc_fence_after();
-  const int warp_u = (int)tc::uniform(threadIdx.x >> 5);
-  const int gid = warp_u / 4, wq = warp_u % 4, row = threadIdx.x % GX, lane = threadIdx.x & 31;
-  const bool issuer = wq == 0;
-  const uint32_t tmem = tc::uniform(tmem_base_s) + gid * TG;
-  const uint32_t tlane = tmem + ((uint32_t)(wq * 32) << 16);
-  uint64_t* bar = bars + gid;
-  uint32_t par = 0;
-  auto gsync = [&]() { tc::bar_sync(1 + gid, GX); };
-  auto publish = [&]() { tc::fence_async_smem(); tc::tc_fence_before(); gsync(); tc::tc_fence_after(); };
-  auto gwait = [&]() { tc::mbar_wait(bar, par); par ^= 1u; tc::tc_fence_after(); };
-  uint64_t* bar2 = bars + NGX + gid;
-  uint32_t par2 = 0;
-  uint8_t* G = smem + P1B_WBYTES + gid * P1B_GBYTES;
-  uint8_t* Aimg = G + P1B_AIMG;
-  uint8_t* KfV = G + P1B_KFV;
-  {
-    uint4* ones = reinterpret_cast<uint4*>(KfV + 2 * IMG);
-    ones[row] = make_uint4(F::ONE_LO, 0, 0, 0);
-    ones[128 + row] = make_uint4(0, 0, 0, 0);
-  }
-  const uint32_t sA = tc::smem_u32(Aimg), sKfV = tc::smem_u32(KfV), sW = tc::smem_u32(Wsm);
-  const uint32_t id64 = tc::instr_desc(128, 64, F::FMT, tc::MAJOR_K, tc::MAJOR_K);
-  const uint32_t idkv = tc::instr_desc(64, 72, F::FMT, tc::MAJOR_MN, tc::MAJOR_MN);
-  const Opnd oA = A_IMG(sA), oWk = W_IMG(sW + P1B_WKV, 128), oWv = W_IMG(sW + P1B_WKV + 64 * 16, 128), oWm = W_IMG(sW + P1B_WM, 64),
-             oKf = opnd(sKfV, 128u, 2048u, 256u), oVones = opnd(sKfV + 8 * 2048, 128u, 2048u, 256u);
-
-  const int ngroups = gridDim.x * NGX, gg = blockIdx.x * NGX + gid;
-  const int u0 = (int)((long long)a.n_units * gg / ngroups), u1 = (int)((long long)a.n_units * (gg + 1) / ngroups);
-  int so_next = u0 < u1 ? a.u_search[u0] : 0, slot_next = u0 < u1 ? a.u_slot[u0] : 0;
-  uint32_t areg[32];
-  auto load_row = [&](const uint8_t* img) {
-#pragma unroll
-    for (int c = 0; c < 8; ++c) {
-      const uint4 v = ldg_early(img + c * 2048 + row * 16);
-      areg[4 * c] = v.x; areg[4 * c + 1] = v.y; areg[4 * c + 2] = v.z; areg[4 * c + 3] = v.w;
-    }
-  };
-  if (u0 < u1) load_row(a.A_out + ((size_t)slot_next * 2 + a.role) * a.NT * IMG);
-  for (int u = u0; u < u1; ++u) {
-    const int so = so_next, slot = slot_next;
-    if (u + 1 < u1) { so_next = a.u_search[u + 1]; slot_next = a.u_slot[u + 1]; }
-    for (int tile = 0; tile < a.NT; ++tile) {
-      const size_t ti = (size_t)so * a.NT + tile;
-      tc::tmem_st32(tlane + AC, areg);
-      tc::tmem_st_wait();
-      tc::tc_fence_before();
-      gsync();
-      tc::tc_fence_after();
-      if (issuer) {
-        if (tc::elect_one()) {
-#pragma unroll
-          for (int ks = 0; ks < 4; ++ks) tc::umma_f16_ts(tmem, tmem + AC + 8 * ks, oWk.desc + (uint64_t)(ks * oWk.kstep), id64, ks > 0 ? 1u : 0u);
-          tc::umma_commit(bar);
-        }
-        __syncwarp();
-      }
-      {
-        int ns = slot, nt = tile + 1;
-        if (nt == a.NT) { ns = slot_next; nt = 0; }
-        if (nt != 0 || u + 1 < u1) {
-          load_row(a.A_out + (((size_t)ns * 2 + a.role) * a.NT + nt) * IMG);
-          int ns2 = ns, nt2 = nt + 1;
-          if (nt2 == a.NT) { nt2 = 0; ns2 = -1; }
-          if (ns2 >= 0) prefetch_l2_16k(a.A_out + (((size_t)ns2 * 2 + a.role) * a.NT + nt2) * IMG, row);
-        }
-      }
-      gwait();
-      if (tile > 0) { tc::mbar_wait(bar2, par2); par2 ^= 1u; tc::tc_fence_after(); }
-      {
-        const bool keep = tile * 128 + row < a.npts;
-#pragma unroll
-        for (int q = 0; q < 4; ++q) {
-          uint32_t r[16];
-          tc::tmem_ld16(tlane + 16 * q, r);
-          tc::tmem_ld_wait();
-#pragma unroll
-          for (int c = 0; c < 2; ++c) {
-            uint32_t w[4];
-#pragma unroll
-            for (int j = 0; j < 4; ++j)
-              w[j] = keep ? F::elu1(__uint_as_float(r[c * 8 + 2 * j]), __uint_as_float(r[c * 8 + 2 * j + 1])) : 0u;
-            *reinterpret_cast<uint4*>(KfV + (2 * q + c) * 2048 + row * 16) = make_uint4(w[0], w[1], w[2], w[3]);
-          }
-        }
-      }
-      tc::tc_fence_before();
-      gsync();
-      tc::tc_fence_after();
-      if (issuer) {
-        if (tc::elect_one()) {
-#pragma unroll
-          for (int ks = 0; ks < 4; ++ks) tc::umma_f16_ts(tmem, tmem + AC + 8 * ks, oWv.desc + (uint64_t)(ks * oWv.kstep), id64, ks > 0 ? 1u : 0u);
-          tc::umma_commit(bar);
-        }
-        __syncwarp();
-      }
-      {
-        uint4 sdPV[8];
-        load_side<8>(sdPV, a.PV + ti * IMG, 0, row);
-        gwait();
-#pragma unroll
-        for (int q = 0; q < 4; ++q) {
-          uint32_t r[16];
-          tc::tmem_ld16(tlane + 16 * q, r);
-          tc::tmem_ld_wait();
-#pragma unroll
-          for (int c = 0; c < 2; ++c) {
-            const uint4 s4 = sdPV[2 * q + c];
-            const uint32_t sw[4] = {s4.x, s4.y, s4.z, s4.w};
-            uint32_t w[4];
-#pragma unroll
-            for (int j = 0; j < 4; ++j)
-              w[j] = F::add(__uint_as_float(r[c * 8 + 2 * j]), __uint_as_float(r[c * 8 + 2 * j + 1]), sw[j]);
-            *reinterpret_cast<uint4*>(KfV + (8 + 2 * q + c) * 2048 + row * 16) = make_uint4(w[0], w[1], w[2], w[3]);
-          }
-        }
-      }
-      publish();
-      if (issuer) {
-        if (tc::elect_one()) { issue_gemm<8>(tmem + KVC, oKf, oVones, idkv, tile > 0); tc::umma_commit(bar2); }
-        __syncwarp();
-      }
-    }
-    tc::mbar_wait(bar2, par2);
-    par2 ^= 1u;
-    tc::tc_fence_after();
-    {
-      {
-        float kv[64];
-        uint32_t r8[8];
-#pragma unroll
-        for (int q = 0; q < 4; ++q) {
-          uint32_t r[16];
-          tc::tmem_ld16(tlane + KVC + 16 * q, r);
-          tc::tmem_ld_wait();
-#pragma unroll
-          for (int j = 0; j < 16; ++j) kv[16 * q + j] = __uint_as_float(r[j]) * a.kv_scale;
-        }
-        tc::tmem_ld8(tlane + KVC + 64, r8);
-        tc::tmem_ld_wait();
-        if (lane < 16) {
-          const int i = 16 * wq + lane, hd = i >> 5;
-          ksum_s[gid][i] = __uint_as_float(r8[0]) * a.kv_scale;
-#pragma unroll
-          for (int c = 0; c < 8; ++c) {
-            uint32_t w[4];
-#pragma unroll
-            for (int j = 0; j < 4; ++j) w[j] = ((c >> 2) == hd) ? F::pack(kv[c * 8 + 2 * j], kv[c * 8 + 2 * j + 1]) : 0u;
-            *reinterpret_cast<uint4*>(Aimg + c * 2048 + i * 16) = make_uint4(w[0], w[1], w[2], w[3]);
-          }
-        }
-      }
-      if (row >= 64) {
-#pragma unroll
-        for (int c = 0; c < 8; ++c) *reinterpret_cast<uint4*>(Aimg + c * 2048 + row * 16) = make_uint4(0, 0, 0, 0);
-      }
-      publish();
-      if (issuer) { if (tc::elect_one()) { issue_gemm<4>(tmem, oA, oWm, id64, false); tc::umma_commit(bar); } __syncwarp(); }
-      gwait();
-      if (row < 64) {
-        float kv[64];
-#pragma unroll
-        for (int q = 0; q < 4; ++q) {
-          uint32_t r[16];
-          tc::tmem_ld16(tlane + 16 * q, r);
-          tc::tmem_ld_wait();
-#pragma unroll
-          for (int j = 0; j < 16; ++j) kv[16 * q + j] = __uint_as_float(r[j]);
-        }
-        write_b7_row<F>(kv, ksum_s[gid][row], row, a.B7_out + ((size_t)slot * 2 + a.role) * B7_BYTES);
-      }
-      tc::tc_fence_before();
-      gsync();
-    }
-  }
-  tc::tc_fence_before();
-  __syncthreads();
-  if (threadIdx.x < 32) tc::tmem_dealloc(tmem_base_s, 512);
-}
-
 
 template <class F>
 __global__ void __launch_bounds__(256) pack_image_kernel(int B, int C, int N, const float* __restrict__ src, long long s_bs,
@@ -429,24 +232,19 @@
 
 }
 
-template <class F, int CS>
-static int launch_p1b_cs(const P1Args& a, int grid, cudaStream_t st) {
+template <class F, int CS, bool BULK>
+static int launch_p1b3(const P1Args& a, int grid, cudaStream_t st) {
   const int smem = P1B_WBYTES + NGX * P1B_GBYTES;
-  cudaFuncSetAttribute(pair_p1b_kernel<F, CS>, cudaFuncAttributeMaxDynamicSharedMemorySize, smem);
-  pair_p1b_kernel<F, CS><<<grid, NGX * GX * CS, smem, st>>>(a);
+  cudaFuncSetAttribute(pair_p1b3_kernel<F, CS, BULK>, cudaFuncAttributeMaxDynamicSharedMemorySize, smem);
+  pair_p1b3_kernel<F, CS, BULK><<<grid, NGX * GX * CS, smem, st>>>(a);
   return pcreid_launch_status();
 }
 template <class F>
 static int launch_p1b(const P1Args& a, int grid, cudaStream_t st) {
-  static const int gen = [] { const char* e = getenv("PCREID_P1B"); return e ? atoi(e) : 2; }();
+  static const bool bulk = [] { const char* e = getenv("PCREID_P1B"); return !(e && atoi(e) == 1); }();
   static const int cs = [] { const char* e = getenv("PCREID_P1B_SPLIT"); return e ? atoi(e) : 1; }();
-  if (gen == 2) {
-    const int smem = P1B_WBYTES + NGX * P1B_GBYTES;
-    cudaFuncSetAttribute(pair_p1b2_kernel<F>, cudaFuncAttributeMaxDynamicSharedMemorySize, smem);
-    pair_p1b2_kernel<F><<<grid, NGX * GX, smem, st>>>(a);
-    return pcreid_launch_status();
-  }
-  return cs == 2 ? launch_p1b_cs<F, 2>(a, grid, st) : launch_p1b_cs<F, 1>(a, grid, st);
+  if (cs == 2) return bulk ? launch_p1b3<F, 2, true>(a, grid, st) : launch_p1b3<F, 2, false>(a, grid, st);
+  return bulk ? launch_p1b3<F, 1, true>(a, grid, st) : launch_p1b3<F, 1, false>(a, grid, st);
 }
 
 extern "C" {
@@ -474,7 +272,7 @@
 int pcreid_pair_p1b_n(int n_units, int npts, int role, int fmt, float kv_scale, const int* u_search, const int* u_templ,
                       const int* u_slot, const void* PV, const void* W, void* A_out, void* B7_out, int n_ctas, void* stream) {
   if (n_units <= 0) return PCREID_OK;
-  if (!u_search || !u_templ || !u_slot || !PV || !W || !A_out || !B7_out || npts <= 0 ||
+  if (!u_search || !u_templ || !u_slot || !W || !A_out || !B7_out || npts <= 0 ||
       (fmt != PCREID_FMT_BF16 && fmt != PCREID_FMT_F16))
     return PCREID_ERR_ARG;
   const int NT = (npts + 127) / 128;
diff --git a/point-cloud-reid_b200/csrc/rowops.cu b/point-cloud-reid_b200/csrc/rowops.cu
--- a/point-cloud-reid_b200/csrc/rowops.cu
+++ b/point-cloud-reid_b200/csrc/rowops.cu
@@ -720,7 +720,7 @@
 
 extern "C" {
 
-int pcreid_abi_version(void) { return 1; }
+int pcreid_abi_version(void) { return 2; }
 
 int pcreid_cn_linear(const pcreid_linear_args* p, void* stream) {
   if (!p) return PCREID_ERR_ARG;
diff --git a/point-cloud-reid_b200/csrc/tc_common.cuh b/point-cloud-reid_b200/csrc/tc_common.cuh
--- a/point-cloud-reid_b200/csrc/tc_common.cuh
+++ b/point-cloud-reid_b200/csrc/tc_common.cuh
@@ -24,6 +24,14 @@
         : "memory");
   } while (!ok);
 }
+__device__ __forceinline__ void expect_tx(uint64_t* bar, uint32_t bytes) {
+  asm volatile("mbarrier.arrive.expect_tx.shared::cta.b64 _, [%0], %1;" ::"r"(smem_u32(bar)), "r"(bytes) : "memory");
+}
+__device__ __forceinline__ void bulk_g2s(uint32_t dst, const void* src, uint32_t bytes, uint64_t* bar) {
+  asm volatile("cp.async.bulk.shared::cluster.global.mbarrier::complete_tx::bytes [%0], [%1], %2, [%3];" ::"r"(dst), "l"(src),
+               "r"(bytes), "r"(smem_u32(bar))
+               : "memory");
+}
 
 __device__ __forceinline__ void fence_async_smem() { asm volatile("fence.proxy.async.shared::cta;" ::: "memory"); }
 __device__ __forceinline__ void tc_fence_before() { asm volatile("tcgen05.fence::before_thread_sync;" ::: "memory"); }
diff --git a/point-cloud-reid_b200/models/fused_pairs.py b/point-cloud-reid_b200/models/fused_pairs.py
--- a/point-cloud-reid_b200/models/fused_pairs.py
+++ b/point-cloud-reid_b200/models/fused_pairs.py
@@ -21,6 +21,11 @@
 
 
 _OPS = _T.ops
+
+
+def fold_value_merge(Wv, Wm, nhead):
+    dh = Wv.shape[0] // nhead
+    return torch.cat([Wm[:, h * dh:(h + 1) * dh] @ Wv[h * dh:(h + 1) * dh] for h in range(nhead)], 1)
 
 
 def _w_image(w, dtype):
@@ -70,9 +75,8 @@
                 self._w1a2 = torch.cat([
                     _w_image(W0ext1, dt), _w_image(_center_out(X1.mlp[2].weight), dt), _f32_bytes(X1.norm2.weight)]).contiguous()
                 self._merge1c = kmajor(_center_out(X1.merge.weight))
-                self._w1b2 = torch.cat([
-                    _w_image(torch.cat([X2.k_proj.weight, X2.v_proj.weight], 0), dt),
-                    _w_image(_center_out(X2.merge.weight), dt)]).contiguous()
+                Wcomb = fold_value_merge(f(X2.v_proj.weight), _center_out(X2.merge.weight), X2.nhead)
+                self._w1b2 = torch.cat([_w_image(X2.k_proj.weight, dt), _w_image(Wcomb, dt)]).contiguous()
                 W0ext = torch.zeros((2 * d, 2 * d + 16), device=W0_2.device)
                 W0ext[:, :d] = W0_2[:, :d]
                 W0ext[:, d:2 * d] = W0_2[:, d:] * f(X2.norm1.weight)[None, :]
@@ -109,7 +113,7 @@
 
     def prepare(self, h, xyz):
         X1, X2 = self.model.cross_stage1, self.model.cross_stage2
-        pk1, pk2 = X1.packed(), X2.packed()
+        pk1 = X1.packed()
         self._weights()
         B, C, N = h.shape
         o = ObjectPack()
@@ -118,10 +122,7 @@
         o.H = torch.empty((B, (N + 127) // 128, C // 8, 128, 16), device=h.device, dtype=torch.uint8)
         _OPS.pack_image_bias(B, C, N, h, h.stride(0), h.stride(1), self._b2_1, self.fmt, o.H)
         pos2 = X2.position_code(xyz)
-        if pos2 is None:
-            o.PV = torch.zeros((B, (N + 127) // 128, C // 8, 128, 16), device=h.device, dtype=torch.uint8)
-        else:
-            o.PV = self._pack_image(K.cn_linear(pos2, pk2["v"]))
+        o.PV = None if pos2 is None else self._pack_image(pos2)
         wkv, ksum = X1.template_summary(h, X1.position_code(xyz))
         M = K.cn_linear(wkv, self._merge1c, x1_pm=True, y_pm=True)
         sc = self.kv_scale(N)
@@ -191,7 +192,7 @@
             self._tock("pair_p1a2_kernel", e0, P)
             e0 = self._tick()
             _OPS.pair_p1b_n(P, N, role, self.fmt, sc, bs, bt, bl, ps.PV, self._w1b2, A, B7, self.n_ctas)
-            self._tock("pair_p1b_kernel" if os.environ.get("PCREID_P1B") == "1" else "pair_p1b2_kernel", e0, P)
+            self._tock("pair_p1b3_kernel", e0, P)
         slots = torch.arange(P, device=dev, dtype=torch.int32)
         pooled = torch.empty((1, 128, P), device=dev, dtype=torch.float32)
         for role in (0, 1):
```

New measurement: 7.426 million, median of 6. No clear change (-0.3%).
